# NVlabs/nvbio

Measured on AMD Instinct MI355X. Metric: aligned reads/s (100 bp, band=15), higher is better.
Workload: dtype int32 results (int16 lanes where proven exact; all-int32 kernel in roofline.a32); 1 GPU; nvbio::aln batched banded SW (configs[1]): 10000000 x 100 bp reads vs 150 bp windows per GPU, band=15, LOCAL Gotoh (2,-1,-2,-1); reads_per_gpu=10000000, read_len=100, band=15, type=LOCAL, parallelism=read-shard x1, gather to rank 0

## Files before the change

include/nvbio_hip.h:

```cpp
#ifndef NVBIO_HIP_H
#define NVBIO_HIP_H

#include <stdint.h>

#ifdef __cplusplus
extern "C" {
#endif

#define NVBIO_HIP_ABI_VERSION 2

enum { NVBIO_HIP_GLOBAL = 0, NVBIO_HIP_LOCAL = 1, NVBIO_HIP_SEMI_GLOBAL = 2 };

typedef struct nvbio_hip_string_set {
    const uint32_t* words;
    uint64_t        n_words;
    uint32_t        bits;
    uint32_t        big_endian;
    const uint64_t* begin;
    const uint32_t* length;
    uint32_t        fixed_length;
    uint32_t        _pad;
} nvbio_hip_string_set;

typedef struct nvbio_hip_gotoh_scheme {
    int32_t match, mismatch, gap_open, gap_ext;
} nvbio_hip_gotoh_scheme;


int nvbio_hip_banded_gotoh_score(
    const nvbio_hip_gotoh_scheme* scheme , int32_t type, uint32_t band_len,
    const nvbio_hip_string_set* patterns ,
    const nvbio_hip_string_set* texts    ,
    uint32_t max_pattern_len, uint32_t max_text_len ,
    uint32_t n, int32_t* out_score, uint32_t* out_sink, void* stream);

int nvbio_hip_gotoh_score(
    const nvbio_hip_gotoh_scheme* scheme , int32_t type,
    const nvbio_hip_string_set* patterns, const nvbio_hip_string_set* texts,
    uint32_t max_pattern_len, uint32_t max_text_len, const int32_t* min_score ,
    uint32_t n, int32_t* out_score, uint32_t* out_sink, uint8_t* out_ok, void* stream);

typedef struct nvbio_hip_sw_scheme { int32_t match, mismatch, deletion, insertion; } nvbio_hip_sw_scheme;

int nvbio_hip_banded_sw_score(
    const nvbio_hip_sw_scheme* scheme , int32_t type, uint32_t band_len,
    const nvbio_hip_string_set* patterns, const nvbio_hip_string_set* texts,
    uint32_t max_pattern_len, uint32_t max_text_len,
    uint32_t n, int32_t* out_score, uint32_t* out_sink, void* stream);
int nvbio_hip_sw_score(
    const nvbio_hip_sw_scheme* scheme , int32_t type,
    const nvbio_hip_string_set* patterns, const nvbio_hip_string_set* texts,
    uint32_t max_pattern_len, uint32_t max_text_len,
    uint32_t n, int32_t* out_score, uint32_t* out_sink, void* stream);

enum { NVBIO_HIP_GOTOH_ALIGNER = 0, NVBIO_HIP_SW_ALIGNER = 1 };
enum { NVBIO_HIP_PATTERN_BLOCKING = 0, NVBIO_HIP_TEXT_BLOCKING = 1 };
int nvbio_hip_alignment_score(
    int32_t aligner, int32_t algorithm, const int32_t* scheme4 , int32_t type,
    const nvbio_hip_string_set* patterns, const nvbio_hip_string_set* texts,
    uint32_t max_pattern_len, uint32_t max_text_len, const int32_t* min_score ,
    uint32_t n, int32_t* out_score, uint32_t* out_sink, uint8_t* out_ok , void* stream);

typedef struct nvbio_hip_gotoh_qual_scheme {
    int32_t match;
    int32_t pattern_gap_open, pattern_gap_ext, text_gap_open, text_gap_ext;
    int32_t mismatch[256];
} nvbio_hip_gotoh_qual_scheme;

int nvbio_hip_banded_gotoh_score_qual(
    const nvbio_hip_gotoh_qual_scheme* scheme , int32_t type, uint32_t band_len,
    const nvbio_hip_string_set* patterns, const uint8_t* quals, uint64_t n_quals,
    const nvbio_hip_string_set* texts,
    uint32_t max_pattern_len, uint32_t max_text_len,
    uint32_t n, int32_t* out_score, uint32_t* out_sink, void* stream);

int nvbio_hip_banded_gotoh_score_qual_views(
    const nvbio_hip_gotoh_qual_scheme* scheme , int32_t type, uint32_t band_len,
    const nvbio_hip_string_set* patterns, const uint8_t* quals, uint64_t n_quals, const uint8_t* pattern_flags ,
    const nvbio_hip_string_set* texts,
    uint32_t max_pattern_len, uint32_t max_text_len,
    uint32_t n, int32_t* out_score, uint32_t* out_sink, void* stream);

int nvbio_hip_banded_gotoh_score_qual_wave(
    const nvbio_hip_gotoh_qual_scheme* scheme, int32_t type, uint32_t band_len,
    const nvbio_hip_string_set* patterns, const uint8_t* quals , uint64_t n_quals,
    const nvbio_hip_string_set* texts, uint32_t max_pattern_len,
    uint32_t n, const uint32_t* n_on_device , const uint32_t* job_index , const uint32_t* out_index ,
    const uint32_t* gate , uint32_t gate_limit,
    int32_t* out_score, uint32_t* out_sink, void* stream);

int nvbio_hip_banded_gotoh_score_qual_bounded(
    const nvbio_hip_gotoh_qual_scheme* scheme, int32_t type, uint32_t band_len,
    const nvbio_hip_string_set* patterns, const uint8_t* quals, uint64_t n_quals, const uint8_t* pattern_flags,
    const nvbio_hip_string_set* texts,
    uint32_t max_pattern_len, uint32_t max_text_len,
    uint32_t n, const uint32_t* n_on_device, const int32_t* min_score, uint32_t* work_counter, const uint32_t* out_index,
    const uint32_t* gate , uint32_t gate_limit,
    int32_t* out_score, uint32_t* out_sink, void* stream);

uint64_t nvbio_hip_banded_gotoh_traceback_temp_bytes(uint32_t band_len, uint32_t max_pattern_len, uint32_t n);
int nvbio_hip_banded_gotoh_traceback(
    const nvbio_hip_gotoh_scheme* scheme , int32_t type, uint32_t band_len,
    const nvbio_hip_string_set* patterns, const nvbio_hip_string_set* texts,
    uint32_t max_pattern_len, uint32_t max_text_len, uint32_t n,
    int32_t* out_score, uint32_t* out_sink, uint32_t* out_source,
    uint16_t* out_cigar, uint32_t cigar_stride, uint32_t* out_cigar_len,
    void* temp, uint64_t temp_bytes, void* stream);
int nvbio_hip_banded_gotoh_traceback_qual(
    const nvbio_hip_gotoh_qual_scheme* scheme , int32_t type, uint32_t band_len,
    const nvbio_hip_string_set* patterns, const uint8_t* quals, uint64_t n_quals,
    const nvbio_hip_string_set* texts,
    uint32_t max_pattern_len, uint32_t max_text_len, uint32_t n,
    int32_t* out_score, uint32_t* out_sink, uint32_t* out_source,
    uint16_t* out_cigar, uint32_t cigar_stride, uint32_t* out_cigar_len,
    void* temp, uint64_t temp_bytes, void* stream);
int nvbio_hip_banded_gotoh_traceback_qual_known(
    const nvbio_hip_gotoh_qual_scheme* scheme , int32_t type, uint32_t band_len,
    const nvbio_hip_string_set* patterns, const uint8_t* quals, uint64_t n_quals,
    const nvbio_hip_string_set* texts,
    uint32_t max_pattern_len, uint32_t max_text_len, uint32_t n,
    int32_t* score , uint32_t* sink , uint32_t* out_source,
    uint16_t* out_cigar, uint32_t cigar_stride, uint32_t* out_cigar_len,
    void* temp, uint64_t temp_bytes, void* stream);

uint64_t nvbio_hip_gotoh_traceback_temp_bytes(uint32_t max_pattern_len, uint32_t max_text_len, uint32_t n);
int nvbio_hip_gotoh_traceback(
    const nvbio_hip_gotoh_scheme* scheme , int32_t type,
    const nvbio_hip_string_set* patterns, const nvbio_hip_string_set* texts,
    uint32_t max_pattern_len, uint32_t max_text_len, uint32_t n,
    int32_t* out_score, uint32_t* out_sink, uint32_t* out_source,
    uint16_t* out_cigar, uint32_t cigar_stride, uint32_t* out_cigar_len,
    void* temp, uint64_t temp_bytes, void* stream);

int nvbio_hip_gotoh_traceback_qual(
    const nvbio_hip_gotoh_qual_scheme* scheme , int32_t type,
    const nvbio_hip_string_set* patterns, const uint8_t* quals, uint64_t n_quals, const nvbio_hip_string_set* texts,
    uint32_t max_pattern_len, uint32_t max_text_len, uint32_t n,
    int32_t* out_score, uint32_t* out_sink, uint32_t* out_source,
    uint16_t* out_cigar, uint32_t cigar_stride, uint32_t* out_cigar_len,
    void* temp, uint64_t temp_bytes, void* stream);

int nvbio_hip_gotoh_traceback_known_score(
    const nvbio_hip_gotoh_scheme* scheme , int32_t type,
    const nvbio_hip_string_set* patterns, const nvbio_hip_string_set* texts, const int32_t* known_score,
    uint32_t max_pattern_len, uint32_t max_text_len, uint32_t n,
    int32_t* out_score, uint32_t* out_sink, uint32_t* out_source,
    uint16_t* out_cigar, uint32_t cigar_stride, uint32_t* out_cigar_len,
    void* temp, uint64_t temp_bytes, void* stream);
int nvbio_hip_gotoh_traceback_qual_known_score(
    const nvbio_hip_gotoh_qual_scheme* scheme , int32_t type,
    const nvbio_hip_string_set* patterns, const uint8_t* quals, uint64_t n_quals, const nvbio_hip_string_set* texts, const int32_t* known_score,
    uint32_t max_pattern_len, uint32_t max_text_len, uint32_t n,
    int32_t* out_score, uint32_t* out_sink, uint32_t* out_source,
    uint16_t* out_cigar, uint32_t cigar_stride, uint32_t* out_cigar_len,
    void* temp, uint64_t temp_bytes, void* stream);

uint64_t nvbio_hip_known_score_redone(void);

int nvbio_hip_banded_sw_traceback(
    const nvbio_hip_sw_scheme* scheme , int32_t type, uint32_t band_len,
    const nvbio_hip_string_set* patterns, const nvbio_hip_string_set* texts,
    uint32_t max_pattern_len, uint32_t max_text_len, uint32_t n,
    int32_t* out_score, uint32_t* out_sink, uint32_t* out_source,
    uint16_t* out_cigar, uint32_t cigar_stride, uint32_t* out_cigar_len,
    void* temp, uint64_t temp_bytes, void* stream);
int nvbio_hip_sw_traceback(
    const nvbio_hip_sw_scheme* scheme , int32_t type,
    const nvbio_hip_string_set* patterns, const nvbio_hip_string_set* texts,
    uint32_t max_pattern_len, uint32_t max_text_len, uint32_t n,
    int32_t* out_score, uint32_t* out_sink, uint32_t* out_source,
    uint16_t* out_cigar, uint32_t cigar_stride, uint32_t* out_cigar_len,
    void* temp, uint64_t temp_bytes, void* stream);

int nvbio_hip_alignment_score_qual(
    const nvbio_hip_gotoh_qual_scheme* scheme , int32_t algorithm, int32_t type,
    const nvbio_hip_string_set* patterns, const uint8_t* quals, uint64_t n_quals, const nvbio_hip_string_set* texts,
    uint32_t max_pattern_len, uint32_t max_text_len, const int32_t* min_score ,
    uint32_t n, int32_t* out_score, uint32_t* out_sink, uint8_t* out_ok , void* stream);

int nvbio_hip_alignment_score_qual_jobs(
    const nvbio_hip_gotoh_qual_scheme* scheme , int32_t algorithm, int32_t type,
    const nvbio_hip_string_set* patterns, const uint8_t* quals, uint64_t n_quals, const nvbio_hip_string_set* texts,
    uint32_t max_pattern_len, uint32_t max_text_len, const int32_t* min_score ,
    uint32_t n, const uint32_t* n_on_device, const uint32_t* job_index, const uint32_t* gate, uint32_t gate_limit, int32_t wave_form,
    int32_t* out_score, uint32_t* out_sink, uint8_t* out_ok , void* stream);

int nvbio_hip_hamming_score(
    const nvbio_hip_sw_scheme* scheme , int32_t algorithm, int32_t type,
    const nvbio_hip_string_set* patterns, const nvbio_hip_string_set* texts,
    uint32_t max_pattern_len, uint32_t max_text_len, const int32_t* min_score ,
    uint32_t n, int32_t* out_score, uint32_t* out_sink, uint8_t* out_ok , void* stream);
int nvbio_hip_hamming_score_qual(
    const nvbio_hip_gotoh_qual_scheme* scheme , int32_t algorithm, int32_t type,
    const nvbio_hip_string_set* patterns, const uint8_t* quals, uint64_t n_quals, const nvbio_hip_string_set* texts,
    uint32_t max_pattern_len, uint32_t max_text_len, const int32_t* min_score ,
    uint32_t n, int32_t* out_score, uint32_t* out_sink, uint8_t* out_ok , void* stream);
int nvbio_hip_hamming_score_qual_jobs(
    const nvbio_hip_gotoh_qual_scheme* scheme , int32_t algorithm, int32_t type,
    const nvbio_hip_string_set* patterns, const uint8_t* quals, uint64_t n_quals, const nvbio_hip_string_set* texts,
    uint32_t max_pattern_len, uint32_t max_text_len, const int32_t* min_score ,
    uint32_t n, const uint32_t* n_on_device, const uint32_t* job_index, const uint32_t* gate, uint32_t gate_limit, int32_t wave_form,
    int32_t* out_score, uint32_t* out_sink, uint8_t* out_ok , void* stream);

typedef struct nvbio_hip_fmindex {
    uint32_t        length;
    uint32_t        primary;
    uint32_t        L2[5];
    uint32_t        sa_int;
    const uint32_t* bwt_occ;
    const uint32_t* ssa;
    const uint32_t* ktab;
    uint32_t        ktab_k;
    uint32_t        _pad;
    const uint32_t* dimer;
    uint32_t        dimer_p1, dimer_fill1;
    uint32_t        dimer_S[4], dimer_T[4];
    const uint32_t* trimer;
} nvbio_hip_fmindex;

int nvbio_hip_fm_rank(const nvbio_hip_fmindex* fmi, const uint32_t* k, const uint8_t* c,
                      uint32_t n, uint32_t* out, void* stream);

int nvbio_hip_fm_rank4(const nvbio_hip_fmindex* fmi, const uint32_t* k,
                       uint32_t n, uint32_t* out, void* stream);

int nvbio_hip_fm_rank_range(const nvbio_hip_fmindex* fmi, const uint32_t* range, const uint8_t* c,
                            uint32_t n, uint32_t* out, void* stream);

int nvbio_hip_fm_match(const nvbio_hip_fmindex* fmi, const nvbio_hip_string_set* seeds,
                       uint32_t n, uint32_t* out_range, void* stream);

uint64_t nvbio_hip_fm_dimer_index_bytes(uint32_t length);
uint64_t nvbio_hip_fm_build_dimer_index_temp_bytes(uint32_t length);
int nvbio_hip_fm_build_dimer_index(const nvbio_hip_fmindex* fmi, uint32_t* out_dimer, void* temp, uint64_t temp_bytes, void* stream);
int nvbio_hip_fm_attach_dimer_index(nvbio_hip_fmindex* fmi, const uint32_t* dimer, void* stream);

uint64_t nvbio_hip_fm_trimer_index_bytes(uint32_t length);
uint64_t nvbio_hip_fm_build_trimer_index_temp_bytes(uint32_t length);
int nvbio_hip_fm_build_trimer_index(const nvbio_hip_fmindex* fmi, uint32_t* out_trimer, void* temp, uint64_t temp_bytes, void* stream);
int nvbio_hip_fm_attach_trimer_index(nvbio_hip_fmindex* fmi, const uint32_t* trimer, void* stream);

int nvbio_hip_banded_gotoh_score_host(const nvbio_hip_gotoh_scheme* scheme, int32_t type, uint32_t band_len,
                                      const nvbio_hip_string_set* patterns, const nvbio_hip_string_set* texts,
                                      uint32_t n, int32_t* out_score, uint32_t* out_sink, int32_t n_threads);
int nvbio_hip_banded_sw_score_host(const nvbio_hip_sw_scheme* scheme, int32_t type, uint32_t band_len,
                                   const nvbio_hip_string_set* patterns, const nvbio_hip_string_set* texts,
                                   uint32_t n, int32_t* out_score, uint32_t* out_sink, int32_t n_threads);
int nvbio_hip_alignment_score_host(int32_t aligner, int32_t algorithm, const int32_t* scheme4, int32_t type,
                                   const nvbio_hip_string_set* patterns, const nvbio_hip_string_set* texts, const int32_t* min_score ,
                                   uint32_t n, int32_t* out_score, uint32_t* out_sink, uint8_t* out_ok , int32_t n_threads);
int nvbio_hip_hamming_score_host(const nvbio_hip_sw_scheme* scheme, int32_t algorithm, int32_t type,
                                 const nvbio_hip_string_set* patterns, const nvbio_hip_string_set* texts, const int32_t* min_score ,
                                 uint32_t n, int32_t* out_score, uint32_t* out_sink, uint8_t* out_ok , int32_t n_threads);
int nvbio_hip_hamming_score_qual_host(const nvbio_hip_gotoh_qual_scheme* scheme, int32_t algorithm, int32_t type,
                                      const nvbio_hip_string_set* patterns, const uint8_t* quals, uint64_t n_quals, const nvbio_hip_string_set* texts,
                                      const int32_t* min_score ,
                                      uint32_t n, int32_t* out_score, uint32_t* out_sink, uint8_t* out_ok , int32_t n_threads);
int nvbio_hip_fm_rank_host(const nvbio_hip_fmindex* fmi, const uint32_t* k, const uint8_t* c, uint32_t n, uint32_t* out, int32_t n_threads);
int nvbio_hip_fm_match_host(const nvbio_hip_fmindex* fmi, const nvbio_hip_string_set* seeds, uint32_t n, uint32_t* out_range, int32_t n_threads);
int nvbio_hip_fm_locate_host(const nvbio_hip_fmindex* fmi, const uint32_t* sa_rows, uint32_t n, uint32_t* out_pos, int32_t n_threads);

int nvbio_hip_fm_build_ktab(const nvbio_hip_fmindex* fmi, uint32_t k, uint32_t* out_ktab, void* stream);
uint64_t nvbio_hip_fm_dense_ssa_entries(uint32_t length, uint32_t sa_int);
int nvbio_hip_fm_build_dense_ssa(const nvbio_hip_fmindex* fmi, uint32_t sa_int_out, uint32_t* out_ssa, void* stream);

typedef struct nvbio_hip_map_params {
    uint32_t seed_len;
    uint32_t min_read_len;
    uint32_t max_hits;
    uint32_t max_reseed;
    uint32_t retry;
    uint32_t rep_seeds;
    uint32_t fw, rc;
} nvbio_hip_map_params;

int nvbio_hip_map_exact(const nvbio_hip_fmindex* fmi, const nvbio_hip_string_set* reads,
                        const uint32_t* in_queue, uint32_t n, const nvbio_hip_map_params* params ,
                        const uint32_t* seed_freq_by_len ,
                        uint64_t* out_hits, uint32_t hits_stride, uint32_t* out_counts, uint8_t* out_reseed, void* stream);

enum { NVBIO_HIP_EXACT_MAPPING = 0, NVBIO_HIP_APPROX_MAPPING = 1, NVBIO_HIP_CASE_PRUNING_MAPPING = 2 };

int nvbio_hip_map(int32_t algorithm, uint32_t subseed_len,
                  const nvbio_hip_fmindex* fmi, const nvbio_hip_fmindex* rfmi ,
                  const nvbio_hip_string_set* reads, const uint32_t* in_queue, uint32_t n,
                  const nvbio_hip_map_params* params , const uint32_t* seed_freq_by_len ,
                  uint64_t* out_hits, uint32_t hits_stride, uint32_t* out_counts, uint8_t* out_reseed, void* stream);

uint64_t nvbio_hip_alignment_invalid(void);
int nvbio_hip_init_alignments(uint32_t n_reads, const uint32_t* read_len , uint32_t fixed_read_len,
                              const int32_t* worst_score_by_len , uint32_t mate,
                              uint64_t* best_alignments, uint32_t best_stride, void* stream);
int nvbio_hip_score_reduce(uint32_t n_active, const uint32_t* read_ids , const uint64_t* hit_begin,
                           const int32_t* hit_score, const uint32_t* hit_loc, const uint8_t* hit_rc,
                           const uint32_t* read_len , uint32_t fixed_read_len,
                           uint64_t* best_alignments, uint32_t best_stride, void* stream);

uint32_t nvbio_hip_sum_tree_node_count(uint32_t size);
int nvbio_hip_select_init(uint32_t n_reads, const char* read_names, const uint32_t* read_names_idx,
                          const uint64_t* hits, uint32_t hits_stride, const uint32_t* hit_counts,
                          float* probs, uint32_t probs_stride, uint32_t* trys , uint32_t* rseeds,
                          uint32_t max_effort_init, int32_t randomized, int32_t top_seed, void* stream);
int nvbio_hip_select_init_queued(uint32_t n_queue, const uint32_t* queue, const char* read_names, const uint32_t* read_names_idx,
                                 const uint64_t* hits, uint32_t hits_stride, const uint32_t* hit_counts,
                                 float* probs, uint32_t probs_stride, uint32_t* trys , uint32_t* rseeds,
                                 uint32_t max_effort_init, int32_t randomized, int32_t top_seed, void* stream);
uint64_t nvbio_hip_select_temp_bytes(uint32_t n_active, uint32_t n_multi);
int nvbio_hip_select(int32_t randomized, uint32_t n_multi, const uint32_t* active_in, uint32_t n_active,
                     uint64_t* hits, uint32_t hits_stride, uint32_t* hit_counts,
                     float* probs, uint32_t probs_stride, uint32_t* rseeds, const uint32_t* trys,
                     uint32_t* active_out, uint64_t* hit_begin, uint32_t* hit_read_id, uint32_t* hit_loc, uint32_t* hit_seed,
                     uint32_t* out_sizes, void* temp, uint64_t temp_bytes, void* stream);
int nvbio_hip_hit_deque_replay(uint32_t n_cases, const uint32_t* case_start, const uint8_t* ops, const uint64_t* vals, const uint32_t* caps,
                               const uint64_t* state_start, uint64_t* scratch, uint32_t scratch_stride, uint64_t* out_states, void* stream);
int nvbio_hip_locate_hits(const nvbio_hip_fmindex* fmi, const nvbio_hip_fmindex* rfmi, uint32_t n,
                          uint32_t* hit_loc, const uint32_t* hit_seed, void* stream);
int nvbio_hip_score_best_setup(uint32_t n_hits, const uint32_t* hit_read_id, const uint32_t* hit_loc, const uint32_t* hit_seed,
                               const uint64_t* read_begin , const uint32_t* read_len , uint32_t fixed_read_len,
                               uint64_t rc_offset, uint32_t band_len, uint32_t genome_length,
                               const uint64_t* best_alignments, uint32_t best_stride, int32_t score_limit,
                               uint64_t* pattern_begin, uint32_t* pattern_len ,
                               uint64_t* text_begin, uint32_t* text_len, int32_t* min_score,
                               int32_t* known_score ,
                               uint32_t* job_count , uint32_t* job_hit , void* stream);
int nvbio_hip_score_reduce_best_approx(uint32_t n_active, const uint32_t* active_reads, const uint64_t* hit_begin,
                                       const int32_t* hit_score, const uint32_t* hit_loc, const uint32_t* hit_seed,
                                       const uint32_t* read_len , uint32_t fixed_read_len,
                                       uint64_t* best_alignments, uint32_t best_stride, int32_t worst_score,
                                       uint32_t* trys, uint32_t* hit_counts,
                                       uint32_t n_ext, uint32_t min_ext, uint32_t max_ext, uint32_t max_effort,
                                       const int32_t* known_score ,
                                       const uint32_t* hit_sink , uint32_t* best_sink ,
                                       void* stream);
int nvbio_hip_traceback_best_known(uint32_t n, const uint32_t* idx , const uint64_t* best_alignments, const uint32_t* best_sink ,
                                   int32_t* out_score, uint32_t* out_sink , void* stream);

int nvbio_hip_score_reduce_paired(uint32_t n_active, const uint32_t* read_ids , const uint64_t* hit_begin,
    const uint32_t* hit_loc, const uint32_t* hit_sink, const int32_t* hit_score, const uint8_t* hit_rc,
    const uint32_t* opposite_loc, const uint32_t* opposite_sink, const uint32_t* opposite_sink2,
    const int32_t* opposite_score, const int32_t* opposite_score2,
    const uint32_t* read_len , uint32_t fixed_read_len, uint32_t anchor, int32_t pe_policy, int32_t pe_unpaired, int32_t score_limit,
    uint64_t* best_alignments, uint64_t* best_alignments_o, uint32_t best_stride, void* stream);

typedef struct nvbio_hip_pe_params {
    int32_t  pe_policy, min_frag_len, max_frag_len, pe_overlap, score_limit;
    uint32_t anchor, genome_length;
} nvbio_hip_pe_params;

int nvbio_hip_opposite_mate_windows(uint32_t n_hits, const uint32_t* hit_read_id, const uint8_t* hit_rc, const uint32_t* hit_loc, const int32_t* hit_score,
    const uint32_t* a_read_len , const uint32_t* o_read_len , uint32_t a_fixed_len, uint32_t o_fixed_len,
    const uint64_t* best_alignments, const uint64_t* best_alignments_o, uint32_t best_stride,
    int32_t match, const int32_t* min_score_by_len , int32_t text_gap_open, int32_t text_gap_ext, const nvbio_hip_pe_params* params ,
    uint8_t* out_valid, int32_t* out_min_score, uint8_t* out_read_rc, uint32_t* out_genome_begin, uint32_t* out_genome_end, void* stream);

int nvbio_hip_anchor_score_setup(uint32_t n_hits, const uint32_t* hit_read_id, const uint32_t* hit_loc, const uint32_t* hit_seed,
    const uint64_t* a_read_begin , const uint32_t* a_read_len , const uint32_t* o_read_len ,
    uint32_t a_fixed_len, uint32_t o_fixed_len, uint64_t rc_offset,
    uint32_t band_len, uint32_t genome_length, const uint64_t* best_alignments, const uint64_t* best_alignments_o, uint32_t best_stride,
    int32_t match, const int32_t* min_score_by_len , int32_t score_limit, uint32_t anchor,
    uint64_t* pattern_begin, uint32_t* pattern_len , uint64_t* text_begin, uint32_t* text_len, int32_t* min_score, void* stream);
int nvbio_hip_anchor_score_finish(uint32_t n_hits, const int32_t* raw_score, const uint32_t* raw_sink , const uint64_t* text_begin,
    const int32_t* min_score, int32_t worst_score, int32_t* hit_score, uint32_t* hit_sink, void* stream);
int nvbio_hip_opposite_score_setup(uint32_t n_hits, const uint32_t* hit_read_id, const uint32_t* hit_seed, const uint32_t* hit_loc, const int32_t* hit_score,
    int32_t worst_score, const uint32_t* a_read_len, const uint32_t* o_read_len, uint32_t a_fixed_len, uint32_t o_fixed_len,
    const uint64_t* best_alignments, const uint64_t* best_alignments_o, uint32_t best_stride,
    int32_t match, const int32_t* min_score_by_len , int32_t text_gap_open, int32_t text_gap_ext, const nvbio_hip_pe_params* params ,
    uint8_t* out_valid, int32_t* out_min_score, uint8_t* out_read_rc, uint32_t* out_genome_begin, uint32_t* out_genome_end,
    const uint64_t* o_read_begin, uint64_t o_rc_offset, uint64_t* out_pattern_begin, uint64_t* out_text_begin, uint32_t* out_text_len, void* stream);
int nvbio_hip_opposite_score_finish(uint32_t n_valid, const uint32_t* valid_idx, const uint8_t* valid_flags, const int32_t* raw_score , const uint32_t* raw_sink ,
    const int32_t* min_score , const uint32_t* genome_begin , int32_t worst_score,
    int32_t* opposite_score, int32_t* opposite_score2, uint32_t* opposite_loc, uint32_t* opposite_sink, uint32_t* opposite_sink2, void* stream);
int nvbio_hip_score_reduce_paired_best_approx(uint32_t n_active, const uint32_t* active_reads, const uint64_t* hit_begin,
    const uint32_t* hit_loc, const uint32_t* hit_sink, const int32_t* hit_score, const uint32_t* hit_seed,
    const uint32_t* opposite_loc, const uint32_t* opposite_sink, const uint32_t* opposite_sink2, const int32_t* opposite_score, const int32_t* opposite_score2,
    const uint32_t* read_len , uint32_t fixed_read_len, uint32_t anchor, int32_t pe_policy, int32_t pe_unpaired, int32_t score_limit,
    uint64_t* best_alignments, uint64_t* best_alignments_o, uint32_t best_stride,
    uint32_t* trys, uint32_t* hit_counts, uint32_t n_ext, uint32_t min_ext, uint32_t max_ext, uint32_t max_effort, void* stream);
int nvbio_hip_anchor_memo_mark(uint32_t n_hits, const uint32_t* hit_read_id, const uint32_t* hit_seed, const uint64_t* text_begin, const uint32_t* text_len,
    uint32_t anchor, const uint32_t* memo, uint8_t* from_memo, uint32_t* text_len_out,
    uint32_t* live_count , uint32_t* live_idx , void* stream);
int nvbio_hip_anchor_score_finish_memo(uint32_t n_hits, const int32_t* raw_score, const uint32_t* raw_sink, const uint64_t* text_begin, const int32_t* min_score,
    int32_t worst_score, const uint8_t* from_memo, const uint32_t* hit_read_id, const uint32_t* memo, int32_t* hit_score, uint32_t* hit_sink, void* stream);
int nvbio_hip_anchor_memo_update(uint32_t n_active, const uint32_t* active_reads, const uint64_t* hit_begin, const uint32_t* hit_read_id, const uint32_t* hit_seed,
    const uint64_t* text_begin, const uint32_t* text_len_setup, const uint8_t* from_memo, const int32_t* raw_score, const uint32_t* raw_sink, uint32_t anchor, uint32_t* memo, void* stream);
int nvbio_hip_list_flagged(uint32_t n, const uint8_t* flags, uint32_t value, uint32_t* count, uint32_t* idx, void* stream);
int nvbio_hip_opposite_memo_lookup(uint32_t n_hits, const uint32_t* hit_read_id, uint8_t* valid, const uint8_t* read_rc, const uint32_t* genome_begin,
    const uint32_t* genome_end, const int32_t* min_score, uint32_t anchor, const uint32_t* memo, int32_t worst_score,
    int32_t* opposite_score, int32_t* opposite_score2, uint32_t* opposite_loc, uint32_t* opposite_sink, uint32_t* opposite_sink2,
    uint32_t* text_len , void* stream);
int nvbio_hip_opposite_memo_update(uint32_t n_active, const uint32_t* active_reads, const uint64_t* hit_begin, const uint8_t* valid, const uint8_t* read_rc,
    const uint32_t* genome_begin, const uint32_t* genome_end, const int32_t* min_score, const int32_t* opposite_score, const uint32_t* opposite_sink,
    uint32_t anchor, uint32_t* memo, void* stream);
int nvbio_hip_mark_discordant(uint32_t n_reads, uint64_t* best_alignments, uint64_t* best_alignments_o, uint32_t best_stride, void* stream);

int nvbio_hip_pack_read_queue(uint32_t n, const uint32_t* queue, uint32_t top_flag, uint32_t* out, void* stream);

int nvbio_hip_mark_unaligned(uint32_t n_active, const uint32_t* active_reads, const uint64_t* best_alignments, uint8_t* reseed, void* stream);
uint64_t nvbio_hip_copy_flagged_temp_bytes(uint32_t n);
int nvbio_hip_copy_flagged(uint32_t n, const uint32_t* in, const uint8_t* flags, uint32_t* out, uint32_t* out_count ,
                           void* temp, uint64_t temp_bytes, void* stream);
int nvbio_hip_scatter_rows(uint32_t n, const uint32_t* idx, const void* src, void* dst, uint32_t row_bytes , void* stream);
int nvbio_hip_gather_rows(uint32_t n, const uint32_t* idx, const void* src, void* dst, uint32_t row_bytes , void* stream);
int nvbio_hip_traceback_best_setup(uint32_t n, const uint32_t* idx , const uint64_t* best_alignments, uint32_t band_len, uint32_t genome_length,
                                   const uint64_t* read_begin , const uint32_t* read_len , uint32_t fixed_read_len,
                                   uint64_t rc_offset, uint64_t mate_offset, int32_t want,
                                   uint8_t* out_valid, uint64_t* pattern_begin, uint32_t* pattern_len ,
                                   uint64_t* text_begin, uint32_t* text_len, void* stream);
int nvbio_hip_traceback_best_setup_mates(uint32_t n, const uint32_t* idx , const uint64_t* best_alignments, uint32_t band_len, uint32_t genome_length,
                                         const uint64_t* const read_begin[2] , const uint32_t* const read_len[2],
                                         const uint32_t fixed_read_len[2], const uint64_t rc_offset[2], uint64_t mate_offset, int32_t want,
                                         uint8_t* out_valid, uint64_t* pattern_begin, uint32_t* pattern_len, uint64_t* text_begin, uint32_t* text_len, void* stream);

int nvbio_hip_finish_alignment(uint32_t n, const uint8_t* valid, const nvbio_hip_string_set* patterns, const uint8_t* quals , uint64_t n_quals,
                               const nvbio_hip_string_set* texts, const uint16_t* cigar, uint32_t cigar_stride, const uint32_t* cigar_len,
                               const uint32_t* cigar_source , int32_t match, const int32_t* mismatch_by_quality , int32_t n_penalty,
                               const int32_t* gap_costs , const uint32_t* idx , uint64_t* best_alignments, uint8_t* out_mds, uint32_t mds_stride, uint32_t* out_mds_len, void* stream);

int nvbio_hip_gather_ranges(uint32_t n_ranges, uint32_t n_reads, const uint64_t* hits, uint32_t hits_stride, const uint32_t* hit_count_scan,
                            uint64_t* out_ranges, void* stream);
int nvbio_hip_select_all(uint64_t begin, uint32_t count, uint32_t n_reads, uint32_t n_ranges, const uint64_t* hits, uint32_t hits_stride,
                         const uint32_t* hit_count_scan, const uint64_t* hit_range_scan, uint32_t* out_loc, uint32_t* out_seed, uint32_t* out_read_id,
                         void* stream);
int nvbio_hip_mark_straddling(uint32_t n, const uint32_t* idx_queue, uint32_t n_sequences, const uint32_t* sequence_index, const uint32_t* hit_loc,
                              uint32_t seed_len, uint8_t* flags, void* stream);
int nvbio_hip_score_all_setup(uint32_t n, const uint32_t* idx , const uint32_t* hit_read_id, const uint32_t* hit_loc, const uint32_t* hit_seed,
                              const uint64_t* read_begin , const uint32_t* read_len , uint32_t fixed_read_len, uint64_t rc_offset,
                              uint32_t band_len, uint32_t genome_length,
                              uint64_t* pattern_begin, uint32_t* pattern_len , uint64_t* text_begin, uint32_t* text_len, void* stream);
int nvbio_hip_score_all_output(uint32_t n, const uint32_t* idx , const uint32_t* hit_read_id, const uint32_t* hit_loc, const uint32_t* hit_seed,
                               const int32_t* score, const int32_t* min_score_by_len , const uint32_t* read_len , uint32_t fixed_read_len,
                               uint8_t* out_flags, uint64_t* out_alignments, uint32_t* out_read_id, void* stream);
int nvbio_hip_traceback_all_setup(uint32_t n, const uint64_t* alignments, const uint32_t* read_id,
                                  const uint64_t* read_begin , const uint32_t* read_len , uint32_t fixed_read_len, uint64_t rc_offset,
                                  uint32_t band_len, uint32_t genome_length,
                                  uint64_t* pattern_begin, uint32_t* pattern_len , uint64_t* text_begin, uint32_t* text_len, void* stream);

uint64_t nvbio_hip_all_mapping_temp_bytes(uint32_t n);
int nvbio_hip_inclusive_scan_u32(uint32_t n, const uint32_t* in, uint32_t* out, void* temp, uint64_t temp_bytes, void* stream);
int nvbio_hip_inclusive_scan_u64(uint32_t n, const uint64_t* in, uint64_t* out, void* temp, uint64_t temp_bytes, void* stream);
int nvbio_hip_sort_hi_bits(uint32_t n, const uint32_t* keys, uint32_t* out_idx, void* temp, uint64_t temp_bytes, void* stream);
int nvbio_hip_sort_hits(uint32_t n, const uint32_t* hit_read_id, const uint32_t* hit_loc, const uint32_t* hit_seed, uint32_t* out_idx, uint8_t* out_first,
                        void* temp, uint64_t temp_bytes, void* stream);
int nvbio_hip_sort_hits_pingpong(uint32_t n, const uint32_t* hit_read_id, const uint32_t* hit_loc, const uint32_t* hit_seed, uint32_t* out_idx, uint8_t* out_first,
                                 uint32_t* out_stale, void* temp, uint64_t temp_bytes, void* stream);

int nvbio_hip_mapq(int32_t version, int32_t match, int32_t monotone, const int32_t* min_score_by_len ,
                   uint32_t n_reads, const uint64_t* best_alignments, uint32_t best_stride,
                   const uint32_t* read_len , uint32_t fixed_read_len, uint8_t* out_mapq, void* stream);

int nvbio_hip_mapq_paired(int32_t version, int32_t match, int32_t monotone, const int32_t* min_score_by_len ,
                          uint32_t n_reads, const uint64_t* best_alignments, const uint64_t* best_alignments_o, uint32_t best_stride,
                          const uint32_t* read_len , const uint32_t* o_read_len ,
                          uint32_t fixed_read_len, uint32_t o_fixed_read_len, uint8_t* out_mapq, void* stream);

int nvbio_hip_fm_locate(const nvbio_hip_fmindex* fmi, const uint32_t* sa_rows,
                        uint32_t n, uint32_t* out_pos, void* stream);

int nvbio_hip_fm_locate_ssa_iterator(const nvbio_hip_fmindex* fmi, const uint32_t* sa_rows,
                                     uint32_t n, uint32_t* out_it, void* stream);
int nvbio_hip_fm_lookup_ssa_iterator(const nvbio_hip_fmindex* fmi, const uint32_t* it,
                                     uint32_t n, uint32_t* out_pos, void* stream);

uint64_t nvbio_hip_fm_filter_temp_bytes(uint32_t n);
int nvbio_hip_fm_filter_rank(const nvbio_hip_fmindex* fmi, const nvbio_hip_string_set* seeds,
                             uint32_t n, uint32_t* out_range, uint64_t* out_slots,
                             void* temp, uint64_t temp_bytes, void* stream);

int nvbio_hip_fm_filter_locate(const nvbio_hip_fmindex* fmi, const uint32_t* range, const uint64_t* slots,
                               uint32_t n_queries, uint64_t begin, uint64_t end,
                               uint32_t* out_hits, void* stream);

#define NVBIO_HIP_EXTEND_FORWARD   0
#define NVBIO_HIP_EXTEND_BACKWARDS 1
int nvbio_hip_fm_extend(int32_t direction, const nvbio_hip_fmindex* f_fmi, const nvbio_hip_fmindex* r_fmi,
                        const uint32_t* f_ranges, const uint32_t* r_ranges, const uint8_t* c, uint32_t n,
                        uint32_t* out_f_ranges, uint32_t* out_r_ranges, void* stream);

#define NVBIO_HIP_ERROR_CAPACITY 0x10001
uint64_t nvbio_hip_fm_mem_temp_bytes(uint32_t n, uint32_t max_pattern_len);
int nvbio_hip_fm_mem_rank(const nvbio_hip_fmindex* f_fmi, const nvbio_hip_fmindex* r_fmi, const nvbio_hip_string_set* strings,
                          uint32_t n, uint32_t max_pattern_len, uint32_t min_intv, uint32_t max_intv, uint32_t min_span,
                          uint32_t* out_ranges, uint64_t capacity, uint64_t* out_index, uint64_t* out_slots, uint64_t* out_n_ranges,
                          void* temp, uint64_t temp_bytes, void* stream);

int nvbio_hip_fm_mem_locate(const nvbio_hip_fmindex* f_fmi, const uint32_t* ranges, const uint64_t* slots, uint64_t n_ranges,
                            uint64_t begin, uint64_t end, uint32_t* out_hits, void* stream);

int nvbio_hip_fm_extend_host(int32_t direction, const nvbio_hip_fmindex* f_fmi, const nvbio_hip_fmindex* r_fmi,
                             const uint32_t* f_ranges, const uint32_t* r_ranges, const uint8_t* c, uint32_t n,
                             uint32_t* out_f_ranges, uint32_t* out_r_ranges, int32_t n_threads);
int nvbio_hip_fm_mem_rank_host(const nvbio_hip_fmindex* f_fmi, const nvbio_hip_fmindex* r_fmi, const nvbio_hip_string_set* strings,
                               uint32_t n, uint32_t max_pattern_len, uint32_t min_intv, uint32_t max_intv, uint32_t min_span,
                               uint32_t* out_ranges, uint64_t capacity, uint64_t* out_index, uint64_t* out_slots, uint64_t* out_n_ranges,
                               uint64_t* out_records, int32_t n_threads);
int nvbio_hip_fm_mem_locate_host(const nvbio_hip_fmindex* f_fmi, const uint32_t* ranges, const uint64_t* slots, uint64_t n_ranges,
                                 uint64_t begin, uint64_t end, uint32_t* out_hits, int32_t n_threads);

uint64_t nvbio_hip_fm_mem_split_temp_bytes(uint32_t n, uint32_t max_pattern_len, uint64_t capacity);
int nvbio_hip_fm_mem_rank_split(const nvbio_hip_fmindex* f_fmi, const nvbio_hip_fmindex* r_fmi, const nvbio_hip_string_set* strings,
                                uint32_t n, uint32_t max_pattern_len, uint32_t min_intv, uint32_t max_intv, uint32_t min_span,
                                uint32_t split_len, uint32_t split_width,
                                uint32_t* out_ranges, uint64_t capacity, uint64_t* out_index, uint64_t* out_slots, uint64_t* out_n_ranges,
                                void* temp, uint64_t temp_bytes, void* stream);
int nvbio_hip_fm_mem_rank_split_host(const nvbio_hip_fmindex* f_fmi, const nvbio_hip_fmindex* r_fmi, const nvbio_hip_string_set* strings,
                                     uint32_t n, uint32_t max_pattern_len, uint32_t min_intv, uint32_t max_intv, uint32_t min_span,
                                     uint32_t split_len, uint32_t split_width,
                                     uint32_t* out_ranges, uint64_t capacity, uint64_t* out_index, uint64_t* out_slots, uint64_t* out_n_ranges,
                                     uint64_t* out_records, int32_t n_threads);

uint64_t nvbio_hip_build_bwt_occ_temp_bytes(uint32_t n);
int nvbio_hip_build_bwt_occ(uint32_t n, const uint32_t* bwt_words, uint32_t* out_bwt_occ, uint32_t* out_L2,
                            void* temp, uint64_t temp_bytes, void* stream);

uint64_t nvbio_hip_suffix_sort_temp_bytes(uint64_t n);
int nvbio_hip_suffix_sort(const uint32_t* words, uint32_t bits, uint32_t big_endian, uint64_t n, uint32_t* sa_out,
                          void* temp, uint64_t temp_bytes, void* stream);
uint32_t nvbio_hip_suffix_sort_last_rounds(uint64_t* out_unresolved, uint32_t capacity);
uint64_t nvbio_hip_bwt_temp_bytes(uint64_t n);
int nvbio_hip_bwt(const uint32_t* words, uint32_t bits, uint32_t big_endian, uint64_t n, uint32_t sa_int, uint32_t* bwt_words_out,
                  uint32_t* primary_out, uint32_t* ssa_out, uint32_t* sa_out, void* temp, uint64_t temp_bytes, void* stream);
int nvbio_hip_suffix_sort_host(const uint32_t* words, uint32_t bits, uint32_t big_endian, uint64_t n, uint32_t* sa_out, int32_t n_threads);
int nvbio_hip_bwt_host(const uint32_t* words, uint32_t bits, uint32_t big_endian, uint64_t n, uint32_t sa_int, uint32_t* bwt_words_out,
                       uint32_t* primary_out, uint32_t* ssa_out, uint32_t* sa_out, int32_t n_threads);

uint64_t nvbio_hip_set_suffix_sort_temp_bytes(uint64_t n_suffixes, uint32_t n_strings);
int nvbio_hip_set_suffix_sort(const nvbio_hip_string_set* set ,
                              uint32_t n_strings, uint64_t n_suffixes,
                              uint32_t* suffixes_out   ,
                              uint32_t* string_ids_out ,
                              uint32_t* cum_lengths_out,
                              void* temp, uint64_t temp_bytes, void* stream);
uint64_t nvbio_hip_set_bwt_temp_bytes(uint64_t n_suffixes, uint32_t n_strings);
int nvbio_hip_set_bwt(const nvbio_hip_string_set* set, uint32_t n_strings, uint64_t n_suffixes,
                      uint8_t*  bwt_out        ,
                      uint32_t* dollar_rows_out, uint32_t* dollar_ids_out ,
                      uint32_t* suffixes_out   ,
                      void* temp, uint64_t temp_bytes, void* stream);
int nvbio_hip_set_suffix_sort_host(const nvbio_hip_string_set* set, uint32_t n_strings, uint64_t n_suffixes, uint32_t* suffixes_out,
                                   uint32_t* string_ids_out, uint32_t* cum_lengths_out, int32_t n_threads);
int nvbio_hip_set_bwt_host(const nvbio_hip_string_set* set, uint32_t n_strings, uint64_t n_suffixes, uint8_t* bwt_out,
                           uint32_t* dollar_rows_out, uint32_t* dollar_ids_out, uint32_t* suffixes_out, int32_t n_threads);

int nvbio_hip_device_malloc(void** ptr, uint64_t bytes);
int nvbio_hip_device_free(void* ptr);
int nvbio_hip_device_free_ordered(void* ptr);
int nvbio_hip_device_free_after(void* ptr, void* stream);
int nvbio_hip_device_trim(void);
int nvbio_hip_device_mem_info(uint64_t* free_bytes, uint64_t* total_bytes, uint64_t* idle_cached_bytes);
int nvbio_hip_memcpy(void* dst, const void* src, uint64_t bytes, int kind, void* stream);
int nvbio_hip_memset(void* dst, int value, uint64_t bytes, void* stream);
int nvbio_hip_stream_synchronize(void* stream);
int nvbio_hip_stream_query(void* stream);
int nvbio_hip_host_malloc(void** ptr, uint64_t bytes);
int nvbio_hip_host_free(void* ptr);

int nvbio_hip_stream_create(void** stream, uint32_t non_blocking);
int nvbio_hip_stream_destroy(void* stream);

int nvbio_hip_comm_available(void);
int nvbio_hip_device_count(void);
int nvbio_hip_set_device(int device);
int nvbio_hip_get_device(void);
int nvbio_hip_comm_unique_id(uint8_t* id128);
int nvbio_hip_comm_init_rank(void** comm, int world, int rank, const uint8_t* id128);
int nvbio_hip_comm_init_all(void** comms, int n_devices, const int* devices );
int nvbio_hip_comm_destroy(void* comm);
int nvbio_hip_comm_rank(void* comm, int* rank, int* world);
int nvbio_hip_gather_records(void* comm, const void* send, const uint64_t* counts, uint32_t record_bytes, void* recv , int root, void* stream);
int nvbio_hip_comm_abort(void* comm);
typedef struct nvbio_hip_comm_transport {
    int (*rank)(void* comm, int* rank, int* world);
    int (*group_start)(void* comm);
    int (*group_end)(void* comm);
    int (*send)(void* comm, const void* buf, uint64_t bytes, int peer, void* stream);
    int (*recv)(void* comm, void* buf, uint64_t bytes, int peer, void* stream);
    int (*copy)(void* comm, void* dst, const void* src, uint64_t bytes, void* stream);
    int (*abort)(void* comm);
} nvbio_hip_comm_transport;
void nvbio_hip_comm_set_transport(const nvbio_hip_comm_transport* transport);

int nvbio_hip_set_test_switch(const char* name, int value);
int nvbio_hip_get_test_switch(const char* name);
const char* nvbio_hip_test_switch_name(int index);

int         nvbio_hip_abi_version(void);
const char* nvbio_hip_arch(void);
const char* nvbio_hip_last_kernel(void);
const char* nvbio_hip_last_kernel_detail(void);
const char* nvbio_hip_last_kernel_cell(void);
const char* nvbio_hip_last_kernel_frame(void);
const char* nvbio_hip_last_kernel_row(void);
const char* nvbio_hip_last_kernel_const(void);
const char* nvbio_hip_last_kernel_sub(void);
const char* nvbio_hip_last_kernel_fetch(void);

#ifdef __cplusplus
}
#endif
#endif
```

nvbio_amd/_lib.py:

```python
import ctypes as C
import os

HERE = os.path.dirname(os.path.abspath(__file__))
LIB_PATH = os.path.join(HERE, "lib", "libnvbio_hip.so")

SYMBOLS = [
    "nvbio_hip_banded_gotoh_score", "nvbio_hip_banded_gotoh_score_qual", "nvbio_hip_banded_gotoh_score_qual_views", "nvbio_hip_banded_gotoh_score_qual_bounded", "nvbio_hip_banded_gotoh_score_qual_wave", "nvbio_hip_gotoh_score", "nvbio_hip_banded_sw_score", "nvbio_hip_sw_score", "nvbio_hip_alignment_score", "nvbio_hip_alignment_score_qual", "nvbio_hip_alignment_score_qual_jobs",
    "nvbio_hip_hamming_score", "nvbio_hip_hamming_score_qual", "nvbio_hip_hamming_score_qual_jobs", "nvbio_hip_hamming_score_host", "nvbio_hip_hamming_score_qual_host",
    "nvbio_hip_banded_gotoh_traceback_temp_bytes", "nvbio_hip_banded_gotoh_traceback", "nvbio_hip_banded_gotoh_traceback_qual",
    "nvbio_hip_gotoh_traceback_temp_bytes", "nvbio_hip_gotoh_traceback", "nvbio_hip_gotoh_traceback_qual", "nvbio_hip_gotoh_traceback_known_score", "nvbio_hip_gotoh_traceback_qual_known_score", "nvbio_hip_known_score_redone", "nvbio_hip_banded_sw_traceback", "nvbio_hip_sw_traceback",
    "nvbio_hip_fm_rank", "nvbio_hip_fm_rank4", "nvbio_hip_fm_rank_range",
    "nvbio_hip_fm_match", "nvbio_hip_fm_build_ktab", "nvbio_hip_fm_dense_ssa_entries", "nvbio_hip_fm_build_dense_ssa",
    "nvbio_hip_banded_gotoh_score_host", "nvbio_hip_banded_sw_score_host", "nvbio_hip_alignment_score_host",
    "nvbio_hip_fm_rank_host", "nvbio_hip_fm_match_host", "nvbio_hip_fm_locate_host",
    "nvbio_hip_fm_dimer_index_bytes", "nvbio_hip_fm_build_dimer_index_temp_bytes", "nvbio_hip_fm_build_dimer_index", "nvbio_hip_fm_attach_dimer_index",
    "nvbio_hip_fm_trimer_index_bytes", "nvbio_hip_fm_build_trimer_index_temp_bytes", "nvbio_hip_fm_build_trimer_index", "nvbio_hip_fm_attach_trimer_index", "nvbio_hip_map_exact", "nvbio_hip_map",
    "nvbio_hip_alignment_invalid", "nvbio_hip_init_alignments", "nvbio_hip_score_reduce", "nvbio_hip_score_reduce_paired", "nvbio_hip_opposite_mate_windows", "nvbio_hip_mapq", "nvbio_hip_mapq_paired", "nvbio_hip_fm_locate",
    "nvbio_hip_sum_tree_node_count", "nvbio_hip_select_init", "nvbio_hip_select_init_queued", "nvbio_hip_select_temp_bytes", "nvbio_hip_select", "nvbio_hip_locate_hits", "nvbio_hip_hit_deque_replay",
    "nvbio_hip_score_best_setup", "nvbio_hip_score_reduce_best_approx",
    "nvbio_hip_anchor_score_setup", "nvbio_hip_anchor_score_finish", "nvbio_hip_anchor_memo_mark", "nvbio_hip_anchor_score_finish_memo", "nvbio_hip_anchor_memo_update", "nvbio_hip_opposite_score_setup", "nvbio_hip_opposite_score_finish",
    "nvbio_hip_score_reduce_paired_best_approx", "nvbio_hip_mark_discordant",
    "nvbio_hip_pack_read_queue", "nvbio_hip_mark_unaligned", "nvbio_hip_copy_flagged_temp_bytes", "nvbio_hip_copy_flagged", "nvbio_hip_traceback_best_setup", "nvbio_hip_traceback_best_setup_mates", "nvbio_hip_finish_alignment", "nvbio_hip_scatter_rows",
    "nvbio_hip_gather_ranges", "nvbio_hip_select_all", "nvbio_hip_mark_straddling", "nvbio_hip_score_all_setup", "nvbio_hip_score_all_output",
    "nvbio_hip_traceback_all_setup", "nvbio_hip_all_mapping_temp_bytes", "nvbio_hip_inclusive_scan_u32", "nvbio_hip_inclusive_scan_u64", "nvbio_hip_sort_hi_bits",
    "nvbio_hip_sort_hits", "nvbio_hip_sort_hits_pingpong", "nvbio_hip_gather_rows", "nvbio_hip_list_flagged", "nvbio_hip_opposite_memo_lookup", "nvbio_hip_opposite_memo_update", "nvbio_hip_traceback_best_known", "nvbio_hip_banded_gotoh_traceback_qual_known",
    "nvbio_hip_fm_locate_ssa_iterator", "nvbio_hip_fm_lookup_ssa_iterator",
    "nvbio_hip_fm_filter_temp_bytes", "nvbio_hip_fm_filter_rank", "nvbio_hip_fm_filter_locate",
    "nvbio_hip_fm_extend", "nvbio_hip_fm_mem_temp_bytes", "nvbio_hip_fm_mem_rank", "nvbio_hip_fm_mem_locate",
    "nvbio_hip_fm_extend_host", "nvbio_hip_fm_mem_rank_host", "nvbio_hip_fm_mem_locate_host",
    "nvbio_hip_fm_mem_split_temp_bytes", "nvbio_hip_fm_mem_rank_split", "nvbio_hip_fm_mem_rank_split_host",
    "nvbio_hip_build_bwt_occ_temp_bytes", "nvbio_hip_build_bwt_occ",
    "nvbio_hip_suffix_sort_temp_bytes", "nvbio_hip_suffix_sort", "nvbio_hip_suffix_sort_last_rounds", "nvbio_hip_bwt_temp_bytes", "nvbio_hip_bwt",
    "nvbio_hip_suffix_sort_host", "nvbio_hip_bwt_host",
    "nvbio_hip_set_suffix_sort_temp_bytes", "nvbio_hip_set_suffix_sort", "nvbio_hip_set_bwt_temp_bytes", "nvbio_hip_set_bwt",
    "nvbio_hip_set_suffix_sort_host", "nvbio_hip_set_bwt_host",
    "nvbio_hip_device_malloc", "nvbio_hip_device_free", "nvbio_hip_device_free_ordered", "nvbio_hip_device_free_after", "nvbio_hip_device_trim", "nvbio_hip_device_mem_info", "nvbio_hip_memcpy", "nvbio_hip_memset",
    "nvbio_hip_stream_synchronize", "nvbio_hip_stream_query", "nvbio_hip_host_malloc", "nvbio_hip_host_free", "nvbio_hip_stream_create", "nvbio_hip_stream_destroy",
    "nvbio_hip_comm_available", "nvbio_hip_device_count", "nvbio_hip_set_device", "nvbio_hip_get_device", "nvbio_hip_comm_unique_id", "nvbio_hip_comm_init_rank",
    "nvbio_hip_comm_init_all", "nvbio_hip_comm_destroy", "nvbio_hip_comm_rank", "nvbio_hip_gather_records", "nvbio_hip_comm_abort", "nvbio_hip_comm_set_transport",
    "nvbio_hip_abi_version", "nvbio_hip_arch", "nvbio_hip_last_kernel", "nvbio_hip_last_kernel_detail", "nvbio_hip_last_kernel_cell", "nvbio_hip_last_kernel_frame", "nvbio_hip_last_kernel_row", "nvbio_hip_last_kernel_const", "nvbio_hip_last_kernel_sub", "nvbio_hip_last_kernel_fetch", "nvbio_hip_set_test_switch", "nvbio_hip_get_test_switch", "nvbio_hip_test_switch_name",
]


class PeParamsStruct(C.Structure):
    _fields_ = [("pe_policy", C.c_int32), ("min_frag_len", C.c_int32), ("max_frag_len", C.c_int32), ("pe_overlap", C.c_int32),
                ("score_limit", C.c_int32), ("anchor", C.c_uint32), ("genome_length", C.c_uint32)]


class StringSetStruct(C.Structure):
    _fields_ = [("words", C.c_void_p), ("n_words", C.c_uint64), ("bits", C.c_uint32), ("big_endian", C.c_uint32),
                ("begin", C.c_void_p), ("length", C.c_void_p), ("fixed_length", C.c_uint32), ("_pad", C.c_uint32)]


class GotohSchemeStruct(C.Structure):
    _fields_ = [("match", C.c_int32), ("mismatch", C.c_int32), ("gap_open", C.c_int32), ("gap_ext", C.c_int32)]


class GotohQualSchemeStruct(C.Structure):
    _fields_ = [("match", C.c_int32), ("pattern_gap_open", C.c_int32), ("pattern_gap_ext", C.c_int32),
                ("text_gap_open", C.c_int32), ("text_gap_ext", C.c_int32), ("mismatch", C.c_int32 * 256)]


class MapParamsStruct(C.Structure):
    _fields_ = [(k, C.c_uint32) for k in ("seed_len", "min_read_len", "max_hits", "max_reseed", "retry", "rep_seeds", "fw", "rc")]


class FMIndexStruct(C.Structure):
    _fields_ = [("length", C.c_uint32), ("primary", C.c_uint32), ("L2", C.c_uint32 * 5), ("sa_int", C.c_uint32),
                ("bwt_occ", C.c_void_p), ("ssa", C.c_void_p), ("ktab", C.c_void_p), ("ktab_k", C.c_uint32), ("_pad", C.c_uint32),
                ("dimer", C.c_void_p), ("dimer_p1", C.c_uint32), ("dimer_fill1", C.c_uint32),
                ("dimer_S", C.c_uint32 * 4), ("dimer_T", C.c_uint32 * 4), ("trimer", C.c_void_p)]


_lib = None
ABI_VERSION = 2
ERROR_CAPACITY = 0x10001


def lib():
    global _lib
    if _lib is None:
        if not os.path.exists(LIB_PATH):
            raise RuntimeError(
                "nvbio_amd: %s is missing -- build it with `python -m nvbio_amd.build` "
                "(hipcc --offload-arch=gfx950); there is no CPU fallback" % LIB_PATH)
        L = C.CDLL(LIB_PATH)
        try:
            L.nvbio_hip_abi_version.restype = C.c_int
            found = L.nvbio_hip_abi_version()
        except AttributeError:
            found = None
        if found != ABI_VERSION:
            raise RuntimeError("nvbio_amd: lib/libnvbio_hip.so has ABI version %s, this package needs %d -- rebuild it (python -m nvbio_amd.build)" % (found, ABI_VERSION))
        for s in SYMBOLS:
            getattr(L, s)
        vp, u32, u64, i32 = C.c_void_p, C.c_uint32, C.c_uint64, C.c_int32
        P = C.POINTER
        L.nvbio_hip_banded_gotoh_score.argtypes = [P(GotohSchemeStruct), i32, u32, P(StringSetStruct), P(StringSetStruct), u32, u32, u32, vp, vp, vp]
        L.nvbio_hip_banded_gotoh_score_qual.argtypes = [P(GotohQualSchemeStruct), i32, u32, P(StringSetStruct), vp, u64, P(StringSetStruct), u32, u32, u32, vp, vp, vp]
        L.nvbio_hip_banded_gotoh_score_qual_views.argtypes = [P(GotohQualSchemeStruct), i32, u32, P(StringSetStruct), vp, u64, vp, P(StringSetStruct), u32, u32, u32, vp, vp, vp]
        L.nvbio_hip_banded_gotoh_score_qual_bounded.argtypes = [P(GotohQualSchemeStruct), i32, u32, P(StringSetStruct), vp, u64, vp, P(StringSetStruct), u32, u32, u32, vp, vp, vp, vp, vp, u32, vp, vp, vp]
        L.nvbio_hip_banded_gotoh_score_qual_wave.argtypes = [P(GotohQualSchemeStruct), i32, u32, P(StringSetStruct), vp, u64, P(StringSetStruct), u32, u32, vp, vp, vp, vp, u32, vp, vp, vp]
        L.nvbio_hip_banded_gotoh_traceback_temp_bytes.argtypes = [u32, u32, u32]
        L.nvbio_hip_banded_gotoh_traceback_temp_bytes.restype = u64
        L.nvbio_hip_banded_gotoh_traceback.argtypes = [P(GotohSchemeStruct), i32, u32, P(StringSetStruct), P(StringSetStruct), u32, u32, u32,
                                                       vp, vp, vp, vp, u32, vp, vp, u64, vp]
        L.nvbio_hip_banded_gotoh_traceback_qual.argtypes = [P(GotohQualSchemeStruct), i32, u32, P(StringSetStruct), vp, u64, P(StringSetStruct), u32, u32, u32,
                                                            vp, vp, vp, vp, u32, vp, vp, u64, vp]
        L.nvbio_hip_banded_gotoh_traceback_qual_known.argtypes = [P(GotohQualSchemeStruct), i32, u32, P(StringSetStruct), vp, u64, P(StringSetStruct), u32, u32, u32,
                                                            vp, vp, vp, vp, u32, vp, vp, u64, vp]
        L.nvbio_hip_banded_sw_score.argtypes = [P(GotohSchemeStruct), i32, u32, P(StringSetStruct), P(StringSetStruct), u32, u32, u32, vp, vp, vp]
        L.nvbio_hip_sw_score.argtypes = [P(GotohSchemeStruct), i32, P(StringSetStruct), P(StringSetStruct), u32, u32, u32, vp, vp, vp]
        L.nvbio_hip_alignment_score.argtypes = [i32, i32, vp, i32, P(StringSetStruct), P(StringSetStruct), u32, u32, vp, u32, vp, vp, vp, vp]
        L.nvbio_hip_gotoh_traceback_temp_bytes.argtypes = [u32, u32, u32]
        L.nvbio_hip_gotoh_traceback_temp_bytes.restype = u64
        L.nvbio_hip_gotoh_traceback.argtypes = [P(GotohSchemeStruct), i32, P(StringSetStruct), P(StringSetStruct), u32, u32, u32,
                                                vp, vp, vp, vp, u32, vp, vp, u64, vp]
        L.nvbio_hip_gotoh_traceback_qual.argtypes = [P(GotohQualSchemeStruct), i32, P(StringSetStruct), vp, u64, P(StringSetStruct), u32, u32, u32,
                                                     vp, vp, vp, vp, u32, vp, vp, u64, vp]
        L.nvbio_hip_gotoh_traceback_known_score.argtypes = [P(GotohSchemeStruct), i32, P(StringSetStruct), P(StringSetStruct), vp, u32, u32, u32,
                                                            vp, vp, vp, vp, u32, vp, vp, u64, vp]
        L.nvbio_hip_gotoh_traceback_qual_known_score.argtypes = [P(GotohQualSchemeStruct), i32, P(StringSetStruct), vp, u64, P(StringSetStruct), vp, u32, u32, u32,
                                                                 vp, vp, vp, vp, u32, vp, vp, u64, vp]
        L.nvbio_hip_known_score_redone.argtypes = []; L.nvbio_hip_known_score_redone.restype = u64
        L.nvbio_hip_banded_sw_traceback.argtypes = [P(GotohSchemeStruct), i32, u32, P(StringSetStruct), P(StringSetStruct), u32, u32, u32,
                                                    vp, vp, vp, vp, u32, vp, vp, u64, vp]
        L.nvbio_hip_sw_traceback.argtypes = [P(GotohSchemeStruct), i32, P(StringSetStruct), P(StringSetStruct), u32, u32, u32,
                                             vp, vp, vp, vp, u32, vp, vp, u64, vp]
        L.nvbio_hip_alignment_score_qual.argtypes = [P(GotohQualSchemeStruct), i32, i32, P(StringSetStruct), vp, u64, P(StringSetStruct), u32, u32, vp, u32, vp, vp, vp, vp]
        L.nvbio_hip_gotoh_score.argtypes = [P(GotohSchemeStruct), i32, P(StringSetStruct), P(StringSetStruct), u32, u32, vp, u32, vp, vp, vp, vp]
        L.nvbio_hip_hamming_score.argtypes = [P(GotohSchemeStruct), i32, i32, P(StringSetStruct), P(StringSetStruct), u32, u32, vp, u32, vp, vp, vp, vp]
        L.nvbio_hip_hamming_score_qual.argtypes = [P(GotohQualSchemeStruct), i32, i32, P(StringSetStruct), vp, u64, P(StringSetStruct), u32, u32, vp, u32, vp, vp, vp, vp]
        L.nvbio_hip_hamming_score_qual_jobs.argtypes = [P(GotohQualSchemeStruct), i32, i32, P(StringSetStruct), vp, u64, P(StringSetStruct), u32, u32, vp,
                                                        u32, vp, vp, vp, u32, i32, vp, vp, vp, vp]
        L.nvbio_hip_hamming_score_host.argtypes = [P(GotohSchemeStruct), i32, i32, P(StringSetStruct), P(StringSetStruct), vp, u32, vp, vp, vp, i32]
        L.nvbio_hip_hamming_score_qual_host.argtypes = [P(GotohQualSchemeStruct), i32, i32, P(StringSetStruct), vp, u64, P(StringSetStruct), vp, u32, vp, vp, vp, i32]
        L.nvbio_hip_fm_rank.argtypes = [P(FMIndexStruct), vp, vp, u32, vp, vp]
        L.nvbio_hip_fm_rank4.argtypes = [P(FMIndexStruct), vp, u32, vp, vp]
        L.nvbio_hip_fm_rank_range.argtypes = [P(FMIndexStruct), vp, vp, u32, vp, vp]
        L.nvbio_hip_fm_match.argtypes = [P(FMIndexStruct), P(StringSetStruct), u32, vp, vp]
        L.nvbio_hip_fm_build_ktab.argtypes = [P(FMIndexStruct), u32, vp, vp]
        L.nvbio_hip_banded_gotoh_score_host.argtypes = [P(GotohSchemeStruct), i32, u32, P(StringSetStruct), P(StringSetStruct), u32, vp, vp, i32]
        L.nvbio_hip_banded_sw_score_host.argtypes = [P(GotohSchemeStruct), i32, u32, P(StringSetStruct), P(StringSetStruct), u32, vp, vp, i32]
        L.nvbio_hip_alignment_score_host.argtypes = [i32, i32, vp, i32, P(StringSetStruct), P(StringSetStruct), vp, u32, vp, vp, vp, i32]
        L.nvbio_hip_fm_rank_host.argtypes = [P(FMIndexStruct), vp, vp, u32, vp, i32]
        L.nvbio_hip_fm_match_host.argtypes = [P(FMIndexStruct), P(StringSetStruct), u32, vp, i32]
        L.nvbio_hip_fm_locate_host.argtypes = [P(FMIndexStruct), vp, u32, vp, i32]
        L.nvbio_hip_fm_dimer_index_bytes.argtypes = [u32]; L.nvbio_hip_fm_dimer_index_bytes.restype = u64
        L.nvbio_hip_fm_build_dimer_index_temp_bytes.argtypes = [u32]; L.nvbio_hip_fm_build_dimer_index_temp_bytes.restype = u64
        L.nvbio_hip_fm_build_dimer_index.argtypes = [P(FMIndexStruct), vp, vp, u64, vp]
        L.nvbio_hip_fm_attach_dimer_index.argtypes = [P(FMIndexStruct), vp, vp]
        L.nvbio_hip_fm_trimer_index_bytes.argtypes = [u32]; L.nvbio_hip_fm_trimer_index_bytes.restype = u64
        L.nvbio_hip_fm_build_trimer_index_temp_bytes.argtypes = [u32]; L.nvbio_hip_fm_build_trimer_index_temp_bytes.restype = u64
        L.nvbio_hip_fm_build_trimer_index.argtypes = [P(FMIndexStruct), vp, vp, u64, vp]
        L.nvbio_hip_fm_attach_trimer_index.argtypes = [P(FMIndexStruct), vp, vp]
        L.nvbio_hip_map_exact.argtypes = [P(FMIndexStruct), P(StringSetStruct), vp, u32, P(MapParamsStruct), vp, vp, u32, vp, vp, vp]
        L.nvbio_hip_map.argtypes = [i32, u32, P(FMIndexStruct), P(FMIndexStruct), P(StringSetStruct), vp, u32, P(MapParamsStruct), vp, vp, u32, vp, vp, vp]
        L.nvbio_hip_alignment_invalid.argtypes = []
        L.nvbio_hip_alignment_invalid.restype = u64
        L.nvbio_hip_init_alignments.argtypes = [u32, vp, u32, vp, u32, vp, u32, vp]
        L.nvbio_hip_score_reduce.argtypes = [u32, vp, vp, vp, vp, vp, vp, u32, vp, u32, vp]
        L.nvbio_hip_sum_tree_node_count.argtypes = [u32]; L.nvbio_hip_sum_tree_node_count.restype = u32
        L.nvbio_hip_select_init.argtypes = [u32, vp, vp, vp, u32, vp, vp, u32, vp, vp, u32, i32, i32, vp]
        L.nvbio_hip_select_init_queued.argtypes = [u32, vp, vp, vp, vp, u32, vp, vp, u32, vp, vp, u32, i32, i32, vp]
        L.nvbio_hip_select_temp_bytes.argtypes = [u32, u32]; L.nvbio_hip_select_temp_bytes.restype = u64
        L.nvbio_hip_select.argtypes = [i32, u32, vp, u32, vp, u32, vp, vp, u32, vp, vp, vp, vp, vp, vp, vp, vp, vp, u64, vp]
        L.nvbio_hip_hit_deque_replay.argtypes = [u32, vp, vp, vp, vp, vp, vp, u32, vp, vp]
        L.nvbio_hip_locate_hits.argtypes = [P(FMIndexStruct), P(FMIndexStruct), u32, vp, vp, vp]
        L.nvbio_hip_score_best_setup.argtypes = [u32, vp, vp, vp, vp, vp, u32, u64, u32, u32, vp, u32, i32, vp, vp, vp, vp, vp, vp, vp, vp, vp]
        L.nvbio_hip_score_reduce_best_approx.argtypes = [u32, vp, vp, vp, vp, vp, vp, u32, vp, u32, i32, vp, vp, u32, u32, u32, u32, vp, vp, vp, vp]
        L.nvbio_hip_traceback_best_known.argtypes = [u32, vp, vp, vp, vp, vp, vp]
        L.nvbio_hip_anchor_score_setup.argtypes = [u32, vp, vp, vp, vp, vp, vp, u32, u32, u64, u32, u32, vp, vp, u32, i32, vp, i32, u32, vp, vp, vp, vp, vp, vp]
        L.nvbio_hip_anchor_score_finish.argtypes = [u32, vp, vp, vp, vp, i32, vp, vp, vp]
        L.nvbio_hip_opposite_score_setup.argtypes = [u32, vp, vp, vp, vp, i32, vp, vp, u32, u32, vp, vp, u32, i32, vp, i32, i32, P(PeParamsStruct), vp, vp, vp, vp, vp, vp, u64, vp, vp, vp, vp]
        L.nvbio_hip_scatter_rows.argtypes = [u32, vp, vp, vp, u32, vp]
        L.nvbio_hip_gather_rows.argtypes = [u32, vp, vp, vp, u32, vp]
        L.nvbio_hip_opposite_memo_lookup.argtypes = [u32, vp, vp, vp, vp, vp, vp, u32, vp, i32, vp, vp, vp, vp, vp, vp, vp]
        L.nvbio_hip_opposite_memo_update.argtypes = [u32, vp, vp, vp, vp, vp, vp, vp, vp, vp, u32, vp, vp]
        L.nvbio_hip_gather_ranges.argtypes = [u32, u32, vp, u32, vp, vp, vp]
        L.nvbio_hip_select_all.argtypes = [u64, u32, u32, u32, vp, u32, vp, vp, vp, vp, vp, vp]
        L.nvbio_hip_mark_straddling.argtypes = [u32, vp, u32, vp, vp, u32, vp, vp]
        L.nvbio_hip_score_all_setup.argtypes = [u32, vp, vp, vp, vp, vp, vp, u32, u64, u32, u32, vp, vp, vp, vp, vp]
        L.nvbio_hip_score_all_output.argtypes = [u32, vp, vp, vp, vp, vp, vp, vp, u32, vp, vp, vp, vp]
        L.nvbio_hip_traceback_all_setup.argtypes = [u32, vp, vp, vp, vp, u32, u64, u32, u32, vp, vp, vp, vp, vp]
        L.nvbio_hip_all_mapping_temp_bytes.argtypes = [u32]; L.nvbio_hip_all_mapping_temp_bytes.restype = u64
        L.nvbio_hip_inclusive_scan_u32.argtypes = [u32, vp, vp, vp, u64, vp]
        L.nvbio_hip_inclusive_scan_u64.argtypes = [u32, vp, vp, vp, u64, vp]
        L.nvbio_hip_sort_hi_bits.argtypes = [u32, vp, vp, vp, u64, vp]
        L.nvbio_hip_sort_hits.argtypes = [u32, vp, vp, vp, vp, vp, vp, u64, vp]
        L.nvbio_hip_sort_hits_pingpong.argtypes = [u32, vp, vp, vp, vp, vp, vp, vp, u64, vp]
        L.nvbio_hip_opposite_score_finish.argtypes = [u32, vp, vp, vp, vp, vp, vp, i32, vp, vp, vp, vp, vp, vp]
        L.nvbio_hip_score_reduce_paired_best_approx.argtypes = [u32, vp, vp, vp, vp, vp, vp, vp, vp, vp, vp, vp, vp, u32, u32, i32, i32, i32, vp, vp, u32, vp, vp, u32, u32, u32, u32, vp]
        L.nvbio_hip_mark_discordant.argtypes = [u32, vp, vp, u32, vp]
        L.nvbio_hip_pack_read_queue.argtypes = [u32, vp, u32, vp, vp]
        L.nvbio_hip_mark_unaligned.argtypes = [u32, vp, vp, vp, vp]
        L.nvbio_hip_copy_flagged_temp_bytes.argtypes = [u32]; L.nvbio_hip_copy_flagged_temp_bytes.restype = u64
        L.nvbio_hip_copy_flagged.argtypes = [u32, vp, vp, vp, vp, vp, u64, vp]
        L.nvbio_hip_finish_alignment.argtypes = [u32, vp, P(StringSetStruct), vp, u64, P(StringSetStruct), vp, u32, vp, vp, i32, vp, i32, vp, vp, vp, vp, u32, vp, vp]
        L.nvbio_hip_traceback_best_setup.argtypes = [u32, vp, vp, u32, u32, vp, vp, u32, u64, u64, i32, vp, vp, vp, vp, vp, vp]
        L.nvbio_hip_traceback_best_setup_mates.argtypes = [u32, vp, vp, u32, u32, C.POINTER(C.c_void_p), C.POINTER(C.c_void_p), C.POINTER(C.c_uint32), C.POINTER(C.c_uint64),
                                                           u64, i32, vp, vp, vp, vp, vp, vp]
        L.nvbio_hip_score_reduce_paired.argtypes = [u32, vp, vp, vp, vp, vp, vp, vp, vp, vp, vp, vp, vp, u32, u32, i32, i32, i32, vp, vp, u32, vp]
        L.nvbio_hip_opposite_mate_windows.argtypes = [u32, vp, vp, vp, vp, vp, vp, u32, u32, vp, vp, u32, i32, vp, i32, i32, P(PeParamsStruct),
                                                      vp, vp, vp, vp, vp, vp]
        L.nvbio_hip_mapq.argtypes = [i32, i32, i32, vp, u32, vp, u32, vp, u32, vp, vp]
        L.nvbio_hip_mapq_paired.argtypes = [i32, i32, i32, vp, u32, vp, vp, u32, vp, vp, u32, u32, vp, vp]
        L.nvbio_hip_fm_locate.argtypes = [P(FMIndexStruct), vp, u32, vp, vp]
        L.nvbio_hip_fm_locate_ssa_iterator.argtypes = [P(FMIndexStruct), vp, u32, vp, vp]
        L.nvbio_hip_fm_lookup_ssa_iterator.argtypes = [P(FMIndexStruct), vp, u32, vp, vp]
        L.nvbio_hip_fm_filter_temp_bytes.argtypes = [u32]
        L.nvbio_hip_fm_filter_temp_bytes.restype = u64
        L.nvbio_hip_fm_filter_rank.argtypes = [P(FMIndexStruct), P(StringSetStruct), u32, vp, vp, vp, u64, vp]
        L.nvbio_hip_fm_filter_locate.argtypes = [P(FMIndexStruct), vp, vp, u32, u64, u64, vp, vp]
        L.nvbio_hip_fm_extend.argtypes = [i32, P(FMIndexStruct), P(FMIndexStruct), vp, vp, vp, u32, vp, vp, vp]
        L.nvbio_hip_fm_mem_temp_bytes.argtypes = [u32, u32]
        L.nvbio_hip_fm_mem_temp_bytes.restype = u64
        L.nvbio_hip_fm_mem_rank.argtypes = [P(FMIndexStruct), P(FMIndexStruct), P(StringSetStruct), u32, u32, u32, u32, u32, vp, u64, vp, vp, P(u64), vp, u64, vp]
        L.nvbio_hip_fm_mem_locate.argtypes = [P(FMIndexStruct), vp, vp, u64, u64, u64, vp, vp]
        L.nvbio_hip_fm_extend_host.argtypes = [i32, P(FMIndexStruct), P(FMIndexStruct), vp, vp, vp, u32, vp, vp, i32]
        L.nvbio_hip_fm_mem_rank_host.argtypes = [P(FMIndexStruct), P(FMIndexStruct), P(StringSetStruct), u32, u32, u32, u32, u32, vp, u64, vp, vp, P(u64), P(u64), i32]
        L.nvbio_hip_fm_mem_locate_host.argtypes = [P(FMIndexStruct), vp, vp, u64, u64, u64, vp, i32]
        L.nvbio_hip_fm_mem_split_temp_bytes.argtypes = [u32, u32, u64]
        L.nvbio_hip_fm_mem_split_temp_bytes.restype = u64
        L.nvbio_hip_fm_mem_rank_split.argtypes = [P(FMIndexStruct), P(FMIndexStruct), P(StringSetStruct), u32, u32, u32, u32, u32, u32, u32, vp, u64, vp, vp, P(u64), vp, u64, vp]
        L.nvbio_hip_fm_mem_rank_split_host.argtypes = [P(FMIndexStruct), P(FMIndexStruct), P(StringSetStruct), u32, u32, u32, u32, u32, u32, u32, vp, u64, vp, vp, P(u64), P(u64), i32]
        L.nvbio_hip_build_bwt_occ_temp_bytes.argtypes = [u32]
        L.nvbio_hip_build_bwt_occ_temp_bytes.restype = u64
        L.nvbio_hip_build_bwt_occ.argtypes = [u32, vp, vp, vp, vp, u64, vp]
        L.nvbio_hip_suffix_sort_temp_bytes.argtypes = [u64]
        L.nvbio_hip_suffix_sort_temp_bytes.restype = u64
        L.nvbio_hip_suffix_sort.argtypes = [vp, u32, u32, u64, vp, vp, u64, vp]
        L.nvbio_hip_suffix_sort_last_rounds.argtypes = [P(u64), u32]
        L.nvbio_hip_suffix_sort_last_rounds.restype = u32
        L.nvbio_hip_bwt_temp_bytes.argtypes = [u64]
        L.nvbio_hip_bwt_temp_bytes.restype = u64
        L.nvbio_hip_bwt.argtypes = [vp, u32, u32, u64, u32, vp, P(u32), vp, vp, vp, u64, vp]
        L.nvbio_hip_suffix_sort_host.argtypes = [vp, u32, u32, u64, vp, i32]
        L.nvbio_hip_bwt_host.argtypes = [vp, u32, u32, u64, u32, vp, P(u32), vp, vp, i32]
        L.nvbio_hip_set_suffix_sort_temp_bytes.argtypes = [u64, u32]
        L.nvbio_hip_set_suffix_sort_temp_bytes.restype = u64
        L.nvbio_hip_set_suffix_sort.argtypes = [P(StringSetStruct), u32, u64, vp, vp, vp, vp, u64, vp]
        L.nvbio_hip_set_bwt_temp_bytes.argtypes = [u64, u32]
        L.nvbio_hip_set_bwt_temp_bytes.restype = u64
        L.nvbio_hip_set_bwt.argtypes = [P(StringSetStruct), u32, u64, vp, vp, vp, vp, vp, u64, vp]
        L.nvbio_hip_set_suffix_sort_host.argtypes = [P(StringSetStruct), u32, u64, vp, vp, vp, i32]
        L.nvbio_hip_set_bwt_host.argtypes = [P(StringSetStruct), u32, u64, vp, vp, vp, vp, i32]
        L.nvbio_hip_comm_unique_id.argtypes = [vp]
        L.nvbio_hip_comm_init_rank.argtypes = [P(vp), C.c_int, C.c_int, vp]
        L.nvbio_hip_comm_init_all.argtypes = [vp, C.c_int, vp]
        L.nvbio_hip_comm_destroy.argtypes = [vp]
        L.nvbio_hip_comm_rank.argtypes = [vp, P(C.c_int), P(C.c_int)]
        L.nvbio_hip_gather_records.argtypes = [vp, vp, vp, u32, vp, C.c_int, vp]
        L.nvbio_hip_set_device.argtypes = [C.c_int]
        L.nvbio_hip_abi_version.restype = C.c_int
        L.nvbio_hip_set_test_switch.argtypes = [C.c_char_p, C.c_int]
        L.nvbio_hip_get_test_switch.argtypes = [C.c_char_p]
        L.nvbio_hip_fm_dense_ssa_entries.argtypes = [u32, u32]
        L.nvbio_hip_fm_dense_ssa_entries.restype = u64
        L.nvbio_hip_fm_build_dense_ssa.argtypes = [P(FMIndexStruct), u32, vp, vp]
        L.nvbio_hip_test_switch_name.argtypes = [C.c_int]
        L.nvbio_hip_test_switch_name.restype = C.c_char_p
        L.nvbio_hip_device_free_after.argtypes = [vp, vp]
        L.nvbio_hip_device_mem_info.argtypes = [P(u64), P(u64), P(u64)]
        L.nvbio_hip_arch.restype = C.c_char_p
        L.nvbio_hip_last_kernel.restype = C.c_char_p
        L.nvbio_hip_last_kernel_detail.restype = C.c_char_p
        L.nvbio_hip_last_kernel_cell.restype = C.c_char_p
        L.nvbio_hip_last_kernel_frame.restype = C.c_char_p
        L.nvbio_hip_last_kernel_fetch.restype = C.c_char_p
        L.nvbio_hip_last_kernel_row.restype = C.c_char_p
        L.nvbio_hip_last_kernel_const.restype = C.c_char_p
        L.nvbio_hip_last_kernel_sub.restype = C.c_char_p
        _lib = L
    return _lib


def check(err, what):
    if err != 0:
        raise RuntimeError("nvbio_amd: %s failed with hipError %d" % (what, err))


def test_switch_names():
    out, k = [], 0
    while True:
        n = lib().nvbio_hip_test_switch_name(k)
        if not n:
            return out
        out.append(n.decode()); k += 1


def device_mem_info():
    f, t, i = C.c_uint64(), C.c_uint64(), C.c_uint64()
    check(lib().nvbio_hip_device_mem_info(C.byref(f), C.byref(t), C.byref(i)), "nvbio_hip_device_mem_info")
    return f.value, t.value, i.value


def set_test_switch(name, value):
    check(lib().nvbio_hip_set_test_switch(name.encode(), int(value)), "nvbio_hip_set_test_switch(%s)" % name)


class test_switch:

    def __init__(self, name, value):
        self.name, self.value = name, int(value)

    def __enter__(self):
        self.saved = lib().nvbio_hip_get_test_switch(self.name.encode())
        set_test_switch(self.name, self.value)
        return self

    def __exit__(self, *exc):
        set_test_switch(self.name, self.saved)
        return False


def current_stream_ptr():
    import torch
    if not torch.cuda.is_available():
        return C.c_void_p(0)
    return C.c_void_p(torch.cuda.current_stream().cuda_stream)
```

nvbio_amd/csrc/banded_gotoh.hip:

```cpp
#include "banded_gotoh_bounded.h"
#define NVB_PAIR_EXTERN
#include "banded_gotoh_pair.h"
#include <mutex>
#include <unordered_map>
#include <atomic>
#include <vector>
#include <algorithm>
#include <cstring>
#include <cstdlib>

namespace nvb {

thread_local const char* g_last_kernel = "";
thread_local PairLaunch g_last_pair;

#define NVB_DECL(B) \
    extern template hipError_t launch_band_width<B, NoQual>(const GotohParams&, const NoQual&, int, bool, hipStream_t); \
    extern template hipError_t launch_band_width<B, QualArgs>(const GotohParams&, const QualArgs&, int, bool, hipStream_t);
NVB_DECL(3) NVB_DECL(5) NVB_DECL(7) NVB_DECL(15) NVB_DECL(31)
#undef NVB_DECL
#define NVB_DECL(B) extern template hipError_t launch_band_width_asym<B>(const GotohParams&, int, bool, hipStream_t);
NVB_DECL(3) NVB_DECL(5) NVB_DECL(7) NVB_DECL(15) NVB_DECL(31)
#undef NVB_DECL
#define NVB_DECL(B) \
    extern template hipError_t launch_band_width_bounded<B, NoQual>(const GotohParams&, const NoQual&, const BoundArgs&, int, bool, hipStream_t); \
    extern template hipError_t launch_band_width_bounded<B, QualArgs>(const GotohParams&, const QualArgs&, const BoundArgs&, int, bool, hipStream_t);
NVB_DECL(3) NVB_DECL(5) NVB_DECL(7) NVB_DECL(15) NVB_DECL(31)
#undef NVB_DECL

template <typename QA>
static hipError_t launch_bounded(const GotohParams& p, const QA& qa, const BoundArgs& ba, int type, uint32_t band, bool width16, hipStream_t s)
{
    switch (band) {
    case 3:  return launch_band_width_bounded<3, QA>(p, qa, ba, type, width16, s);
    case 5:  return launch_band_width_bounded<5, QA>(p, qa, ba, type, width16, s);
    case 7:  return launch_band_width_bounded<7, QA>(p, qa, ba, type, width16, s);
    case 15: return launch_band_width_bounded<15, QA>(p, qa, ba, type, width16, s);
    case 31: return launch_band_width_bounded<31, QA>(p, qa, ba, type, width16, s);
    default: return hipErrorNotSupported;
    }
}

static hipError_t launch_asym(const GotohParams& p, int type, uint32_t band, bool width16, hipStream_t s)
{
    switch (band) {
    case 3:  return launch_band_width_asym<3>(p, type, width16, s);
    case 5:  return launch_band_width_asym<5>(p, type, width16, s);
    case 7:  return launch_band_width_asym<7>(p, type, width16, s);
    case 15: return launch_band_width_asym<15>(p, type, width16, s);
    case 31: return launch_band_width_asym<31>(p, type, width16, s);
    default: return hipErrorNotSupported;
    }
}

template <typename QA>
static hipError_t launch(const GotohParams& p, const QA& qa, int type, uint32_t band, bool width16, hipStream_t s)
{
    switch (band) {
    case 3:  return launch_band_width<3, QA>(p, qa, type, width16, s);
    case 5:  return launch_band_width<5, QA>(p, qa, type, width16, s);
    case 7:  return launch_band_width<7, QA>(p, qa, type, width16, s);
    case 15: return launch_band_width<15, QA>(p, qa, type, width16, s);
    case 31: return launch_band_width<31, QA>(p, qa, type, width16, s);
    default: return hipErrorNotSupported;
    }
}

static uint32_t max_len_16bit(int32_t match, int32_t best_pair , int64_t A , int32_t gap_open, int32_t gap_ext, int type, uint32_t band,
                              int32_t row_step )
{
    if (gap_open > 0 || gap_ext > 0) return 0;
    if (A == 0) return 0xFFFFFFFFu;
    if (type == NVBIO_HIP_LOCAL) {
        if (match < 0 || A > 100) return 0;
        const int64_t per_row = int64_t(std::max(best_pair, 0)) + row_step;
        if (per_row <= 0) return 0xFFFFFFFFu;
        return uint32_t(1022 / per_row);
    }
    const int64_t lim = (15000 / A - int64_t(band) - 2) / (row_step ? 2 : 1);
    return lim <= 0 ? 0u : uint32_t(lim);
}

static bool pair_admitted(const GotohParams& p, int type, uint32_t band, uint32_t lim16)
{
    if (test_switch(SW_BANDED_PAIR) == 1 || type != NVBIO_HIP_LOCAL || band != 15u) return false;
    if (p.pat.length || p.txt.length || p.n_dev || p.out_index || p.gate) return false;
    const uint32_t M = p.pat.fixed_length, N = p.txt.fixed_length;
    if (M == 0u || M > lim16 || uint64_t(N) < uint64_t(M) + band - 1u) return false;
    if (p.gap_ext > 0 || p.gap_open > p.gap_ext) return false;
    return p.mismatch >= p.gap_open && int64_t(std::max(p.match, p.mismatch)) - p.gap_open <= 7 && p.match >= p.gap_open;
}

static bool pair_stream_admitted(const GotohParams& p)
{
    return p.pat.s.bits != 8u && p.pat.s.n_words <= (1ull << 29) && p.txt.s.n_words <= (1ull << 29);
}
template <typename CELL, int ROW>
static hipError_t launch_pair_row(const GotohParams& p, hipStream_t s)
{
    g_last_pair.row = (ROW & PF_ROW2) ? "fold2" : "plain";
    g_last_pair.consts = (ROW & PF_CONST2) ? "literal" : "scalar";
    g_last_pair.sub = (ROW & PF_SUBLDS) ? "lds" : "perm";
    g_last_pair.fetch = "generic";
    if (!pair_stream_admitted(p)) return launch_band_pair<15, CELL, PF_SINK_VCC | ROW>(p, s);
    g_last_pair.fetch = "stream";
    switch (PF_STREAM | (p.pat.s.bits == 2u ? PF_PAT2 : 0) | (p.pat.s.big_endian ? PF_PBE : 0) | (p.txt.s.big_endian ? PF_TBE : 0)) {
#define NVB_CASE(F) case (F): return launch_band_pair<15, CELL, (F) | ROW>(p, s);
    NVB_PAIR_STREAM_FORMS(NVB_CASE)
#undef NVB_CASE
    }
    return hipErrorNotSupported;
}
template <typename CELL>
static hipError_t launch_pair(const GotohParams& p, hipStream_t s)
{
    if constexpr (CELL::COLUMN)
    {
        if (test_switch(SW_PAIR_ROW) != 1)
        {
            if (test_switch(SW_PAIR_CONST) != 1 && test_switch(SW_PAIR_SUB) != 1)
                switch (p.gap_ext) {
                case  0: return launch_pair_row<CELL, PF_ROW2 | PF_CONST2 | PF_SUBLDS>(p, s);
                case -1: return launch_pair_row<CELL, PF_ROW2 | PF_CONST2 | PF_SUBLDS | PF_GE1>(p, s);
                case -2: return launch_pair_row<CELL, PF_ROW2 | PF_CONST2 | PF_SUBLDS | PF_GE2>(p, s);
                case -3: return launch_pair_row<CELL, PF_ROW2 | PF_CONST2 | PF_SUBLDS | PF_GE3>(p, s);
                }
            if (test_switch(SW_PAIR_CONST) != 1)
                switch (p.gap_ext) {
                case  0: return launch_pair_row<CELL, PF_ROW2 | PF_CONST2>(p, s);
                case -1: return launch_pair_row<CELL, PF_ROW2 | PF_CONST2 | PF_GE1>(p, s);
                case -2: return launch_pair_row<CELL, PF_ROW2 | PF_CONST2 | PF_GE2>(p, s);
                case -3: return launch_pair_row<CELL, PF_ROW2 | PF_CONST2 | PF_GE3>(p, s);
                }
            return launch_pair_row<CELL, PF_ROW2>(p, s);
        }
    }
    return launch_pair_row<CELL, 0>(p, s);
}

static bool pair_max3_admitted(const GotohParams& p)
{
    if (test_switch(SW_BANDED_PAIR) == 2) return false;
    const int64_t per_row = int64_t(std::max(std::max(p.match, p.mismatch), 0)) - p.gap_ext;
    return int64_t(p.pat.fixed_length) * per_row <= PM3_ROW_LIMIT;
}

static bool pair_column_admitted(const GotohParams& p)
{
    if (test_switch(SW_BANDED_PAIR) == 3 || !pair_max3_admitted(p)) return false;
    const int64_t s_max = std::max(p.match, p.mismatch), G = -int64_t(p.gap_ext) * 32, D = (int64_t(p.gap_ext) - p.gap_open) * 32;
    if (s_max - p.gap_open - p.gap_ext > PD3_BYTE_LIMIT) return false;
    return pd3_top(D, G, p.pat.fixed_length, std::max<int64_t>(s_max, 0)) <= PD3_TOP;
}

}

template <typename QA>
static int banded_gotoh_dispatch(nvb::GotohParams& p, const QA& qa, int64_t max_abs_cost, int32_t best_pair, int32_t type, uint32_t band_len,
                                 const nvbio_hip_string_set* patterns, hipStream_t s, const char* tag16, const char* tag32, const bool views = false,
                                 const nvb::BoundArgs* bound = nullptr, const bool asym = false, const bool plain_entry = false)
{
    using namespace nvb;
    g_last_pair = PairLaunch();
    const bool rt = !asym && !bound;
    const uint32_t lim_plain = test_switch(SW_FORCE_32BIT) == 1 ? 0u
                             : max_len_16bit(p.match, best_pair, max_abs_cost, std::max(p.gap_open, p.txt_gap_open), std::max(p.gap_ext, p.txt_gap_ext), type, band_len, 0);
    const uint32_t lim16 = !rt ? lim_plain : test_switch(SW_FORCE_32BIT) == 1 ? 0u
                         : max_len_16bit(p.match, best_pair, max_abs_cost, std::max(p.gap_open, p.txt_gap_open), std::max(p.gap_ext, p.txt_gap_ext), type, band_len,
                                         p.gap_ext < 0 ? -p.gap_ext : 0);
    const uint32_t lim16p = (rt && type == NVBIO_HIP_LOCAL && lim_plain > lim16) ? lim_plain : lim16;
    const bool fixed = (patterns->length == nullptr);
    hipError_t e = hipSuccess;
    {
        const uint32_t maxM = fixed ? patterns->fixed_length : p.stage_pw ;
        p.stage_pw = p.stage_tw = 0;
        if (maxM != 0 && test_switch(SW_NO_STAGING) != 1) {
            uint32_t pw = stage_words_pattern(32u / patterns->bits - 1u, maxM, patterns->bits);
            if (views) {
                const uint32_t per = 32u / patterns->bits, c16 = (maxM + 15u) & ~15u;
                pw = std::max(pw, (per - 1u + c16 + 16u + per - 1u) / per + (patterns->bits == 4 ? 3u : 2u));
            }
            pw = (pw + 3u) & ~3u;
            const uint32_t tw = (stage_words_text(15u, maxM, band_len) + 3u) & ~3u;
            if ((pw + tw) * 1024u <= 32768u) { p.stage_pw = pw; p.stage_tw = tw; }
        }
    }
    auto go = [&](const bool width16) -> hipError_t {
        if (asym)   return launch_asym(p, type, band_len, width16, s);
        if (!bound) return launch<QA>(p, qa, type, band_len, width16, s);
        if (hipError_t z = hipMemsetAsync(bound->counter, 0, 4u, s)) return z;
        return launch_bounded<QA>(p, qa, *bound, type, band_len, width16, s);
    };
    p.plain16 = 0u;
    if (plain_entry && pair_admitted(p, type, band_len, lim16)) {
        g_last_kernel = g_last_pair.kernel = tag16;
        const bool max3 = pair_max3_admitted(p);
        const bool column = max3 && pair_column_admitted(p);
        g_last_pair.cell = max3 ? "max3" : "u16";
        g_last_pair.frame = column ? "column" : "row";
        return column ? launch_pair<PD3>(p, s) : max3 ? launch_pair<PM3>(p, s) : launch_pair<P16>(p, s);
    }
    if (lim16 > 0 && (!fixed || patterns->fixed_length <= lim16)) {
        p.len_lo = 0; p.len_hi = lim16;
        g_last_kernel = tag16;
        e = go(true);
        if (e != hipSuccess) return e;
    }
    if (lim16p > lim16 && (!fixed || (patterns->fixed_length > lim16 && patterns->fixed_length <= lim16p))) {
        p.len_lo = lim16 + 1u; p.len_hi = lim16p; p.plain16 = 1u;
        if (fixed) g_last_kernel = tag16;
        e = go(true);
        p.plain16 = 0u;
        if (e != hipSuccess) return e;
    }
    if (lim16p != 0xFFFFFFFFu && (!fixed || patterns->fixed_length > lim16p)) {
        p.len_lo = lim16p > 0 ? lim16p + 1 : 0; p.len_hi = 0xFFFFFFFFu;
        if (fixed || lim16p == 0) g_last_kernel = tag32;
        e = go(false);
    }
    return e;
}

static int check_banded_args(int32_t type, uint32_t band_len, const nvbio_hip_string_set* patterns, const nvbio_hip_string_set* texts)
{
    if (!patterns || !texts) return hipErrorInvalidValue;
    if (type < 0 || type > 2) return hipErrorInvalidValue;
    if (!(patterns->bits == 2 || patterns->bits == 4 || patterns->bits == 8) || texts->bits != 2) return hipErrorNotSupported;
    if (!(band_len == 3 || band_len == 5 || band_len == 7 || band_len == 15 || band_len == 31)) return hipErrorNotSupported;
    return hipSuccess;
}
static int check_banded_ptrs(const nvbio_hip_string_set* patterns, const nvbio_hip_string_set* texts, const int32_t* out_score, const uint32_t* out_sink)
{
    if (!out_score || !out_sink) return hipErrorInvalidValue;
    if (!patterns->words || !texts->words || !patterns->begin || !texts->begin ||
        patterns->n_words == 0 || texts->n_words == 0) return hipErrorInvalidValue;
    return hipSuccess;
}
static inline int64_t iabs64(int32_t v) { return v < 0 ? -int64_t(v) : int64_t(v); }

NVB_API int nvbio_hip_banded_gotoh_score(
    const nvbio_hip_gotoh_scheme* scheme, int32_t type, uint32_t band_len,
    const nvbio_hip_string_set* patterns, const nvbio_hip_string_set* texts,
    uint32_t max_pattern_len, uint32_t max_text_len,
    uint32_t n, int32_t* out_score, uint32_t* out_sink, void* stream)
{
    (void)max_text_len;
    using namespace nvb;
    if (!scheme) return hipErrorInvalidValue;
    if (int e = check_banded_args(type, band_len, patterns, texts)) return e;
    if (n == 0) return hipSuccess;
    if (int e = check_banded_ptrs(patterns, texts, out_score, out_sink)) return e;

    GotohParams p;
    p.pat = make_string_set(patterns);
    p.txt = make_string_set(texts);
    p.match = scheme->match; p.mismatch = scheme->mismatch;
    p.gap_open = scheme->gap_open; p.gap_ext = scheme->gap_ext;
    p.txt_gap_open = scheme->gap_open; p.txt_gap_ext = scheme->gap_ext;
    p.n = n; p.out_score = out_score; p.out_sink = out_sink; p.n_dev = nullptr; p.out_index = nullptr; p.gate = nullptr; p.gate_limit = 0;
    p.stage_pw = max_pattern_len; p.stage_tw = 0;
    const int64_t A = std::max(std::max(iabs64(scheme->match), iabs64(scheme->mismatch)), std::max(iabs64(scheme->gap_open), iabs64(scheme->gap_ext)));
    return banded_gotoh_dispatch(p, NoQual(), A, std::max(scheme->match, scheme->mismatch), type, band_len, patterns, to_stream(stream),
                                 "banded_gotoh_score_kernel<A16>", "banded_gotoh_score_kernel<A32>", false, nullptr, false, true);
}

NVB_API int nvbio_hip_banded_gotoh_score_qual(
    const nvbio_hip_gotoh_qual_scheme* scheme, int32_t type, uint32_t band_len,
    const nvbio_hip_string_set* patterns, const uint8_t* quals, uint64_t n_quals,
    const nvbio_hip_string_set* texts,
    uint32_t max_pattern_len, uint32_t max_text_len,
    uint32_t n, int32_t* out_score, uint32_t* out_sink, void* stream)
{
    return nvbio_hip_banded_gotoh_score_qual_views(scheme, type, band_len, patterns, quals, n_quals, nullptr, texts, max_pattern_len, max_text_len, n, out_score, out_sink, stream);
}

NVB_API int nvbio_hip_banded_gotoh_score_qual_views(
    const nvbio_hip_gotoh_qual_scheme* scheme, int32_t type, uint32_t band_len,
    const nvbio_hip_string_set* patterns, const uint8_t* quals, uint64_t n_quals, const uint8_t* pattern_flags,
    const nvbio_hip_string_set* texts,
    uint32_t max_pattern_len, uint32_t max_text_len,
    uint32_t n, int32_t* out_score, uint32_t* out_sink, void* stream)
{
    (void)max_text_len;
    using namespace nvb;
    if (!scheme) return hipErrorInvalidValue;
    if (int e = check_banded_args(type, band_len, patterns, texts)) return e;
    if (n == 0) return hipSuccess;
    if (int e = check_banded_ptrs(patterns, texts, out_score, out_sink)) return e;
    if (!quals || n_quals < 4) return hipErrorInvalidValue;
    if (pattern_flags && patterns->bits == 8u) return hipErrorNotSupported;

    GotohParams p;
    p.pat = make_string_set(patterns);
    p.txt = make_string_set(texts);
    p.match = scheme->match; p.mismatch = 0;
    p.gap_open = scheme->pattern_gap_open; p.gap_ext = scheme->pattern_gap_ext;
    p.txt_gap_open = scheme->text_gap_open; p.txt_gap_ext = scheme->text_gap_ext;
    p.n = n; p.out_score = out_score; p.out_sink = out_sink; p.n_dev = nullptr; p.out_index = nullptr; p.gate = nullptr; p.gate_limit = 0;
    p.stage_pw = max_pattern_len; p.stage_tw = 0;
    QualArgs qa;
    qa.quals = quals; qa.n_quals = n_quals; qa.flags = pattern_flags;
    int64_t A = std::max(std::max(iabs64(scheme->match), iabs64(scheme->pattern_gap_open)), std::max(iabs64(scheme->pattern_gap_ext),
                std::max(iabs64(scheme->text_gap_open), iabs64(scheme->text_gap_ext))));
    int32_t best_pair = scheme->match;
    for (int i = 0; i < 256; ++i) { qa.lut[i] = scheme->mismatch[i]; A = std::max(A, iabs64(scheme->mismatch[i])); best_pair = std::max(best_pair, scheme->mismatch[i]); }
    return banded_gotoh_dispatch(p, qa, A, best_pair, type, band_len, patterns, to_stream(stream),
                                 pattern_flags ? "banded_gotoh_score_kernel<A16,qual,views>" : "banded_gotoh_score_kernel<A16,qual>",
                                 pattern_flags ? "banded_gotoh_score_kernel<A32,qual,views>" : "banded_gotoh_score_kernel<A32,qual>", pattern_flags != nullptr);
}

NVB_API int nvbio_hip_banded_gotoh_score_qual_bounded(
    const nvbio_hip_gotoh_qual_scheme* scheme, int32_t type, uint32_t band_len,
    const nvbio_hip_string_set* patterns, const uint8_t* quals, uint64_t n_quals, const uint8_t* pattern_flags,
    const nvbio_hip_string_set* texts,
    uint32_t max_pattern_len, uint32_t max_text_len,
    uint32_t n, const uint32_t* n_on_device, const int32_t* min_score, uint32_t* work_counter, const uint32_t* out_index,
    const uint32_t* gate, uint32_t gate_limit,
    int32_t* out_score, uint32_t* out_sink, void* stream)
{
    (void)max_text_len;
    using namespace nvb;
    if (!scheme || (min_score && !work_counter) || (min_score && gate)) return hipErrorInvalidValue;
    if (int e = check_banded_args(type, band_len, patterns, texts)) return e;
    if (n == 0) return hipSuccess;
    if (int e = check_banded_ptrs(patterns, texts, out_score, out_sink)) return e;
    if (!quals || n_quals < 4) return hipErrorInvalidValue;
    if (pattern_flags && patterns->bits == 8u) return hipErrorNotSupported;

    GotohParams p;
    p.pat = make_string_set(patterns);
    p.txt = make_string_set(texts);
    p.match = scheme->match; p.mismatch = 0;
    p.gap_open = scheme->pattern_gap_open; p.gap_ext = scheme->pattern_gap_ext;
    p.txt_gap_open = scheme->text_gap_open; p.txt_gap_ext = scheme->text_gap_ext;
    p.n = n; p.out_score = out_score; p.out_sink = out_sink; p.n_dev = nullptr; p.out_index = nullptr; p.gate = nullptr; p.gate_limit = 0;
    p.stage_pw = max_pattern_len; p.stage_tw = 0;
    QualArgs qa;
    qa.quals = quals; qa.n_quals = n_quals; qa.flags = pattern_flags;
    int64_t A = std::max(std::max(iabs64(scheme->match), iabs64(scheme->pattern_gap_open)), std::max(iabs64(scheme->pattern_gap_ext),
                std::max(iabs64(scheme->text_gap_open), iabs64(scheme->text_gap_ext))));
    int32_t best_pair = scheme->match;
    for (int i = 0; i < 256; ++i) { qa.lut[i] = scheme->mismatch[i]; A = std::max(A, iabs64(scheme->mismatch[i])); best_pair = std::max(best_pair, scheme->mismatch[i]); }
    if (!min_score)
    {
        p.n_dev = n_on_device; p.out_index = out_index; p.gate = gate; p.gate_limit = gate_limit;
        return banded_gotoh_dispatch(p, qa, A, best_pair, type, band_len, patterns, to_stream(stream),
                                     pattern_flags ? "banded_gotoh_score_kernel<A16,qual,views>" : "banded_gotoh_score_kernel<A16,qual>",
                                     pattern_flags ? "banded_gotoh_score_kernel<A32,qual,views>" : "banded_gotoh_score_kernel<A32,qual>", pattern_flags != nullptr);
    }
    BoundArgs ba;
    const bool gaps_ok = scheme->pattern_gap_open <= 0 && scheme->pattern_gap_ext <= 0;
    ba.min_score = gaps_ok ? min_score : nullptr;
    ba.n_dev = n_on_device; ba.counter = work_counter; ba.out_index = out_index;
    ba.cap = std::max(best_pair, 0);
    static const int refill = [] { const char* e = getenv("NVBIO_HIP_BOUNDED_REFILL"); return std::min(64, std::max(1, e ? atoi(e) : 16)); }();
    ba.refill = uint32_t(refill);
    return banded_gotoh_dispatch(p, qa, A, best_pair, type, band_len, patterns, to_stream(stream),
                                 "banded_gotoh_score_bounded_kernel<A16,qual>", "banded_gotoh_score_bounded_kernel<A32,qual>", pattern_flags != nullptr, &ba);
}

NVB_API int nvbio_hip_banded_sw_score(
    const nvbio_hip_sw_scheme* scheme, int32_t type, uint32_t band_len,
    const nvbio_hip_string_set* patterns, const nvbio_hip_string_set* texts,
    uint32_t max_pattern_len, uint32_t max_text_len,
    uint32_t n, int32_t* out_score, uint32_t* out_sink, void* stream)
{
    if (!scheme) return hipErrorInvalidValue;
    if (scheme->deletion == scheme->insertion)
    {
        const nvbio_hip_gotoh_scheme g = { scheme->match, scheme->mismatch, scheme->deletion, scheme->deletion };
        return nvbio_hip_banded_gotoh_score(&g, type, band_len, patterns, texts, max_pattern_len, max_text_len, n, out_score, out_sink, stream);
    }
    (void)max_text_len;
    using namespace nvb;
    if (int e = check_banded_args(type, band_len, patterns, texts)) return e;
    if (n == 0) return hipSuccess;
    if (int e = check_banded_ptrs(patterns, texts, out_score, out_sink)) return e;
    GotohParams p;
    p.pat = make_string_set(patterns);
    p.txt = make_string_set(texts);
    p.match = scheme->match; p.mismatch = scheme->mismatch;
    p.gap_open = p.gap_ext = scheme->insertion;
    p.f_gap_open = p.f_gap_ext = scheme->deletion;
    p.txt_gap_open = p.txt_gap_ext = scheme->deletion;
    p.n = n; p.out_score = out_score; p.out_sink = out_sink; p.n_dev = nullptr; p.out_index = nullptr; p.gate = nullptr; p.gate_limit = 0;
    p.stage_pw = max_pattern_len; p.stage_tw = 0;
    const int64_t A = std::max(std::max(iabs64(scheme->match), iabs64(scheme->mismatch)), std::max(iabs64(scheme->deletion), iabs64(scheme->insertion)));
    return banded_gotoh_dispatch(p, NoQual(), A, std::max(scheme->match, scheme->mismatch), type, band_len, patterns, to_stream(stream),
                                 "banded_gotoh_score_kernel<A16X>", "banded_gotoh_score_kernel<A32X>", false, nullptr, true);
}

namespace nvb {
static std::mutex g_streams_mtx;
static std::vector<hipStream_t> g_streams[64];
static void register_stream(int dev, hipStream_t s) { if (dev >= 0 && dev < 64) { std::lock_guard<std::mutex> lock(g_streams_mtx); g_streams[dev].push_back(s); } }
static void forget_stream(hipStream_t s)
{
    std::lock_guard<std::mutex> lock(g_streams_mtx);
    for (auto& v : g_streams) v.erase(std::remove(v.begin(), v.end(), s), v.end());
}

struct CachedBlock { void* ptr; uint64_t bytes; uint64_t stamp; };
struct BlockCache
{
    std::mutex mtx;
    std::vector<CachedBlock> idle;
    std::unordered_map<void*, uint64_t> live;
    uint64_t idle_bytes = 0, clock = 0;
};
static BlockCache g_cache[64];
static int env_int(const char* name, int dflt) { const char* e = getenv(name); return e ? atoi(e) : dflt; }
static uint64_t cache_keep_bytes() { static const uint64_t keep = uint64_t(std::max(0, env_int("NVBIO_HIP_POOL_KEEP_MB", 2048))) << 20; return keep; }
static hipMemPool_t rocm_pool(int dev)
{
    static std::mutex mtx;
    static hipMemPool_t pools[64] = {};
    static bool tried[64] = {};
    static const bool use = env_int("NVBIO_HIP_ROCM_POOL", 0) == 1;
    if (!use || dev < 0 || dev >= 64) return nullptr;
    std::lock_guard<std::mutex> lock(mtx);
    if (!tried[dev]) {
        tried[dev] = true;
        hipMemPoolProps props = {};
        props.allocType = hipMemAllocationTypePinned;
        props.handleTypes = hipMemHandleTypeNone;
        props.location.type = hipMemLocationTypeDevice;
        props.location.id = dev;
        hipMemPool_t pool = nullptr;
        if (hipMemPoolCreate(&pool, &props) == hipSuccess) {
            uint64_t keep = uint64_t(256) << 20;
            (void)hipMemPoolSetAttribute(pool, hipMemPoolAttrReleaseThreshold, &keep);
            pools[dev] = pool;
        } else (void)hipGetLastError();
    }
    return pools[dev];
}
static void drop_idle(BlockCache& c, std::vector<void*>& victims, uint64_t keep)
{
    while (c.idle_bytes > keep && !c.idle.empty())
    {
        size_t k = 0;
        for (size_t j = 1; j < c.idle.size(); ++j) if (c.idle[j].stamp < c.idle[k].stamp) k = j;
        victims.push_back(c.idle[k].ptr);
        c.idle_bytes -= c.idle[k].bytes;
        c.idle[k] = c.idle.back(); c.idle.pop_back();
    }
}
}
NVB_API int nvbio_hip_device_malloc(void** ptr, uint64_t bytes)
{
    if (!ptr) return hipErrorInvalidValue;
    int dev = 0;
    if (hipError_t e = hipGetDevice(&dev)) return e;
    if (dev < 0 || dev >= 64) return hipMalloc(ptr, bytes ? bytes : 1);
    if (hipMemPool_t pool = nvb::rocm_pool(dev))
    {
        if (hipError_t e = hipMallocFromPoolAsync(ptr, bytes ? bytes : 1, pool, nullptr)) return e;
        return hipStreamSynchronize(nullptr);
    }
    const uint64_t n = ((bytes ? bytes : 1) + 511ull) & ~511ull;
    nvb::BlockCache& c = nvb::g_cache[dev];
    void* p = nullptr;
    {
        std::lock_guard<std::mutex> lock(c.mtx);
        size_t best = c.idle.size();
        for (size_t k = 0; k < c.idle.size(); ++k)
            if (c.idle[k].bytes >= n && c.idle[k].bytes <= 2u * n && (best == c.idle.size() || c.idle[k].bytes < c.idle[best].bytes)) best = k;
        if (best != c.idle.size())
        {
            p = c.idle[best].ptr;
            c.live[p] = c.idle[best].bytes;
            c.idle_bytes -= c.idle[best].bytes;
            c.idle[best] = c.idle.back(); c.idle.pop_back();
        }
    }
    if (!p)
    {
        hipError_t e = hipMalloc(&p, n);
        if (e != hipSuccess)
        {
            (void)hipGetLastError();
            std::vector<void*> victims;
            { std::lock_guard<std::mutex> lock(c.mtx); nvb::drop_idle(c, victims, 0); }
            for (void* v : victims) (void)hipFree(v);
            e = hipMalloc(&p, n);
            if (e != hipSuccess) return e;
        }
        std::lock_guard<std::mutex> lock(c.mtx);
        c.live[p] = n;
    }
    *ptr = p;
    static const int poison = nvb::env_int("NVBIO_HIP_POISON_ALLOC", -1);
    if (poison >= 0) (void)hipMemsetAsync(p, poison & 255, bytes ? bytes : 1, nullptr);
    return hipStreamSynchronize(nullptr);
}
static int free_impl(void* ptr, bool ordered, hipStream_t extra = nullptr)
{
    if (!ptr) return hipSuccess;
    int dev = 0;
    static const bool sync_free = nvb::env_int("NVBIO_HIP_SYNC_FREE", 0) == 1;
    const bool have_dev = hipGetDevice(&dev) == hipSuccess && dev >= 0 && dev < 64;
    if (!have_dev) { if (hipError_t e = hipDeviceSynchronize()) return e; return hipFree(ptr); }
    if (sync_free || !ordered) { if (hipError_t e = hipDeviceSynchronize()) return e; }
    else
    {
        std::lock_guard<std::mutex> lock(nvb::g_streams_mtx);
        std::vector<hipStream_t> behind(nvb::g_streams[dev]);
        if (extra && std::find(behind.begin(), behind.end(), extra) == behind.end()) behind.push_back(extra);
        for (hipStream_t s : behind)
        {
            hipEvent_t ev = nullptr;
            hipError_t e = hipEventCreateWithFlags(&ev, hipEventDisableTiming);
            if (e == hipSuccess) e = hipEventRecord(ev, s);
            if (e == hipSuccess) e = hipStreamWaitEvent(nullptr, ev, 0);
            if (ev) (void)hipEventDestroy(ev);
            if (e != hipSuccess)
            {
                (void)hipGetLastError();
                if (hipError_t es = hipDeviceSynchronize()) return es;
                break;
            }
        }
    }
    if (nvb::rocm_pool(dev)) return hipFreeAsync(ptr, nullptr);
    nvb::BlockCache& c = nvb::g_cache[dev];
    std::vector<void*> victims;
    {
        std::lock_guard<std::mutex> lock(c.mtx);
        auto it = c.live.find(ptr);
        if (it == c.live.end()) victims.push_back(ptr);
        else
        {
            c.idle.push_back(nvb::CachedBlock{ ptr, it->second, ++c.clock });
            c.idle_bytes += it->second;
            c.live.erase(it);
            nvb::drop_idle(c, victims, nvb::cache_keep_bytes());
        }
    }
    hipError_t r = hipSuccess;
    for (void* v : victims) { const hipError_t e = hipFree(v); if (e != hipSuccess) r = e; }
    return r;
}
NVB_API int nvbio_hip_device_free(void* ptr)         { return free_impl(ptr, false); }
NVB_API int nvbio_hip_device_free_ordered(void* ptr) { return free_impl(ptr, true); }
NVB_API int nvbio_hip_device_free_after(void* ptr, void* stream) { return free_impl(ptr, true, nvb::to_stream(stream)); }
NVB_API int nvbio_hip_device_trim(void)
{
    int dev = 0;
    if (hipError_t e = hipGetDevice(&dev)) return e;
    if (dev < 0 || dev >= 64) return hipSuccess;
    std::vector<void*> victims;
    { std::lock_guard<std::mutex> lock(nvb::g_cache[dev].mtx); nvb::drop_idle(nvb::g_cache[dev], victims, 0); }
    hipError_t r = hipSuccess;
    for (void* v : victims) { const hipError_t e = hipFree(v); if (e != hipSuccess) r = e; }
    return r;
}
NVB_API int nvbio_hip_device_mem_info(uint64_t* free_bytes, uint64_t* total_bytes, uint64_t* idle_cached_bytes)
{
    size_t f = 0, t = 0;
    if (hipError_t e = hipMemGetInfo(&f, &t)) return e;
    int dev = 0;
    uint64_t idle = 0;
    if (hipGetDevice(&dev) == hipSuccess && dev >= 0 && dev < 64) { std::lock_guard<std::mutex> lock(nvb::g_cache[dev].mtx); idle = nvb::g_cache[dev].idle_bytes; }
    if (free_bytes) *free_bytes = f;
    if (total_bytes) *total_bytes = t;
    if (idle_cached_bytes) *idle_cached_bytes = idle;
    return hipSuccess;
}
namespace nvb {
uint32_t seeding_grid(uint64_t n_items) { return uint32_t((n_items + 255u) / 256u); }
}
NVB_API int nvbio_hip_stream_create(void** stream, uint32_t non_blocking)
{
    if (!stream) return hipErrorInvalidValue;
    hipStream_t s = nullptr;
    const hipError_t e = hipStreamCreateWithFlags(&s, non_blocking ? hipStreamNonBlocking : hipStreamDefault);
    *stream = s;
    int dev = 0;
    if (e == hipSuccess && hipGetDevice(&dev) == hipSuccess) nvb::register_stream(dev, s);
    return e;
}
NVB_API int nvbio_hip_stream_destroy(void* stream)
{
    if (!stream) return hipSuccess;
    nvb::forget_stream(nvb::to_stream(stream));
    return hipStreamDestroy(nvb::to_stream(stream));
}

namespace nvb {
static std::atomic<int> g_switch[SW_COUNT];
static const char* const g_switch_name[SW_COUNT] = { "NVBIO_HIP_FORCE_32BIT", "NVBIO_HIP_NO_STAGING", "NVBIO_HIP_FULL_GENERIC", "NVBIO_HIP_ED_SWEEP",
                                                     "NVBIO_HIP_FULL_SINGLE_JOB", "NVBIO_HIP_FULL_ROWS", "NVBIO_HIP_TRACEBACK_LANES", "NVBIO_HIP_SELECT_LANES",
                                                     "NVBIO_HIP_BANDED_PAIR", "NVBIO_HIP_PAIR_ROW", "NVBIO_HIP_PAIR_CONST", "NVBIO_HIP_PAIR_SUB" };
static void seed_switches()
{
    static std::once_flag once;
    std::call_once(once, [] { for (int k = 0; k < SW_COUNT; ++k) { const char* e = getenv(g_switch_name[k]); g_switch[k].store(e ? atoi(e) : 0, std::memory_order_relaxed); } });
}
int test_switch(TestSwitch which) { seed_switches(); return g_switch[which].load(std::memory_order_relaxed); }
}
NVB_API int nvbio_hip_set_test_switch(const char* name, int value)
{
    if (!name) return hipErrorInvalidValue;
    nvb::seed_switches();
    for (int k = 0; k < nvb::SW_COUNT; ++k)
        if (strcmp(name, nvb::g_switch_name[k]) == 0) { nvb::g_switch[k].store(value, std::memory_order_relaxed); return hipSuccess; }
    return hipErrorInvalidValue;
}
NVB_API const char* nvbio_hip_test_switch_name(int index) { return (index >= 0 && index < nvb::SW_COUNT) ? nvb::g_switch_name[index] : nullptr; }
NVB_API int nvbio_hip_get_test_switch(const char* name)
{
    if (!name) return -1;
    for (int k = 0; k < nvb::SW_COUNT; ++k) if (strcmp(name, nvb::g_switch_name[k]) == 0) return nvb::test_switch(nvb::TestSwitch(k));
    return -1;
}

NVB_API int nvbio_hip_memcpy(void* dst, const void* src, uint64_t bytes, int kind, void* stream)
{
    const hipMemcpyKind k = kind == 1 ? hipMemcpyHostToDevice : kind == 2 ? hipMemcpyDeviceToHost : hipMemcpyDeviceToDevice;
    if (bytes == 0) return hipSuccess;
    hipError_t e = hipMemcpyAsync(dst, src, bytes, k, nvb::to_stream(stream));
    if (e != hipSuccess) return e;
    return kind == 2 ? hipStreamSynchronize(nvb::to_stream(stream)) : hipSuccess;
}
NVB_API int nvbio_hip_memset(void* dst, int value, uint64_t bytes, void* stream) { return bytes ? hipMemsetAsync(dst, value, bytes, nvb::to_stream(stream)) : hipSuccess; }
NVB_API int nvbio_hip_stream_synchronize(void* stream) { return hipStreamSynchronize(nvb::to_stream(stream)); }
NVB_API int nvbio_hip_stream_query(void* stream)
{
    const hipError_t e = hipStreamQuery(nvb::to_stream(stream));
    if (e == hipErrorNotReady) (void)hipGetLastError();
    return e;
}
NVB_API int nvbio_hip_host_malloc(void** ptr, uint64_t bytes)
{
    if (!ptr) return hipErrorInvalidValue;
    *ptr = nullptr;
    return hipHostMalloc(ptr, bytes ? bytes : 1u, hipHostMallocDefault);
}
NVB_API int nvbio_hip_host_free(void* ptr) { return ptr ? hipHostFree(ptr) : hipSuccess; }

NVB_API int         nvbio_hip_abi_version(void) { return NVBIO_HIP_ABI_VERSION; }
NVB_API const char* nvbio_hip_arch(void)        { return "gfx950"; }
NVB_API const char* nvbio_hip_last_kernel(void) { return nvb::g_last_kernel; }
static const char* pair_fact(const char* fact) { return (nvb::g_last_pair.kernel && nvb::g_last_pair.kernel == nvb::g_last_kernel) ? fact : ""; }
NVB_API const char* nvbio_hip_last_kernel_detail(void) { return pair_fact("pair"); }
NVB_API const char* nvbio_hip_last_kernel_fetch(void)  { return pair_fact(nvb::g_last_pair.fetch); }
NVB_API const char* nvbio_hip_last_kernel_frame(void)  { return pair_fact(nvb::g_last_pair.frame); }
NVB_API const char* nvbio_hip_last_kernel_row(void)    { return pair_fact(nvb::g_last_pair.row); }
NVB_API const char* nvbio_hip_last_kernel_const(void)  { return pair_fact(nvb::g_last_pair.consts); }
NVB_API const char* nvbio_hip_last_kernel_sub(void)    { return pair_fact(nvb::g_last_pair.sub); }
NVB_API const char* nvbio_hip_last_kernel_cell(void)   { return pair_fact(nvb::g_last_pair.cell); }
```

nvbio_amd/csrc/banded_gotoh_pair.h:

```cpp
#pragma once
#include "banded_gotoh_impl.h"

namespace nvb {

template <int BAND>
struct PairState {
    uint32_t S[BAND];
    uint32_t F[BAND - 1];
    uint32_t tc[16];
    uint32_t z;
    uint32_t best[2], besti[2];
};

enum PairForm : int {
    PF_SINK_VCC = 0, PF_SINK_KEY = 1,
    PF_STREAM   = 4,
    PF_PAT2     = 2,
    PF_PBE      = 8, PF_TBE = 256,
    PF_KO_SINK  = 16, PF_KO_TABLE = 32, PF_KO_FETCH = 64, PF_KO_BOUND = 128,
    PF_FOLD2    = 1024,
    PF_CONST2   = 16384 | 131072,
    PF_GE1      = 32768, PF_GE2 = 65536, PF_GE3 = PF_GE1 | PF_GE2,
    PF_SUBLDS   = 262144,
    PF_KO_PERM  = 524288
};
constexpr int pair_ge(int form)     { return (form / PF_GE1) & 3; }
constexpr int pair_ge_bits(int ge)  { return ge * PF_GE1; }
constexpr int PF_ROW2 = PF_FOLD2;
#define NVB_PAIR_STREAM_FORMS_(Y, A) \
    Y(A, PF_STREAM) Y(A, PF_STREAM | PF_PBE) Y(A, PF_STREAM | PF_TBE) Y(A, PF_STREAM | PF_PBE | PF_TBE) \
    Y(A, PF_STREAM | PF_PAT2) Y(A, PF_STREAM | PF_PAT2 | PF_PBE) Y(A, PF_STREAM | PF_PAT2 | PF_TBE) Y(A, PF_STREAM | PF_PAT2 | PF_PBE | PF_TBE)
#define NVB_PAIR_APPLY_(X, F) X(F)
#define NVB_PAIR_STREAM_FORMS(X) NVB_PAIR_STREAM_FORMS_(NVB_PAIR_APPLY_, X)
#define NVB_PAIR_CELLS_(X, F) X(P16, (F)) X(PM3, (F)) X(PD3, (F)) X(PD3, (F) | PF_ROW2)
#define NVB_PAIR_GES_(X, F)   X(PD3, (F) | PF_ROW2 | PF_CONST2) X(PD3, (F) | PF_ROW2 | PF_CONST2 | PF_GE1) X(PD3, (F) | PF_ROW2 | PF_CONST2 | PF_GE2) X(PD3, (F) | PF_ROW2 | PF_CONST2 | PF_GE3)
#define NVB_PAIR_INSTANCES_B15(X)     NVB_PAIR_CELLS_(X, PF_SINK_VCC) NVB_PAIR_STREAM_FORMS_(NVB_PAIR_CELLS_, X)
#define NVB_PAIR_INSTANCES_B15_LIT(X) NVB_PAIR_GES_(X, PF_SINK_VCC) NVB_PAIR_STREAM_FORMS_(NVB_PAIR_GES_, X)
#define NVB_PAIR_SUBS_(X, F)  NVB_PAIR_GES_(X, (F) | PF_SUBLDS)
#define NVB_PAIR_INSTANCES_B15_SUB(X) NVB_PAIR_SUBS_(X, PF_SINK_VCC) NVB_PAIR_STREAM_FORMS_(NVB_PAIR_SUBS_, X)
#define NVB_PAIR_INSTANCES(X)         NVB_PAIR_INSTANCES_B15(X) NVB_PAIR_INSTANCES_B15_LIT(X) NVB_PAIR_INSTANCES_B15_SUB(X)

__host__ __device__ constexpr uint32_t sub_index(uint32_t ca, uint32_t cb) { return (ca & 3u) | (cb << 2) | ((ca >> 2) << 6); }
__host__ __device__ constexpr uint32_t sub_code_a(uint32_t index)          { return (index & 3u) | ((index >> 6) << 2); }
__host__ __device__ constexpr uint32_t sub_code_b(uint32_t index)          { return (index >> 2) & 15u; }
__device__ __forceinline__ uint32_t sub_bfi(uint32_t mask, uint32_t a, uint32_t b) { return (a & mask) | (b & ~mask); }
__device__ __forceinline__ void sub_row_words(const uint64_t PA, const uint64_t PB, uint64_t& RE, uint64_t& RO)
{
    uint32_t re[2], ro[2];
    #pragma unroll
    for (int h = 0; h < 2; ++h)
    {
        const uint32_t a = uint32_t(PA >> (32 * h)), b = uint32_t(PB >> (32 * h));
        re[h] = sub_bfi(0x03030303u, a,      sub_bfi(0x3C3C3C3Cu, b << 2, a << 4));
        ro[h] = sub_bfi(0x03030303u, a >> 4, sub_bfi(0x3C3C3C3Cu, b >> 2, a));
    }
    RE = re[0] | uint64_t(re[1]) << 32; RO = ro[0] | uint64_t(ro[1]) << 32;
}

struct PairOps {
    static constexpr bool COLUMN = false;
    static __device__ __forceinline__ uint32_t rep(int32_t c)               { return (uint32_t(c) & 0xFFFFu) * 0x10001u; }
    static __device__ __forceinline__ uint32_t mx(uint32_t a, uint32_t b)   { uint32_t r; asm("v_pk_max_u16 %0, %1, %2" : "=v"(r) : "v"(a), "v"(b)); return r; }
    static constexpr uint32_t SEL_BASE = 0x0C040C00u;
    static __device__ __forceinline__ uint32_t subst(uint32_t tlo, uint32_t thi, uint32_t sel) { return __builtin_amdgcn_perm(thi, tlo, sel); }

    template <int FORM, int BAND>
    static __device__ __forceinline__ void sink(PairState<BAND>& st, uint32_t rowkey, const uint32_t i) { fold<FORM>(st, rowkey - st.z, i); }
    template <int FORM, int BAND>
    static __device__ __forceinline__ void fold(PairState<BAND>& st, const uint32_t rowkey, const uint32_t i)
    {
        if (FORM & PF_KO_SINK) { st.best[0] = mx(st.best[0], rowkey); return; }
        if (FORM & PF_SINK_KEY)
        {
            const uint32_t frame = (31u << 15) | (i << 5);
            uint32_t a, b, wa, wb;
            asm("v_and_b32 %[a], 0xffff, %[rk]\n\t"
                "v_lshrrev_b32 %[b], 16, %[rk]\n\t"
                "v_lshl_or_b32 %[wa], %[a], 15, %[fr]\n\t"
                "v_lshl_or_b32 %[wb], %[b], 15, %[fr]\n\t"
                "v_and_or_b32 %[wa], %[a], 31, %[wa]\n\t"
                "v_and_or_b32 %[wb], %[b], 31, %[wb]\n\t"
                "v_max_u32 %[ba], %[ba], %[wa]\n\t"
                "v_max_u32 %[bb], %[bb], %[wb]"
                : [a] "=&v"(a), [b] "=&v"(b), [wa] "=&v"(wa), [wb] "=&v"(wb), [ba] "+&v"(st.best[0]), [bb] "+&v"(st.best[1])
                : [rk] "v"(rowkey), [fr] "s"(frame));
            return;
        }
        const uint32_t rk[2] = { rowkey & 0xFFFFu, rowkey >> 16 };
        #pragma unroll
        for (int h = 0; h < 2; ++h)
        {
            const bool upd = (rk[h] | 31u) >= st.best[h];
            st.best[h]  = upd ? rk[h] : st.best[h];
            st.besti[h] = upd ? i : st.besti[h];
        }
    }
};

struct P16 : PairOps {
    static constexpr int32_t FLOOR = 0;

    template <int J, bool EDGE>
    static __device__ __forceinline__ void cell(uint32_t& Fj, const uint32_t Fnext, const uint32_t Snext, uint32_t& Sj, uint32_t& E, uint32_t& rowkey,
                                                const uint32_t g, const uint32_t D, const uint32_t G, const uint32_t tlo, const uint32_t thi, const uint32_t Z)
    {
        uint32_t d, h;
        if (EDGE)
            asm("v_perm_b32 %[d], %[thi], %[tlo], %[g]\n\t"
                "v_mov_b32 %[f], %[sn]\n\t"
                "v_add_u32 %[d], %[s], %[d]\n\t"
                "v_pk_max_u16 %[h], %[sn], %[z]\n\t"
                "v_pk_max_u16 %[h], %[h], %[d]\n\t"
                "v_pk_max_u16 %[h], %[h], %[e]\n\t"
                "v_sub_u32 %[s], %[h], %[dd]\n\t"
                "v_add_u32 %[d], %[sj], %[h]\n\t"
                "v_pk_max_u16 %[e], %[e], %[s]\n\t"
                "v_sub_u32 %[e], %[e], %[gg]\n\t"
                "v_pk_max_u16 %[rk], %[rk], %[d]"
                : [f] "=&v"(Fj), [d] "=&v"(d), [h] "=&v"(h), [s] "+v"(Sj), [e] "+v"(E), [rk] "+v"(rowkey)
                : [g] "v"(g), [tlo] "v"(tlo), [thi] "v"(thi), [sn] "v"(Snext), [dd] "v"(D), [gg] "v"(G), [z] "v"(Z), [sj] "n"(J * 0x10001));
        else
            asm("v_perm_b32 %[d], %[thi], %[tlo], %[g]\n\t"
                "v_pk_max_u16 %[f], %[fn], %[sn]\n\t"
                "v_add_u32 %[d], %[s], %[d]\n\t"
                "v_pk_max_u16 %[h], %[f], %[z]\n\t"
                "v_pk_max_u16 %[h], %[h], %[d]\n\t"
                "v_pk_max_u16 %[h], %[h], %[e]\n\t"
                "v_sub_u32 %[s], %[h], %[dd]\n\t"
                "v_add_u32 %[d], %[sj], %[h]\n\t"
                "v_pk_max_u16 %[e], %[e], %[s]\n\t"
                "v_sub_u32 %[e], %[e], %[gg]\n\t"
                "v_pk_max_u16 %[rk], %[rk], %[d]"
                : [f] "=&v"(Fj), [d] "=&v"(d), [h] "=&v"(h), [s] "+v"(Sj), [e] "+v"(E), [rk] "+v"(rowkey)
                : [g] "v"(g), [tlo] "v"(tlo), [thi] "v"(thi), [fn] "v"(Fnext), [sn] "v"(Snext), [dd] "v"(D), [gg] "v"(G), [z] "v"(Z), [sj] "n"(J * 0x10001));
    }

    template <int BAND, int R, int J, int END>
    struct Cells {
        static __device__ __forceinline__ void run(PairState<BAND>& st, uint32_t& E, uint32_t& rowkey, const uint32_t D, const uint32_t G, const uint32_t tlo, const uint32_t thi)
        {
            cell<J, J + 1 == BAND - 1>(st.F[J], st.F[J + 1 < BAND - 1 ? J + 1 : 0], st.S[J + 1], st.S[J], E, rowkey, st.tc[(R + J) & 15], D, G, tlo, thi, st.z);
            Cells<BAND, R, J + 1, END>::run(st, E, rowkey, D, G, tlo, thi);
        }
    };
    template <int BAND, int R, int END>
    struct Cells<BAND, R, END, END> {
        static __device__ __forceinline__ void run(PairState<BAND>&, uint32_t&, uint32_t&, uint32_t, uint32_t, uint32_t, uint32_t) {}
    };

    template <int BAND, int R, int FORM>
    static __device__ __forceinline__ void row(PairState<BAND>& st, const uint32_t i, const uint32_t D, const uint32_t G, const uint32_t g_new, const uint32_t tlo, const uint32_t thi)
    {
        st.z += G;
        st.F[0] = (1 == BAND - 1) ? st.S[1] : mx(st.F[1 < BAND - 1 ? 1 : 0], st.S[1]);
        uint32_t hi = mx(mx(st.F[0], st.S[0] + subst(tlo, thi, st.tc[R & 15])), st.z);
        uint32_t rowkey = hi;
        st.S[0] = hi - D;
        uint32_t E = st.S[0] - G;
        Cells<BAND, R, 1, BAND - 1>::run(st, E, rowkey, D, G, tlo, thi);
        st.tc[(R + BAND - 1) & 15] = g_new;
        hi = mx(mx(E, st.S[BAND - 1] + subst(tlo, thi, g_new)), st.z);
        rowkey = mx(rowkey, hi + uint32_t(BAND - 1) * 0x10001u);
        st.S[BAND - 1] = hi - D;
        sink<FORM>(st, rowkey, i);
    }
};

constexpr int32_t PM3_ROW_LIMIT = (0x7BFF - 255 - 0x0400 - 448) / 32;
struct PM3 : PairOps {
    static constexpr int32_t FLOOR = 0x0400;
    static __device__ __forceinline__ uint32_t mx3(uint32_t a, uint32_t b, uint32_t c) { uint32_t r; asm("v_pk_maximum3_f16 %0, %1, %2, %3" : "=v"(r) : "v"(a), "v"(b), "v"(c)); return r; }

    template <int J>
    static __device__ __forceinline__ void cell2(uint32_t& F0, uint32_t& F1, const uint32_t F2, uint32_t& S0, uint32_t& S1, const uint32_t S2, uint32_t& E, uint32_t& rowkey,
                                                 const uint32_t g0, const uint32_t g1, const uint32_t D, const uint32_t G, const uint32_t tlo, const uint32_t thi, const uint32_t Z)
    {
        uint32_t d0, d1, h;
        asm("v_perm_b32 %[d0], %[thi], %[tlo], %[g0]\n\t"
            "v_perm_b32 %[d1], %[thi], %[tlo], %[g1]\n\t"
            "v_pk_maximum3_f16 %[f0], %[f1], %[s1], %[z]\n\t"
            "v_pk_maximum3_f16 %[f1], %[f2], %[s2], %[z]\n\t"
            "v_add_u32 %[d0], %[s0], %[d0]\n\t"
            "v_add_u32 %[d1], %[s1], %[d1]\n\t"
            "v_pk_maximum3_f16 %[h], %[f0], %[d0], %[e]\n\t"
            "v_sub_u32 %[s0], %[h], %[dd]\n\t"
            "v_add_u32 %[d0], %[j0], %[h]\n\t"
            "v_pk_max_u16 %[e], %[e], %[s0]\n\t"
            "v_sub_u32 %[e], %[e], %[gg]\n\t"
            "v_pk_maximum3_f16 %[h], %[f1], %[d1], %[e]\n\t"
            "v_sub_u32 %[s1], %[h], %[dd]\n\t"
            "v_add_u32 %[d1], %[j1], %[h]\n\t"
            "v_pk_max_u16 %[e], %[e], %[s1]\n\t"
            "v_sub_u32 %[e], %[e], %[gg]\n\t"
            "v_pk_maximum3_f16 %[rk], %[rk], %[d0], %[d1]"
            : [f0] "=&v"(F0), [f1] "+&v"(F1), [d0] "=&v"(d0), [d1] "=&v"(d1), [h] "=&v"(h), [s0] "+&v"(S0), [s1] "+&v"(S1), [e] "+&v"(E), [rk] "+&v"(rowkey)
            : [g0] "v"(g0), [g1] "v"(g1), [tlo] "v"(tlo), [thi] "v"(thi), [f2] "v"(F2), [s2] "v"(S2), [dd] "v"(D), [gg] "v"(G), [z] "v"(Z),
              [j0] "n"(J * 0x10001), [j1] "n"((J + 1) * 0x10001));
    }

    template <int J>
    static __device__ __forceinline__ void tail2(uint32_t& F0, uint32_t& S0, uint32_t& S1, uint32_t& E, uint32_t& rowkey,
                                                 const uint32_t g0, const uint32_t g1, const uint32_t D, const uint32_t G, const uint32_t tlo, const uint32_t thi, const uint32_t Z)
    {
        uint32_t d0, d1, h;
        asm("v_perm_b32 %[d0], %[thi], %[tlo], %[g0]\n\t"
            "v_perm_b32 %[d1], %[thi], %[tlo], %[g1]\n\t"
            "v_pk_max_u16 %[f0], %[s1], %[z]\n\t"
            "v_add_u32 %[d0], %[s0], %[d0]\n\t"
            "v_add_u32 %[d1], %[s1], %[d1]\n\t"
            "v_pk_maximum3_f16 %[h], %[f0], %[d0], %[e]\n\t"
            "v_sub_u32 %[s0], %[h], %[dd]\n\t"
            "v_add_u32 %[d0], %[j0], %[h]\n\t"
            "v_pk_max_u16 %[e], %[e], %[s0]\n\t"
            "v_sub_u32 %[e], %[e], %[gg]\n\t"
            "v_pk_maximum3_f16 %[h], %[e], %[d1], %[z]\n\t"
            "v_sub_u32 %[s1], %[h], %[dd]\n\t"
            "v_add_u32 %[d1], %[j1], %[h]\n\t"
            "v_pk_maximum3_f16 %[rk], %[rk], %[d0], %[d1]"
            : [f0] "=&v"(F0), [d0] "=&v"(d0), [d1] "=&v"(d1), [h] "=&v"(h), [s0] "+&v"(S0), [s1] "+&v"(S1), [e] "+&v"(E), [rk] "+&v"(rowkey)
            : [g0] "v"(g0), [g1] "v"(g1), [tlo] "v"(tlo), [thi] "v"(thi), [dd] "v"(D), [gg] "v"(G), [z] "v"(Z),
              [j0] "n"(J * 0x10001), [j1] "n"((J + 1) * 0x10001));
    }

    template <int BAND, int R, int J, int END>
    struct Cells {
        static __device__ __forceinline__ void run(PairState<BAND>& st, uint32_t& E, uint32_t& rowkey, const uint32_t D, const uint32_t G, const uint32_t tlo, const uint32_t thi)
        {
            cell2<J>(st.F[J], st.F[J + 1], st.F[J + 2], st.S[J], st.S[J + 1], st.S[J + 2], E, rowkey, st.tc[(R + J) & 15], st.tc[(R + J + 1) & 15], D, G, tlo, thi, st.z);
            Cells<BAND, R, J + 2, END>::run(st, E, rowkey, D, G, tlo, thi);
        }
    };
    template <int BAND, int R, int END>
    struct Cells<BAND, R, END, END> {
        static __device__ __forceinline__ void run(PairState<BAND>&, uint32_t&, uint32_t&, uint32_t, uint32_t, uint32_t, uint32_t) {}
    };

    template <int BAND, int R, int FORM>
    static __device__ __forceinline__ void row(PairState<BAND>& st, const uint32_t i, const uint32_t D, const uint32_t G, const uint32_t g_new, const uint32_t tlo, const uint32_t thi)
    {
        static_assert(BAND % 2 == 1, "columns 1 ... BAND-3 go two at a time");
        st.z += G;
        st.F[0] = (1 == BAND - 1) ? mx(st.S[1], st.z) : mx3(st.F[1 < BAND - 1 ? 1 : 0], st.S[1], st.z);
        const uint32_t hi = mx(st.F[0], st.S[0] + subst(tlo, thi, st.tc[R & 15]));
        uint32_t rowkey = hi;
        st.S[0] = hi - D;
        uint32_t E = st.S[0] - G;
        Cells<BAND, R, 1, BAND - 2>::run(st, E, rowkey, D, G, tlo, thi);
        st.tc[(R + BAND - 1) & 15] = g_new;
        tail2<BAND - 2>(st.F[BAND - 2], st.S[BAND - 2], st.S[BAND - 1], E, rowkey, st.tc[(R + BAND - 2) & 15], g_new, D, G, tlo, thi, st.z);
        sink<FORM>(st, rowkey, i);
    }
};

constexpr int32_t PD3_TOP = 0x7BFF, PD3_BYTE_LIMIT = 7;
constexpr int64_t pd3_top(int64_t D, int64_t G, int64_t M, int64_t s_plus, int64_t band = 15)
{
    return 0x0400 + D + G + G * (2 * M + band - 1) + 32 * M * s_plus + 255;
}
template <int BAND>
struct ColumnFrame {
    uint32_t z[16];
    uint32_t k[BAND];
    uint32_t D, step;
    uint32_t pair;
};
struct PD3 : PairOps {
    static constexpr bool COLUMN = true;
    static constexpr int32_t FLOOR = 0x0400;

    template <int FORM> static constexpr int32_t klit(int j)     { return int32_t(uint32_t(j + (14 - j) * 32 * pair_ge(FORM)) * 0x10001u); }
    template <int FORM> static constexpr int32_t pairlit()       { return int32_t(uint32_t(2 * 32 * pair_ge(FORM)) * 0x10001u); }

#define NVB_PD3_PERM1 "v_perm_b32 %[d], %[thi], %[tlo], %[g0]\n\t"
#define NVB_PD3_PERM2 "v_perm_b32 %[d0], %[thi], %[tlo], %[g0]\n\t" "v_perm_b32 %[d1], %[thi], %[tlo], %[g1]\n\t"
#define NVB_PD3_XOR1  "v_xor_b32 %[d], %[tlo], %[g0]\n\t"
#define NVB_PD3_XOR2  "v_xor_b32 %[d0], %[tlo], %[g0]\n\t" "v_xor_b32 %[d1], %[tlo], %[g1]\n\t"
#define NVB_PD3_COL0(L) L \
            "v_pk_maximum3_f16 %[f0], %[f1], %[s1], %[z0]\n\t" \
            "v_add_u32 %[d], %[s0], %[d]\n\t" \
            "v_pk_max_u16 %[h], %[f0], %[d]\n\t" \
            "v_subrev_u32 %[s0], %[dd], %[h]\n\t" \
            "v_add_u32 %[rk], %[k0], %[h]"
#define NVB_PD3_COL0_OUT [f0] "=&v"(F0), [d] "=&v"(d), [h] "=&v"(h), [s0] "+&v"(S0), [rk] "=&v"(rowkey)
#define NVB_PD3_COL0_IN  [g0] "v"(g0), [tlo] "v"(tlo), [thi] "v"(thi), [f1] "v"(F1), [s1] "v"(S1), [z0] "s"(Z0)
    template <int FORM>
    static __device__ __forceinline__ void col0(uint32_t& F0, const uint32_t F1, uint32_t& S0, const uint32_t S1, uint32_t& rowkey,
                                                const uint32_t g0, const uint32_t D, const uint32_t tlo, const uint32_t thi, const uint32_t Z0, const uint32_t K0)
    {
        uint32_t d = g0, h;
        if constexpr ((FORM & PF_SUBLDS) != 0)      asm(NVB_PD3_COL0("") : [f0] "=&v"(F0), [d] "+&v"(d), [h] "=&v"(h), [s0] "+&v"(S0), [rk] "=&v"(rowkey)
                                                                         : [f1] "v"(F1), [s1] "v"(S1), [z0] "s"(Z0), [dd] "v"(D), [k0] "n"(klit<FORM>(0)));
        else if constexpr ((FORM & PF_KO_PERM) != 0) asm(NVB_PD3_COL0(NVB_PD3_XOR1) : NVB_PD3_COL0_OUT : NVB_PD3_COL0_IN, [dd] "v"(D), [k0] "n"(klit<FORM>(0)));
        else if constexpr ((FORM & PF_CONST2) != 0) asm(NVB_PD3_COL0(NVB_PD3_PERM1) : NVB_PD3_COL0_OUT : NVB_PD3_COL0_IN, [dd] "v"(D), [k0] "n"(klit<FORM>(0)));
        else                                        asm(NVB_PD3_COL0(NVB_PD3_PERM1) : NVB_PD3_COL0_OUT : NVB_PD3_COL0_IN, [dd] "s"(D), [k0] "s"(K0));
    }

#define NVB_PD3_CELL2(L, P) L \
            "v_pk_maximum3_f16 %[f0], %[f1], %[s1], %[z0]\n\t" \
            "v_pk_maximum3_f16 %[f1], %[f2], %[s2], %[z1]\n\t" \
            "v_add_u32 %[d0], %[s0], %[d0]\n\t" \
            "v_add_u32 %[d1], %[s1], %[d1]\n\t" P \
            "v_pk_maximum3_f16 %[h], %[f0], %[d0], %[ei]\n\t" \
            "v_subrev_u32 %[s0], %[dd], %[h]\n\t" \
            "v_add_u32 %[d0], %[k0], %[h]\n\t" P \
            "v_pk_max_u16 %[e], %[ei], %[s0]\n\t" \
            "v_pk_maximum3_f16 %[h], %[f1], %[d1], %[e]\n\t" \
            "v_subrev_u32 %[s1], %[dd], %[h]\n\t" \
            "v_add_u32 %[d1], %[k1], %[h]\n\t" P \
            "v_pk_max_u16 %[e], %[e], %[s1]\n\t" \
            "v_pk_maximum3_f16 %[rk], %[rk], %[d0], %[d1]"
#define NVB_PD3_CELL2_OUT [f0] "=&v"(F0), [f1] "+&v"(F1), [d0] "=&v"(d0), [d1] "=&v"(d1), [h] "=&v"(h), [s0] "+&v"(S0), [s1] "+&v"(S1), [e] "=&v"(E), [rk] "+&v"(rowkey)
#define NVB_PD3_CELL2_IN  [g0] "v"(g0), [g1] "v"(g1), [tlo] "v"(tlo), [thi] "v"(thi), [f2] "v"(F2), [s2] "v"(S2), [ei] "v"(Ein), [z0] "s"(Z0), [z1] "s"(Z1)
    template <int FORM, int J>
    static __device__ __forceinline__ void cell2(uint32_t& F0, uint32_t& F1, const uint32_t F2, uint32_t& S0, uint32_t& S1, const uint32_t S2, const uint32_t Ein, uint32_t& E,
                                                 uint32_t& rowkey, const uint32_t g0, const uint32_t g1, const uint32_t D, const uint32_t tlo, const uint32_t thi,
                                                 const uint32_t Z0, const uint32_t Z1, const uint32_t K0, const uint32_t K1)
    {
        uint32_t d0 = g0, d1 = g1, h;
        if constexpr ((FORM & PF_SUBLDS) != 0)
            asm(NVB_PD3_CELL2("", "s_nop 0\n\t")
                : [f0] "=&v"(F0), [f1] "+&v"(F1), [d0] "+&v"(d0), [d1] "+&v"(d1), [h] "=&v"(h), [s0] "+&v"(S0), [s1] "+&v"(S1), [e] "=&v"(E), [rk] "+&v"(rowkey)
                : [f2] "v"(F2), [s2] "v"(S2), [ei] "v"(Ein), [z0] "s"(Z0), [z1] "s"(Z1), [dd] "v"(D), [k0] "n"(klit<FORM>(J)), [k1] "n"(klit<FORM>(J + 1)));
        else if constexpr ((FORM & PF_KO_PERM) != 0) asm(NVB_PD3_CELL2(NVB_PD3_XOR2, "s_nop 0\n\t") : NVB_PD3_CELL2_OUT : NVB_PD3_CELL2_IN, [dd] "v"(D), [k0] "n"(klit<FORM>(J)), [k1] "n"(klit<FORM>(J + 1)));
        else if constexpr ((FORM & PF_CONST2) != 0) asm(NVB_PD3_CELL2(NVB_PD3_PERM2, "s_nop 0\n\t") : NVB_PD3_CELL2_OUT : NVB_PD3_CELL2_IN, [dd] "v"(D), [k0] "n"(klit<FORM>(J)), [k1] "n"(klit<FORM>(J + 1)));
        else                                        asm(NVB_PD3_CELL2(NVB_PD3_PERM2, "") : NVB_PD3_CELL2_OUT : NVB_PD3_CELL2_IN, [dd] "s"(D), [k0] "s"(K0), [k1] "s"(K1));
    }

#define NVB_PD3_TAIL2(L) L \
            "v_pk_max_u16 %[f0], %[s1], %[z0]\n\t" \
            "v_add_u32 %[d0], %[s0], %[d0]\n\t" \
            "v_add_u32 %[d1], %[s1], %[d1]\n\t" \
            "v_pk_maximum3_f16 %[h], %[f0], %[d0], %[ei]\n\t" \
            "v_subrev_u32 %[s0], %[dd], %[h]\n\t" \
            "v_add_u32 %[d0], %[k0], %[h]\n\t" \
            "v_pk_max_u16 %[e], %[ei], %[s0]\n\t" \
            "v_pk_maximum3_f16 %[h], %[e], %[d1], %[z1]\n\t" \
            "v_subrev_u32 %[s1], %[dd], %[h]\n\t" \
            "v_add_u32 %[d1], %[k1], %[h]\n\t" \
            "v_pk_maximum3_f16 %[rk], %[rk], %[d0], %[d1]"
#define NVB_PD3_TAIL2_OUT [f0] "=&v"(F0), [d0] "=&v"(d0), [d1] "=&v"(d1), [h] "=&v"(h), [e] "=&v"(e), [s0] "+&v"(S0), [s1] "+&v"(S1), [rk] "+&v"(rowkey)
#define NVB_PD3_TAIL2_IN  [g0] "v"(g0), [g1] "v"(g1), [tlo] "v"(tlo), [thi] "v"(thi), [ei] "v"(Ein), [z0] "s"(Z0), [z1] "s"(Z1)
    template <int FORM, int J>
    static __device__ __forceinline__ void tail2(uint32_t& F0, uint32_t& S0, uint32_t& S1, const uint32_t Ein, uint32_t& rowkey,
                                                 const uint32_t g0, const uint32_t g1, const uint32_t D, const uint32_t tlo, const uint32_t thi,
                                                 const uint32_t Z0, const uint32_t Z1, const uint32_t K0, const uint32_t K1)
    {
        uint32_t d0 = g0, d1 = g1, h, e;
        if constexpr ((FORM & PF_SUBLDS) != 0)
            asm(NVB_PD3_TAIL2("")
                : [f0] "=&v"(F0), [d0] "+&v"(d0), [d1] "+&v"(d1), [h] "=&v"(h), [e] "=&v"(e), [s0] "+&v"(S0), [s1] "+&v"(S1), [rk] "+&v"(rowkey)
                : [ei] "v"(Ein), [z0] "s"(Z0), [z1] "s"(Z1), [dd] "v"(D), [k0] "n"(klit<FORM>(J)), [k1] "n"(klit<FORM>(J + 1)));
        else if constexpr ((FORM & PF_KO_PERM) != 0) asm(NVB_PD3_TAIL2(NVB_PD3_XOR2) : NVB_PD3_TAIL2_OUT : NVB_PD3_TAIL2_IN, [dd] "v"(D), [k0] "n"(klit<FORM>(J)), [k1] "n"(klit<FORM>(J + 1)));
        else if constexpr ((FORM & PF_CONST2) != 0) asm(NVB_PD3_TAIL2(NVB_PD3_PERM2) : NVB_PD3_TAIL2_OUT : NVB_PD3_TAIL2_IN, [dd] "v"(D), [k0] "n"(klit<FORM>(J)), [k1] "n"(klit<FORM>(J + 1)));
        else                                        asm(NVB_PD3_TAIL2(NVB_PD3_PERM2) : NVB_PD3_TAIL2_OUT : NVB_PD3_TAIL2_IN, [dd] "s"(D), [k0] "s"(K0), [k1] "s"(K1));
    }

    template <int BAND, int R, int FORM, int J, int END>
    struct Cells {
        static __device__ __forceinline__ void run(PairState<BAND>& st, const ColumnFrame<BAND>& fr, const uint32_t Ein, uint32_t& E, uint32_t& rowkey, const uint32_t tlo, const uint32_t thi)
        {
            uint32_t En;
            cell2<FORM, J>(st.F[J], st.F[J + 1], st.F[J + 2], st.S[J], st.S[J + 1], st.S[J + 2], Ein, En, rowkey, st.tc[(R + J) & 15], st.tc[(R + J + 1) & 15], fr.D, tlo, thi,
                           fr.z[(2 * R + J) & 15], fr.z[(2 * R + J + 1) & 15], fr.k[J], fr.k[J + 1]);
            Cells<BAND, R, FORM, J + 2, END>::run(st, fr, En, E, rowkey, tlo, thi);
        }
    };
    template <int BAND, int R, int FORM, int END>
    struct Cells<BAND, R, FORM, END, END> {
        static __device__ __forceinline__ void run(PairState<BAND>&, const ColumnFrame<BAND>&, const uint32_t Ein, uint32_t& E, uint32_t&, uint32_t, uint32_t) { E = Ein; }
    };

    template <int BAND, int R, int FORM, int J, int END>
    struct SubCells {
        static __device__ __forceinline__ void run(PairState<BAND>& st, const ColumnFrame<BAND>& fr, const uint32_t Ein, uint32_t& E, uint32_t& rowkey, const uint32_t (&w)[BAND])
        {
            uint32_t En;
            cell2<FORM, J>(st.F[J], st.F[J + 1], st.F[J + 2], st.S[J], st.S[J + 1], st.S[J + 2], Ein, En, rowkey, w[J], w[J + 1], fr.D, 0u, 0u,
                           fr.z[(2 * R + J) & 15], fr.z[(2 * R + J + 1) & 15], fr.k[J], fr.k[J + 1]);
            SubCells<BAND, R, FORM, J + 2, END>::run(st, fr, En, E, rowkey, w);
        }
    };
    template <int BAND, int R, int FORM, int END>
    struct SubCells<BAND, R, FORM, END, END> {
        static __device__ __forceinline__ void run(PairState<BAND>&, const ColumnFrame<BAND>&, const uint32_t Ein, uint32_t& E, uint32_t&, const uint32_t (&)[BAND]) { E = Ein; }
    };

    template <int BAND>
    static __device__ __forceinline__ void open(ColumnFrame<BAND>& fr, const int32_t d32, const int32_t g32)
    {
        #pragma unroll
        for (int s = 0; s < 16; ++s) fr.z[s] = rep(d32 + g32 + FLOOR + g32 * (2 + (s <= BAND - 3 ? s : s - 16)));
        #pragma unroll
        for (int j = 0; j < BAND; ++j) fr.k[j] = rep(j + (BAND - 1 - j) * g32);
        fr.D = rep(d32);
        fr.step = rep(16 * g32);
        fr.pair = rep(2 * g32);
    }

    template <int BAND, int R, int FORM>
    static __device__ __forceinline__ void row(PairState<BAND>& st, ColumnFrame<BAND>& fr, const uint32_t i, const uint32_t g_new, const uint32_t tlo, const uint32_t thi, uint32_t& rk2,
                                               const uint32_t* sub = nullptr)
    {
        static_assert(BAND == 15, "a row's zeros, 2 i ... 2 i + BAND - 1, and the two the next row adds fill the ring of 16; columns go two at a time");
        fr.z[(2 * R + BAND - 2) & 15] += fr.step;
        fr.z[(2 * R + BAND - 1) & 15] += fr.step;
        uint32_t rowkey, E;
        if constexpr ((FORM & PF_SUBLDS) != 0)
        {
            constexpr int HEAD = 8, SPLIT = 5;
            st.tc[(R + BAND - 1) & 15] = g_new;
            uint32_t w[BAND], Em;
            #pragma unroll
            for (int j = 0; j < HEAD; ++j) w[j] = *reinterpret_cast<const uint32_t*>(reinterpret_cast<const char*>(sub) + (tlo ^ st.tc[(R + j) & 15]));
            col0<FORM>(st.F[0], st.F[1], st.S[0], st.S[1], rowkey, w[0], fr.D, 0u, 0u, fr.z[(2 * R) & 15], fr.k[0]);
            SubCells<BAND, R, FORM, 1, SPLIT>::run(st, fr, st.S[0], Em, rowkey, w);
            #pragma unroll
            for (int j = HEAD; j < BAND; ++j) w[j] = *reinterpret_cast<const uint32_t*>(reinterpret_cast<const char*>(sub) + (tlo ^ st.tc[(R + j) & 15]));
            SubCells<BAND, R, FORM, SPLIT, BAND - 2>::run(st, fr, Em, E, rowkey, w);
            tail2<FORM, BAND - 2>(st.F[BAND - 2], st.S[BAND - 2], st.S[BAND - 1], E, rowkey, w[BAND - 2], w[BAND - 1], fr.D, 0u, 0u,
                                  fr.z[(2 * R + BAND - 2) & 15], fr.z[(2 * R + BAND - 1) & 15], fr.k[BAND - 2], fr.k[BAND - 1]);
        }
        else
        {
            col0<FORM>(st.F[0], st.F[1], st.S[0], st.S[1], rowkey, st.tc[R & 15], fr.D, tlo, thi, fr.z[(2 * R) & 15], fr.k[0]);
            Cells<BAND, R, FORM, 1, BAND - 2>::run(st, fr, st.S[0], E, rowkey, tlo, thi);
            st.tc[(R + BAND - 1) & 15] = g_new;
            tail2<FORM, BAND - 2>(st.F[BAND - 2], st.S[BAND - 2], st.S[BAND - 1], E, rowkey, st.tc[(R + BAND - 2) & 15], g_new, fr.D, tlo, thi,
                                  fr.z[(2 * R + BAND - 2) & 15], fr.z[(2 * R + BAND - 1) & 15], fr.k[BAND - 2], fr.k[BAND - 1]);
        }
        if constexpr ((FORM & PF_FOLD2) != 0)
        {
            if constexpr ((R & 1) == 0) rk2 = rowkey;
            else fold<FORM>(st, mx(rk2 + ((FORM & PF_CONST2) ? uint32_t(pairlit<FORM>()) : fr.pair), rowkey + rep(16)) - fr.z[(2 * R + BAND - 1) & 15], i - 1u);
        }
        else fold<FORM>(st, rowkey - fr.z[(2 * R + BAND - 1) & 15], i);
    }

    template <int BAND, int FORM>
    static __device__ __forceinline__ void fold_last(PairState<BAND>& st, const uint32_t rk2, const uint32_t M, const int32_t d32, const int32_t g32)
    {
        fold<FORM>(st, rk2 - rep(d32 + g32 + FLOOR + g32 * int32_t(2u * M + BAND - 1)), M - 1u);
    }
};

template <typename CELL, int BAND, int FORM, int R, int END>
struct PairRows {
    static __device__ __forceinline__ void run(PairState<BAND>& st, ColumnFrame<BAND>& fr, const uint32_t i0, const uint32_t M, const uint32_t D, const uint32_t G,
                                               const uint64_t PA, const uint64_t PB, const uint32_t (&XT)[2], const uint32_t* tab, const uint32_t (&KT)[2], uint32_t& rk2)
    {
        if ((FORM & PF_KO_BOUND) || i0 + R < M)
        {
            if constexpr ((FORM & PF_SUBLDS) != 0)
            {
                constexpr int K = R >> 1;
                const uint32_t zw = uint32_t(((R & 1) ? PB : PA) >> (32 * (K >> 2))), xw = XT[R & 1];
                uint32_t rw = (K & 3) == 0 ? (zw << 2) & 0x3FCu : (zw >> (8 * (K & 3) - 2)) & 0x3FCu;
                uint32_t cw = K == 0 ? (xw << 2) & 0x3Cu : (xw >> (4 * K - 2)) & 0x3Cu;
                asm("" : "+v"(rw)); asm("" : "+v"(cw));
                CELL::template row<BAND, R, FORM>(st, fr, i0 + R, cw, rw, 0u, rk2, tab);
            }
            else if constexpr (CELL::COLUMN)
            {
                const uint32_t g = ((XT[R >> 3] >> (2 * (R & 7))) & 0x00030003u) | CELL::SEL_BASE;
                if (FORM & PF_KO_TABLE) CELL::template row<BAND, R, FORM>(st, fr, i0 + R, g, KT[0], KT[1], rk2);
                else                    CELL::template row<BAND, R, FORM>(st, fr, i0 + R, g, tab[uint32_t(PA >> (4 * R)) & 15u], tab[uint32_t(PB >> (4 * R)) & 15u], rk2);
            }
            else
            {
                const uint32_t g = ((XT[R >> 3] >> (2 * (R & 7))) & 0x00030003u) | CELL::SEL_BASE;
                if (FORM & PF_KO_TABLE) CELL::template row<BAND, R, FORM>(st, i0 + R, D, G, g, KT[0], KT[1]);
                else                    CELL::template row<BAND, R, FORM>(st, i0 + R, D, G, g, tab[uint32_t(PA >> (4 * R)) & 15u], tab[uint32_t(PB >> (4 * R)) & 15u]);
            }
        }
        PairRows<CELL, BAND, FORM, R + 1, END>::run(st, fr, i0, M, D, G, PA, PB, XT, tab, KT, rk2);
    }
};
template <typename CELL, int BAND, int FORM, int END> struct PairRows<CELL, BAND, FORM, END, END> {
    static __device__ __forceinline__ void run(PairState<BAND>&, ColumnFrame<BAND>&, uint32_t, uint32_t, uint32_t, uint32_t, uint64_t, uint64_t, const uint32_t (&)[2], const uint32_t*, const uint32_t (&)[2], uint32_t&) {}
};

constexpr int PAIR_LANES = 128;
template <int BAND, typename CELL, int FORM>
__global__ void __launch_bounds__(PAIR_LANES) __attribute__((amdgpu_waves_per_eu((FORM & PF_SUBLDS) ? 5 : 1)))
banded_gotoh_pair_kernel(const GotohParams p)
{
    static_assert(BAND >= 3 && BAND <= 16, "the ring of 16");
    constexpr bool STREAM = (FORM & PF_STREAM) != 0, KEY = (FORM & PF_SINK_KEY) != 0, FOLD2 = (FORM & PF_FOLD2) != 0, SUBLDS = (FORM & PF_SUBLDS) != 0;
    static_assert(!(FORM & (PF_SUBLDS | PF_KO_PERM)) || ((FORM & PF_FOLD2) && (FORM & PF_CONST2) == PF_CONST2), "the LDS words and the probe's xor row are forms of the library's row");
    static_assert(!SUBLDS || !(FORM & (PF_KO_TABLE | PF_KO_PERM)), "the LDS words have no lookup to knock out");
    static_assert(!(FORM & (PF_FOLD2 | PF_CONST2)) || CELL::COLUMN, "the pair fold and the literals are the column frame's");
    static_assert(!FOLD2 || !(FORM & (PF_SINK_KEY | PF_KO_SINK | PF_KO_BOUND)), "the pair fold is the compare-and-select fold's, over the job's own rows");
    static_assert(!(FORM & PF_GE3) || (FORM & PF_CONST2), "|G_e| is the literal form's parameter");
    constexpr bool P4 = !(FORM & PF_PAT2), PBE = (FORM & PF_PBE) != 0, TBE = (FORM & PF_TBE) != 0;
    __shared__ uint32_t s_tab[16];
    __shared__ uint32_t s_sub[256];
    if constexpr (SUBLDS)
    {
        const uint32_t tg = uint32_t(-p.gap_ext * 32);
        const uint32_t sm = uint32_t((p.match - p.gap_open) * 32) + tg, sx = uint32_t((p.mismatch - p.gap_open) * 32) + tg;
        for (uint32_t k = threadIdx.x; k < 256u; k += uint32_t(PAIR_LANES))
            s_sub[k] = (sub_code_a(k) == 0u ? sm : sx) | ((sub_code_b(k) == 0u ? sm : sx) << 16);
    }
    else if (threadIdx.x < 16u)
    {
        const uint32_t tg = CELL::COLUMN ? uint32_t(-p.gap_ext * 32) : 0u;
        const uint32_t sm = uint32_t((p.match - p.gap_open) * 32) + tg, sx = uint32_t((p.mismatch - p.gap_open) * 32) + tg;
        uint32_t t = sx * 0x01010101u;
        if (threadIdx.x < 4u) t = (t & ~(0xFFu << (8u * threadIdx.x))) | (sm << (8u * threadIdx.x));
        s_tab[threadIdx.x] = t;
    }
    __syncthreads();
    const uint32_t lane = blockIdx.x * uint32_t(PAIR_LANES) + threadIdx.x;
    if (lane >= p.n / 2u + (p.n & 1u)) return;
    const uint32_t id[2] = { 2u * lane, 2u * lane + 1u < p.n ? 2u * lane + 1u : 2u * lane };
    const uint32_t M = (FORM & PF_KO_BOUND) ? 96u : p.pat.fixed_length;
    const Stream ps[2] = { p.pat.s, p.pat.s }, ts[2] = { p.txt.s, p.txt.s };
    const uint64_t pb[2] = { p.pat.begin[id[0]], p.pat.begin[id[1]] }, tb[2] = { p.txt.begin[id[0]], p.txt.begin[id[1]] };

    const int32_t d32 = (p.gap_ext - p.gap_open) * 32, g32 = -p.gap_ext * 32;
    uint32_t D = CELL::rep(d32), G = CELL::rep(g32);
    if (!CELL::COLUMN) { asm("" : "+v"(D)); asm("" : "+v"(G)); }
    uint32_t KT[2] = { 0u, 0u };
    if (FORM & PF_KO_TABLE) { KT[0] = s_tab[threadIdx.x & 3u]; KT[1] = s_tab[(threadIdx.x >> 2) & 3u]; asm("" : "+v"(KT[0])); asm("" : "+v"(KT[1])); }

    PairState<BAND> st;
    #pragma unroll
    for (int j = 0; j < BAND; ++j) st.S[j] = CELL::rep(g32 + CELL::FLOOR + (CELL::COLUMN ? g32 * j : 0));
    #pragma unroll
    for (int j = 0; j < BAND - 1; ++j) st.F[j] = CELL::rep(CELL::FLOOR);
    st.z = CELL::rep(d32 + g32 + CELL::FLOOR);
    ColumnFrame<BAND> fr;
    if constexpr (CELL::COLUMN) CELL::open(fr, d32, g32);
    if constexpr ((FORM & PF_CONST2) != 0) asm("" : "+v"(fr.D));
    st.best[0] = st.best[1] = 0u; st.besti[0] = st.besti[1] = 0u;
    uint32_t rk2 = 0u;
    {
        const uint32_t TA = fetch16_2bit(ts[0], tb[0]), TB = fetch16_2bit(ts[1], tb[1]);
        #pragma unroll
        for (int j = 0; j < BAND - 1; ++j)
            st.tc[j] = SUBLDS ? (((TA >> (2 * j)) & 3u) | (((TB >> (2 * j)) & 3u) << 2)) << 2
                              : CELL::SEL_BASE | ((TA >> (2 * j)) & 3u) | (((TB >> (2 * j)) & 3u) << 16);
    }

    const uint32_t plast = stream_last_off(p.pat.s), tlast = stream_last_off(p.txt.s);
    GroupStream gp[2], gt[2];
    uint64_t PA, PB;
    uint32_t TA, TB;
    if (STREAM)
    {
        if (P4) { PA = stream_open_4bit<PBE>(ps[0], plast, pb[0], gp[0]); PB = stream_open_4bit<PBE>(ps[1], plast, pb[1], gp[1]); }
        else    { PA = expand_2to4(stream_open_2bit<PBE>(ps[0], plast, pb[0], gp[0])); PB = expand_2to4(stream_open_2bit<PBE>(ps[1], plast, pb[1], gp[1])); }
        TA = stream_open_2bit<TBE>(ts[0], tlast, tb[0] + BAND - 1, gt[0]); TB = stream_open_2bit<TBE>(ts[1], tlast, tb[1] + BAND - 1, gt[1]);
    }
    else
    {
        PA = fetch_pattern16(ps[0], pb[0]); PB = fetch_pattern16(ps[1], pb[1]);
        TA = fetch16_2bit(ts[0], tb[0] + BAND - 1); TB = fetch16_2bit(ts[1], tb[1] + BAND - 1);
    }
    for (uint32_t i0 = 0; i0 < M; i0 += 16u)
    {
        uint64_t PAn = 0, PBn = 0;
        uint32_t TAn = 0, TBn = 0;
        uint2 rp[2] = { make_uint2(0u, 0u), make_uint2(0u, 0u) };
        uint32_t rt[2] = { 0u, 0u };
        if (FORM & PF_KO_FETCH) {}
        else if (STREAM)
        {
            if (P4) { rp[0] = stream_load_4bit(ps[0], plast, gp[0]); rp[1] = stream_load_4bit(ps[1], plast, gp[1]); }
            else    { rp[0].x = stream_load_2bit(ps[0], plast, gp[0]); rp[1].x = stream_load_2bit(ps[1], plast, gp[1]); }
            rt[0] = stream_load_2bit(ts[0], tlast, gt[0]); rt[1] = stream_load_2bit(ts[1], tlast, gt[1]);
        }
        else
        {
            PAn = fetch_pattern16(ps[0], pb[0] + i0 + 16u); PBn = fetch_pattern16(ps[1], pb[1] + i0 + 16u);
            TAn = fetch16_2bit(ts[0], tb[0] + i0 + 16u + BAND - 1); TBn = fetch16_2bit(ts[1], tb[1] + i0 + 16u + BAND - 1);
        }
        if constexpr (SUBLDS)
        {
            uint64_t RE, RO;
            sub_row_words(PA, PB, RE, RO);
            const uint32_t XT[2] = { sub_bfi(0x33333333u, TA, TB << 2), sub_bfi(0x33333333u, TA >> 2, TB) };
            PairRows<CELL, BAND, FORM, 0, 16>::run(st, fr, i0, M, D, G, RE, RO, XT, s_sub, KT, rk2);
        }
        else
        {
            const uint32_t XT[2] = { (TA & 0xFFFFu) | (TB << 16), (TA >> 16) | (TB & 0xFFFF0000u) };
            PairRows<CELL, BAND, FORM, 0, 16>::run(st, fr, i0, M, D, G, PA, PB, XT, s_tab, KT, rk2);
        }
        if (FORM & PF_KO_FETCH)
        {
            PA = (PA << 4) | (PA >> 60); PB = (PB << 8) | (PB >> 56);
            TA = funnel(TA, TA, 2u); TB = funnel(TB, TB, 6u);
        }
        else if (STREAM)
        {
            if (P4) { PA = stream_group_4bit<PBE>(gp[0], rp[0]); PB = stream_group_4bit<PBE>(gp[1], rp[1]); }
            else    { PA = expand_2to4(stream_group_2bit<PBE>(gp[0], rp[0].x)); PB = expand_2to4(stream_group_2bit<PBE>(gp[1], rp[1].x)); }
            TA = stream_group_2bit<TBE>(gt[0], rt[0]); TB = stream_group_2bit<TBE>(gt[1], rt[1]);
        }
        else { PA = PAn; PB = PBn; TA = TAn; TB = TBn; }
    }

    if constexpr (FOLD2) { if (M & 1u) CELL::template fold_last<BAND, FORM>(st, rk2, M, d32, g32); }
    #pragma unroll
    for (int h = 0; h < 2; ++h)
    {
        if (h == 1 && id[1] == id[0]) break;
        const uint32_t j = st.best[h] & (FOLD2 ? 15u : 31u), i = KEY ? (st.best[h] >> 5) & 1023u : st.besti[h] + (FOLD2 ? (st.best[h] >> 4) & 1u : 0u);
        p.out_score[id[h]] = int32_t(st.best[h] >> (KEY ? 20 : 5));
        reinterpret_cast<uint2*>(p.out_sink)[id[h]] = make_uint2(i + j + 1u, i + 1u);
    }
}

template <int BAND, typename CELL, int FORM>
hipError_t launch_band_pair(const GotohParams& p, hipStream_t stream)
{
    const uint32_t n_lanes = p.n / 2u + (p.n & 1u);
    hipLaunchKernelGGL((banded_gotoh_pair_kernel<BAND, CELL, FORM>), dim3((n_lanes + PAIR_LANES - 1u) / PAIR_LANES), dim3(PAIR_LANES), 0, stream, p);
    return hipGetLastError();
}

#ifdef NVB_PAIR_EXTERN
#define NVB_DECL(CELL, F) extern template hipError_t launch_band_pair<15, CELL, (F)>(const GotohParams&, hipStream_t);
NVB_PAIR_INSTANCES(NVB_DECL)
#undef NVB_DECL
#endif

}
```

nvbio_amd/csrc/common.h:

```cpp
#pragma once
#include <hip/hip_runtime.h>
#include <stdint.h>
#include "../../include/nvbio_hip.h"

#define NVB_API extern "C" __attribute__((visibility("default")))

namespace nvb {

extern thread_local const char* g_last_kernel;
struct PairLaunch {
    const char* kernel = nullptr;
    const char* cell   = "";
    const char* fetch  = "";
    const char* frame  = "";
    const char* row    = "";
    const char* consts = "";
    const char* sub    = "";
};
extern thread_local PairLaunch g_last_pair;

enum TestSwitch { SW_FORCE_32BIT = 0, SW_NO_STAGING, SW_FULL_GENERIC, SW_ED_SWEEP, SW_FULL_SINGLE_JOB, SW_FULL_ROWS, SW_TRACEBACK_LANES, SW_SELECT_LANES, SW_BANDED_PAIR, SW_PAIR_ROW, SW_PAIR_CONST, SW_PAIR_SUB, SW_COUNT };
int test_switch(TestSwitch which);


__device__ __forceinline__ uint32_t rev2(uint32_t x)
{
    x = __brev(x);
    return ((x & 0xAAAAAAAAu) >> 1) | ((x & 0x55555555u) << 1);
}
__device__ __forceinline__ uint32_t rev4(uint32_t x)
{
    x = __builtin_bswap32(x);
    return ((x & 0xF0F0F0F0u) >> 4) | ((x & 0x0F0F0F0Fu) << 4);
}
__device__ __forceinline__ uint32_t funnel(uint32_t lo, uint32_t hi, uint32_t sh)
{
    return __builtin_amdgcn_alignbit(hi, lo, sh);
}

typedef const uint32_t __attribute__((address_space(3)))* lds_words_t;

struct Stream {
    const uint32_t* words;
    uint64_t        n_words;
    uint32_t        bits;
    uint32_t        big_endian;
    lds_words_t     lds;
    uint64_t        kb;
};

__device__ __forceinline__ uint32_t ld_word_global(const Stream& s, uint64_t k)
{
    return s.words[k < s.n_words ? k : s.n_words - 1];
}
__device__ __forceinline__ uint32_t ld_word(const Stream& s, uint64_t k)
{
    return s.lds ? s.lds[(k - s.kb) * 256u] : ld_word_global(s, k);
}

__device__ __forceinline__ uint32_t fetch16_2bit(const Stream& s, uint64_t sym)
{
    const uint64_t k  = sym >> 4;
    const uint32_t sh = (uint32_t(sym) & 15u) << 1;
    uint32_t w0 = ld_word(s, k), w1 = ld_word(s, k + 1);
    if (s.big_endian) { w0 = rev2(w0); w1 = rev2(w1); }
    return funnel(w0, w1, sh);
}
__device__ __forceinline__ uint64_t fetch16_4bit(const Stream& s, uint64_t sym)
{
    const uint64_t k  = sym >> 3;
    const uint32_t sh = (uint32_t(sym) & 7u) << 2;
    uint32_t w0 = ld_word(s, k), w1 = ld_word(s, k + 1), w2 = ld_word(s, k + 2);
    if (s.big_endian) { w0 = rev4(w0); w1 = rev4(w1); w2 = rev4(w2); }
    const uint32_t lo = funnel(w0, w1, sh), hi = funnel(w1, w2, sh);
    return (uint64_t(hi) << 32) | lo;
}
struct GroupStream {
    uint32_t off;
    uint32_t carry;
    uint32_t sh;
};
__device__ __forceinline__ uint32_t stream_last_off(const Stream& s) { return uint32_t(s.n_words - 1u) * 4u; }
__device__ __forceinline__ uint32_t stream_raw(const Stream& s, uint32_t off) { return *reinterpret_cast<const uint32_t*>(reinterpret_cast<const char*>(s.words) + off); }
template <int BITS, bool BE>
__device__ __forceinline__ uint32_t canonical(uint32_t w) { return !BE ? w : BITS == 2 ? rev2(w) : rev4(w); }
__device__ __forceinline__ uint32_t stream_min(uint32_t a, uint32_t b) { return a < b ? a : b; }
template <bool BE>
__device__ __forceinline__ uint32_t stream_open_2bit(const Stream& s, const uint32_t last, uint64_t sym, GroupStream& g)
{
    const uint64_t k = sym >> 4;
    const uint32_t o0 = k < s.n_words ? uint32_t(k) * 4u : last;
    g.off = stream_min(o0 + 4u, last); g.sh = (uint32_t(sym) & 15u) << 1;
    const uint32_t w0 = canonical<2, BE>(stream_raw(s, o0));
    g.carry = canonical<2, BE>(stream_raw(s, g.off));
    return funnel(w0, g.carry, g.sh);
}
template <bool BE>
__device__ __forceinline__ uint64_t stream_open_4bit(const Stream& s, const uint32_t last, uint64_t sym, GroupStream& g)
{
    const uint64_t k = sym >> 3;
    const uint32_t o0 = k < s.n_words ? uint32_t(k) * 4u : last, o1 = stream_min(o0 + 4u, last);
    g.off = stream_min(o0 + 8u, last); g.sh = (uint32_t(sym) & 7u) << 2;
    const uint32_t w0 = canonical<4, BE>(stream_raw(s, o0)), w1 = canonical<4, BE>(stream_raw(s, o1));
    g.carry = canonical<4, BE>(stream_raw(s, g.off));
    return (uint64_t(funnel(w1, g.carry, g.sh)) << 32) | funnel(w0, w1, g.sh);
}
__device__ __forceinline__ uint32_t stream_load_2bit(const Stream& s, const uint32_t last, GroupStream& g)
{
    g.off = stream_min(g.off + 4u, last);
    return stream_raw(s, g.off);
}
__device__ __forceinline__ uint2 stream_load_4bit(const Stream& s, const uint32_t last, GroupStream& g)
{
    const uint32_t o1 = stream_min(g.off + 4u, last);
    g.off = stream_min(g.off + 8u, last);
    return make_uint2(stream_raw(s, o1), stream_raw(s, g.off));
}
template <bool BE>
__device__ __forceinline__ uint32_t stream_group_2bit(GroupStream& g, const uint32_t raw)
{
    const uint32_t w0 = g.carry;
    g.carry = canonical<2, BE>(raw);
    return funnel(w0, g.carry, g.sh);
}
template <bool BE>
__device__ __forceinline__ uint64_t stream_group_4bit(GroupStream& g, const uint2 raw)
{
    const uint32_t w0 = g.carry, w1 = canonical<4, BE>(raw.x);
    g.carry = canonical<4, BE>(raw.y);
    return (uint64_t(funnel(w1, g.carry, g.sh)) << 32) | funnel(w0, w1, g.sh);
}

__device__ __forceinline__ uint64_t fetch16_8bit(const Stream& s, uint64_t sym)
{
    const uint64_t k  = sym >> 2;
    const uint32_t sh = (uint32_t(sym) & 3u) << 3;
    uint32_t w[5];
    #pragma unroll
    for (int i = 0; i < 5; ++i) { w[i] = ld_word(s, k + i); if (s.big_endian) w[i] = __builtin_bswap32(w[i]); }
    uint64_t out = 0;
    #pragma unroll
    for (int i = 0; i < 4; ++i)
    {
        const uint32_t b = funnel(w[i], w[i + 1], sh);
        const uint32_t t = b & 0xFCFCFCFCu;
        const uint32_t big = ((((t & 0x7F7F7F7Fu) + 0x7F7F7F7Fu) | t) & 0x80808080u) >> 7;
        const uint32_t n = ~b;
        const uint32_t ff = ((((n & 0x7F7F7F7Fu) + 0x7F7F7F7Fu) | n) & 0x80808080u) >> 7;
        uint32_t v = ((b & 0x03030303u) & ~(big * 3u)) | (big << 2) | ((big & ~ff) * 15u);
        v = (v | (v >> 4)) & 0x00FF00FFu;
        v = (v | (v >> 8)) & 0x0000FFFFu;
        out |= uint64_t(v) << (16 * i);
    }
    return out;
}
__device__ __forceinline__ uint64_t expand_2to4(uint32_t v)
{
    uint64_t x = v;
    x = (x | (x << 16)) & 0x0000FFFF0000FFFFull;
    x = (x | (x <<  8)) & 0x00FF00FF00FF00FFull;
    x = (x | (x <<  4)) & 0x0F0F0F0F0F0F0F0Full;
    x = (x | (x <<  2)) & 0x3333333333333333ull;
    return x;
}
__device__ __forceinline__ uint64_t fetch_pattern16(const Stream& s, uint64_t sym)
{
    return (s.bits == 4) ? fetch16_4bit(s, sym) : (s.bits == 8) ? fetch16_8bit(s, sym) : expand_2to4(fetch16_2bit(s, sym));
}
__device__ __forceinline__ uint32_t get_symbol(const Stream& s, uint64_t sym)
{
    if (s.bits == 2) {
        const uint32_t w = ld_word(s, sym >> 4), k = uint32_t(sym) & 15u;
        return (w >> (s.big_endian ? 30u - 2u * k : 2u * k)) & 3u;
    } else if (s.bits == 4) {
        const uint32_t w = ld_word(s, sym >> 3), k = uint32_t(sym) & 7u;
        return (w >> (s.big_endian ? 28u - 4u * k : 4u * k)) & 15u;
    } else {
        const uint32_t w = ld_word(s, sym >> 2), k = uint32_t(sym) & 3u;
        return (w >> (s.big_endian ? 24u - 8u * k : 8u * k)) & 255u;
    }
}

__host__ __device__ inline uint32_t empty_pattern_exit_block(uint32_t N, uint32_t BLK, int32_t match, int32_t min_score)
{
    const uint32_t nb = BLK * ((N + BLK - 1u) / BLK), end_block = nb > BLK ? nb : BLK;
    for (uint32_t block = 0; block + BLK < end_block; block += BLK)
        if (-(1 << 30) + int32_t(N - block - BLK) * match < min_score) return block;
    return 0xFFFFFFFFu;
}

struct StringSet {
    Stream          s;
    const uint64_t* begin;
    const uint32_t* length;
    uint32_t        fixed_length;
};

inline StringSet make_string_set(const nvbio_hip_string_set* h)
{
    StringSet d;
    d.s.words = h->words; d.s.n_words = h->n_words; d.s.bits = h->bits; d.s.big_endian = h->big_endian;
    d.s.lds = nullptr; d.s.kb = 0;
    d.begin = h->begin; d.length = h->length; d.fixed_length = h->fixed_length;
    return d;
}

inline hipStream_t to_stream(void* s) { return reinterpret_cast<hipStream_t>(s); }

uint32_t seeding_grid(uint64_t n_items);

}
```

Before: 6.954 billion reads/s.

## Read substitution scores for two adjacent cells per LDS load in banded pair kernel

```diff
diff --git a/include/nvbio_hip.h b/include/nvbio_hip.h
--- a/include/nvbio_hip.h
+++ b/include/nvbio_hip.h
@@ -592,6 +592,7 @@
 const char* nvbio_hip_last_kernel_row(void);
 const char* nvbio_hip_last_kernel_const(void);
 const char* nvbio_hip_last_kernel_sub(void);
+const char* nvbio_hip_last_kernel_subread(void);
 const char* nvbio_hip_last_kernel_fetch(void);
 
 #ifdef __cplusplus
diff --git a/nvbio_amd/_lib.py b/nvbio_amd/_lib.py
--- a/nvbio_amd/_lib.py
+++ b/nvbio_amd/_lib.py
@@ -38,7 +38,7 @@
     "nvbio_hip_stream_synchronize", "nvbio_hip_stream_query", "nvbio_hip_host_malloc", "nvbio_hip_host_free", "nvbio_hip_stream_create", "nvbio_hip_stream_destroy",
     "nvbio_hip_comm_available", "nvbio_hip_device_count", "nvbio_hip_set_device", "nvbio_hip_get_device", "nvbio_hip_comm_unique_id", "nvbio_hip_comm_init_rank",
     "nvbio_hip_comm_init_all", "nvbio_hip_comm_destroy", "nvbio_hip_comm_rank", "nvbio_hip_gather_records", "nvbio_hip_comm_abort", "nvbio_hip_comm_set_transport",
-    "nvbio_hip_abi_version", "nvbio_hip_arch", "nvbio_hip_last_kernel", "nvbio_hip_last_kernel_detail", "nvbio_hip_last_kernel_cell", "nvbio_hip_last_kernel_frame", "nvbio_hip_last_kernel_row", "nvbio_hip_last_kernel_const", "nvbio_hip_last_kernel_sub", "nvbio_hip_last_kernel_fetch", "nvbio_hip_set_test_switch", "nvbio_hip_get_test_switch", "nvbio_hip_test_switch_name",
+    "nvbio_hip_abi_version", "nvbio_hip_arch", "nvbio_hip_last_kernel", "nvbio_hip_last_kernel_detail", "nvbio_hip_last_kernel_cell", "nvbio_hip_last_kernel_frame", "nvbio_hip_last_kernel_row", "nvbio_hip_last_kernel_const", "nvbio_hip_last_kernel_sub", "nvbio_hip_last_kernel_subread", "nvbio_hip_last_kernel_fetch", "nvbio_hip_set_test_switch", "nvbio_hip_get_test_switch", "nvbio_hip_test_switch_name",
 ]
 
 
@@ -271,6 +271,7 @@
         L.nvbio_hip_last_kernel_row.restype = C.c_char_p
         L.nvbio_hip_last_kernel_const.restype = C.c_char_p
         L.nvbio_hip_last_kernel_sub.restype = C.c_char_p
+        L.nvbio_hip_last_kernel_subread.restype = C.c_char_p
         _lib = L
     return _lib
 
diff --git a/nvbio_amd/csrc/banded_gotoh.hip b/nvbio_amd/csrc/banded_gotoh.hip
--- a/nvbio_amd/csrc/banded_gotoh.hip
+++ b/nvbio_amd/csrc/banded_gotoh.hip
@@ -101,6 +101,7 @@
     g_last_pair.row = (ROW & PF_ROW2) ? "fold2" : "plain";
     g_last_pair.consts = (ROW & PF_CONST2) ? "literal" : "scalar";
     g_last_pair.sub = (ROW & PF_SUBLDS) ? "lds" : "perm";
+    g_last_pair.subread = (ROW & PF_SUBLDS2) ? "pair" : (ROW & PF_SUBLDS) ? "single" : "";
     g_last_pair.fetch = "generic";
     if (!pair_stream_admitted(p)) return launch_band_pair<15, CELL, PF_SINK_VCC | ROW>(p, s);
     g_last_pair.fetch = "stream";
@@ -118,6 +119,13 @@
     {
         if (test_switch(SW_PAIR_ROW) != 1)
         {
+            if (test_switch(SW_PAIR_CONST) != 1 && test_switch(SW_PAIR_SUB) != 1 && test_switch(SW_PAIR_SUB) != 2)
+                switch (p.gap_ext) {
+                case  0: return launch_pair_row<CELL, PF_ROW2 | PF_CONST2 | PF_SUBLDS | PF_SUBLDS2>(p, s);
+                case -1: return launch_pair_row<CELL, PF_ROW2 | PF_CONST2 | PF_SUBLDS | PF_SUBLDS2 | PF_GE1>(p, s);
+                case -2: return launch_pair_row<CELL, PF_ROW2 | PF_CONST2 | PF_SUBLDS | PF_SUBLDS2 | PF_GE2>(p, s);
+                case -3: return launch_pair_row<CELL, PF_ROW2 | PF_CONST2 | PF_SUBLDS | PF_SUBLDS2 | PF_GE3>(p, s);
+                }
             if (test_switch(SW_PAIR_CONST) != 1 && test_switch(SW_PAIR_SUB) != 1)
                 switch (p.gap_ext) {
                 case  0: return launch_pair_row<CELL, PF_ROW2 | PF_CONST2 | PF_SUBLDS>(p, s);
@@ -649,4 +657,5 @@
 NVB_API const char* nvbio_hip_last_kernel_row(void)    { return pair_fact(nvb::g_last_pair.row); }
 NVB_API const char* nvbio_hip_last_kernel_const(void)  { return pair_fact(nvb::g_last_pair.consts); }
 NVB_API const char* nvbio_hip_last_kernel_sub(void)    { return pair_fact(nvb::g_last_pair.sub); }
+NVB_API const char* nvbio_hip_last_kernel_subread(void) { return pair_fact(nvb::g_last_pair.subread); }
 NVB_API const char* nvbio_hip_last_kernel_cell(void)   { return pair_fact(nvb::g_last_pair.cell); }
diff --git a/nvbio_amd/csrc/banded_gotoh_pair.h b/nvbio_amd/csrc/banded_gotoh_pair.h
--- a/nvbio_amd/csrc/banded_gotoh_pair.h
+++ b/nvbio_amd/csrc/banded_gotoh_pair.h
@@ -22,7 +22,10 @@
     PF_CONST2   = 16384 | 131072,
     PF_GE1      = 32768, PF_GE2 = 65536, PF_GE3 = PF_GE1 | PF_GE2,
     PF_SUBLDS   = 262144,
-    PF_KO_PERM  = 524288
+    PF_KO_PERM  = 524288,
+    PF_SUBLDS2  = 1048576,
+    PF_KO_XOR8  = 2097152, PF_PAD_XOR = 4194304, PF_PAD_EDGE = 8388608,
+    PF_AHEAD2   = 16777216
 };
 constexpr int pair_ge(int form)     { return (form / PF_GE1) & 3; }
 constexpr int pair_ge_bits(int ge)  { return ge * PF_GE1; }
@@ -38,7 +41,9 @@
 #define NVB_PAIR_INSTANCES_B15_LIT(X) NVB_PAIR_GES_(X, PF_SINK_VCC) NVB_PAIR_STREAM_FORMS_(NVB_PAIR_GES_, X)
 #define NVB_PAIR_SUBS_(X, F)  NVB_PAIR_GES_(X, (F) | PF_SUBLDS)
 #define NVB_PAIR_INSTANCES_B15_SUB(X) NVB_PAIR_SUBS_(X, PF_SINK_VCC) NVB_PAIR_STREAM_FORMS_(NVB_PAIR_SUBS_, X)
-#define NVB_PAIR_INSTANCES(X)         NVB_PAIR_INSTANCES_B15(X) NVB_PAIR_INSTANCES_B15_LIT(X) NVB_PAIR_INSTANCES_B15_SUB(X)
+#define NVB_PAIR_SUB2S_(X, F) NVB_PAIR_GES_(X, (F) | PF_SUBLDS | PF_SUBLDS2)
+#define NVB_PAIR_INSTANCES_B15_SUB2(X) NVB_PAIR_SUB2S_(X, PF_SINK_VCC) NVB_PAIR_STREAM_FORMS_(NVB_PAIR_SUB2S_, X)
+#define NVB_PAIR_INSTANCES(X)         NVB_PAIR_INSTANCES_B15(X) NVB_PAIR_INSTANCES_B15_LIT(X) NVB_PAIR_INSTANCES_B15_SUB(X) NVB_PAIR_INSTANCES_B15_SUB2(X)
 
 __host__ __device__ constexpr uint32_t sub_index(uint32_t ca, uint32_t cb) { return (ca & 3u) | (cb << 2) | ((ca >> 2) << 6); }
 __host__ __device__ constexpr uint32_t sub_code_a(uint32_t index)          { return (index & 3u) | ((index >> 6) << 2); }
@@ -55,6 +60,39 @@
         ro[h] = sub_bfi(0x03030303u, a >> 4, sub_bfi(0x3C3C3C3Cu, b >> 2, a));
     }
     RE = re[0] | uint64_t(re[1]) << 32; RO = ro[0] | uint64_t(ro[1]) << 32;
+}
+
+__host__ __device__ constexpr uint32_t sub2_index(uint32_t c0a, uint32_t c0b, uint32_t da, uint32_t db, uint32_t na, uint32_t nb)
+{
+    return da | (c0a << 2) | (c0b << 4) | (db << 6) | (na << 8) | (nb << 9);
+}
+__host__ __device__ constexpr uint32_t sub2_row_byte(uint32_t nib_a, uint32_t nib_b) { return (nib_a & 3u) | ((nib_b & 3u) << 2) | (nib_a >= 4u ? 64u : 0u) | (nib_b >= 4u ? 128u : 0u); }
+__host__ __device__ constexpr uint32_t sub2_col_byte(uint32_t t0a, uint32_t t0b, uint32_t t1a, uint32_t t1b) { return (t0a ^ t1a) | (t0a << 2) | (t0b << 4) | ((t0b ^ t1b) << 6); }
+__host__ __device__ constexpr uint32_t sub2_word(uint32_t index, uint32_t h, uint32_t sm, uint32_t sx)
+{
+    const uint32_t ca = ((index >> 2) & 3u) ^ (h ? index & 3u : 0u), cb = ((index >> 4) & 3u) ^ (h ? (index >> 6) & 3u : 0u);
+    return ((ca == 0u && !(index & 256u)) ? sm : sx) | (((cb == 0u && !(index & 512u)) ? sm : sx) << 16);
+}
+__device__ __forceinline__ void sub2_row_words(const uint64_t PA, const uint64_t PB, uint64_t& RE, uint64_t& RO)
+{
+    uint32_t re[2], ro[2];
+    #pragma unroll
+    for (int h = 0; h < 2; ++h)
+    {
+        const uint32_t a = uint32_t(PA >> (32 * h)), b = uint32_t(PB >> (32 * h));
+        const uint32_t na = (a | (a >> 1)) & 0x44444444u, nb = (b | (b >> 1)) & 0x44444444u;
+        re[h] = (a & 0x03030303u)        | ((b << 2) & 0x0C0C0C0Cu) | ((na << 4) & 0x40404040u) | ((nb << 5) & 0x80808080u);
+        ro[h] = ((a >> 4) & 0x03030303u) | ((b >> 2) & 0x0C0C0C0Cu) | (na & 0x40404040u)        | ((nb << 1) & 0x80808080u);
+    }
+    RE = re[0] | uint64_t(re[1]) << 32; RO = ro[0] | uint64_t(ro[1]) << 32;
+}
+__device__ __forceinline__ void sub2_col_words(const uint32_t TA, const uint32_t TB, const uint32_t prev_a, const uint32_t prev_b, uint32_t (&CW)[4])
+{
+    const uint32_t PA = (TA << 2) | prev_a, PB = (TB << 2) | prev_b, DA = TA ^ PA, DB = TB ^ PB;
+    const uint32_t ue = sub_bfi(0x33333333u, DA, PA << 2), uo = sub_bfi(0x33333333u, DA >> 2, PA);
+    const uint32_t ve = sub_bfi(0x33333333u, PB, DB << 2), vo = sub_bfi(0x33333333u, PB >> 2, DB);
+    CW[0] = sub_bfi(0x0F0F0F0Fu, ue, ve << 4); CW[2] = sub_bfi(0x0F0F0F0Fu, ue >> 4, ve);
+    CW[1] = sub_bfi(0x0F0F0F0Fu, uo, vo << 4); CW[3] = sub_bfi(0x0F0F0F0Fu, uo >> 4, vo);
 }
 
 struct PairOps {
@@ -275,12 +313,13 @@
 #define NVB_PD3_PERM2 "v_perm_b32 %[d0], %[thi], %[tlo], %[g0]\n\t" "v_perm_b32 %[d1], %[thi], %[tlo], %[g1]\n\t"
 #define NVB_PD3_XOR1  "v_xor_b32 %[d], %[tlo], %[g0]\n\t"
 #define NVB_PD3_XOR2  "v_xor_b32 %[d0], %[tlo], %[g0]\n\t" "v_xor_b32 %[d1], %[tlo], %[g1]\n\t"
-#define NVB_PD3_COL0(L) L \
+#define NVB_PD3_COL0_(L, P, Q) L \
             "v_pk_maximum3_f16 %[f0], %[f1], %[s1], %[z0]\n\t" \
-            "v_add_u32 %[d], %[s0], %[d]\n\t" \
+            "v_add_u32 %[d], %[s0], %[d]\n\t" P \
             "v_pk_max_u16 %[h], %[f0], %[d]\n\t" \
             "v_subrev_u32 %[s0], %[dd], %[h]\n\t" \
-            "v_add_u32 %[rk], %[k0], %[h]"
+            "v_add_u32 %[rk], %[k0], %[h]" Q
+#define NVB_PD3_COL0(L) NVB_PD3_COL0_(L, "", "")
 #define NVB_PD3_COL0_OUT [f0] "=&v"(F0), [d] "=&v"(d), [h] "=&v"(h), [s0] "+&v"(S0), [rk] "=&v"(rowkey)
 #define NVB_PD3_COL0_IN  [g0] "v"(g0), [tlo] "v"(tlo), [thi] "v"(thi), [f1] "v"(F1), [s1] "v"(S1), [z0] "s"(Z0)
     template <int FORM>
@@ -288,18 +327,20 @@
                                                 const uint32_t g0, const uint32_t D, const uint32_t tlo, const uint32_t thi, const uint32_t Z0, const uint32_t K0)
     {
         uint32_t d = g0, h;
-        if constexpr ((FORM & PF_SUBLDS) != 0)      asm(NVB_PD3_COL0("") : [f0] "=&v"(F0), [d] "+&v"(d), [h] "=&v"(h), [s0] "+&v"(S0), [rk] "=&v"(rowkey)
+        if constexpr ((FORM & PF_PAD_EDGE) != 0)    asm(NVB_PD3_COL0_("", "s_nop 0\n\t", "\n\ts_nop 0") : [f0] "=&v"(F0), [d] "+&v"(d), [h] "=&v"(h), [s0] "+&v"(S0), [rk] "=&v"(rowkey)
+                                                                         : [f1] "v"(F1), [s1] "v"(S1), [z0] "s"(Z0), [dd] "v"(D), [k0] "n"(klit<FORM>(0)));
+        else if constexpr ((FORM & PF_SUBLDS) != 0) asm(NVB_PD3_COL0("") : [f0] "=&v"(F0), [d] "+&v"(d), [h] "=&v"(h), [s0] "+&v"(S0), [rk] "=&v"(rowkey)
                                                                          : [f1] "v"(F1), [s1] "v"(S1), [z0] "s"(Z0), [dd] "v"(D), [k0] "n"(klit<FORM>(0)));
         else if constexpr ((FORM & PF_KO_PERM) != 0) asm(NVB_PD3_COL0(NVB_PD3_XOR1) : NVB_PD3_COL0_OUT : NVB_PD3_COL0_IN, [dd] "v"(D), [k0] "n"(klit<FORM>(0)));
         else if constexpr ((FORM & PF_CONST2) != 0) asm(NVB_PD3_COL0(NVB_PD3_PERM1) : NVB_PD3_COL0_OUT : NVB_PD3_COL0_IN, [dd] "v"(D), [k0] "n"(klit<FORM>(0)));
         else                                        asm(NVB_PD3_COL0(NVB_PD3_PERM1) : NVB_PD3_COL0_OUT : NVB_PD3_COL0_IN, [dd] "s"(D), [k0] "s"(K0));
     }
 
-#define NVB_PD3_CELL2(L, P) L \
+#define NVB_PD3_CELL2_(L, P, W0, W1) L \
             "v_pk_maximum3_f16 %[f0], %[f1], %[s1], %[z0]\n\t" \
             "v_pk_maximum3_f16 %[f1], %[f2], %[s2], %[z1]\n\t" \
-            "v_add_u32 %[d0], %[s0], %[d0]\n\t" \
-            "v_add_u32 %[d1], %[s1], %[d1]\n\t" P \
+            "v_add_u32 %[d0], %[s0], " W0 "\n\t" \
+            "v_add_u32 %[d1], %[s1], " W1 "\n\t" P \
             "v_pk_maximum3_f16 %[h], %[f0], %[d0], %[ei]\n\t" \
             "v_subrev_u32 %[s0], %[dd], %[h]\n\t" \
             "v_add_u32 %[d0], %[k0], %[h]\n\t" P \
@@ -309,6 +350,7 @@
             "v_add_u32 %[d1], %[k1], %[h]\n\t" P \
             "v_pk_max_u16 %[e], %[e], %[s1]\n\t" \
             "v_pk_maximum3_f16 %[rk], %[rk], %[d0], %[d1]"
+#define NVB_PD3_CELL2(L, P) NVB_PD3_CELL2_(L, P, "%[d0]", "%[d1]")
 #define NVB_PD3_CELL2_OUT [f0] "=&v"(F0), [f1] "+&v"(F1), [d0] "=&v"(d0), [d1] "=&v"(d1), [h] "=&v"(h), [s0] "+&v"(S0), [s1] "+&v"(S1), [e] "=&v"(E), [rk] "+&v"(rowkey)
 #define NVB_PD3_CELL2_IN  [g0] "v"(g0), [g1] "v"(g1), [tlo] "v"(tlo), [thi] "v"(thi), [f2] "v"(F2), [s2] "v"(S2), [ei] "v"(Ein), [z0] "s"(Z0), [z1] "s"(Z1)
     template <int FORM, int J>
@@ -317,7 +359,11 @@
                                                  const uint32_t Z0, const uint32_t Z1, const uint32_t K0, const uint32_t K1)
     {
         uint32_t d0 = g0, d1 = g1, h;
-        if constexpr ((FORM & PF_SUBLDS) != 0)
+        if constexpr ((FORM & PF_SUBLDS2) != 0)
+            asm(NVB_PD3_CELL2_("", "s_nop 0\n\t", "%[g0]", "%[g1]")
+                : [f0] "=&v"(F0), [f1] "+&v"(F1), [d0] "=&v"(d0), [d1] "=&v"(d1), [h] "=&v"(h), [s0] "+&v"(S0), [s1] "+&v"(S1), [e] "=&v"(E), [rk] "+&v"(rowkey)
+                : [g0] "v"(g0), [g1] "v"(g1), [f2] "v"(F2), [s2] "v"(S2), [ei] "v"(Ein), [z0] "s"(Z0), [z1] "s"(Z1), [dd] "v"(D), [k0] "n"(klit<FORM>(J)), [k1] "n"(klit<FORM>(J + 1)));
+        else if constexpr ((FORM & PF_SUBLDS) != 0)
             asm(NVB_PD3_CELL2("", "s_nop 0\n\t")
                 : [f0] "=&v"(F0), [f1] "+&v"(F1), [d0] "+&v"(d0), [d1] "+&v"(d1), [h] "=&v"(h), [s0] "+&v"(S0), [s1] "+&v"(S1), [e] "=&v"(E), [rk] "+&v"(rowkey)
                 : [f2] "v"(F2), [s2] "v"(S2), [ei] "v"(Ein), [z0] "s"(Z0), [z1] "s"(Z1), [dd] "v"(D), [k0] "n"(klit<FORM>(J)), [k1] "n"(klit<FORM>(J + 1)));
@@ -326,18 +372,19 @@
         else                                        asm(NVB_PD3_CELL2(NVB_PD3_PERM2, "") : NVB_PD3_CELL2_OUT : NVB_PD3_CELL2_IN, [dd] "s"(D), [k0] "s"(K0), [k1] "s"(K1));
     }
 
-#define NVB_PD3_TAIL2(L) L \
+#define NVB_PD3_TAIL2_(L, P, W0, W1) L \
             "v_pk_max_u16 %[f0], %[s1], %[z0]\n\t" \
-            "v_add_u32 %[d0], %[s0], %[d0]\n\t" \
-            "v_add_u32 %[d1], %[s1], %[d1]\n\t" \
+            "v_add_u32 %[d0], %[s0], " W0 "\n\t" \
+            "v_add_u32 %[d1], %[s1], " W1 "\n\t" P \
             "v_pk_maximum3_f16 %[h], %[f0], %[d0], %[ei]\n\t" \
             "v_subrev_u32 %[s0], %[dd], %[h]\n\t" \
-            "v_add_u32 %[d0], %[k0], %[h]\n\t" \
+            "v_add_u32 %[d0], %[k0], %[h]\n\t" P \
             "v_pk_max_u16 %[e], %[ei], %[s0]\n\t" \
             "v_pk_maximum3_f16 %[h], %[e], %[d1], %[z1]\n\t" \
             "v_subrev_u32 %[s1], %[dd], %[h]\n\t" \
-            "v_add_u32 %[d1], %[k1], %[h]\n\t" \
+            "v_add_u32 %[d1], %[k1], %[h]\n\t" P \
             "v_pk_maximum3_f16 %[rk], %[rk], %[d0], %[d1]"
+#define NVB_PD3_TAIL2(L) NVB_PD3_TAIL2_(L, "", "%[d0]", "%[d1]")
 #define NVB_PD3_TAIL2_OUT [f0] "=&v"(F0), [d0] "=&v"(d0), [d1] "=&v"(d1), [h] "=&v"(h), [e] "=&v"(e), [s0] "+&v"(S0), [s1] "+&v"(S1), [rk] "+&v"(rowkey)
 #define NVB_PD3_TAIL2_IN  [g0] "v"(g0), [g1] "v"(g1), [tlo] "v"(tlo), [thi] "v"(thi), [ei] "v"(Ein), [z0] "s"(Z0), [z1] "s"(Z1)
     template <int FORM, int J>
@@ -346,7 +393,17 @@
                                                  const uint32_t Z0, const uint32_t Z1, const uint32_t K0, const uint32_t K1)
     {
         uint32_t d0 = g0, d1 = g1, h, e;
-        if constexpr ((FORM & PF_SUBLDS) != 0)
+        if constexpr ((FORM & PF_SUBLDS2) != 0 && (FORM & PF_PAD_EDGE) != 0)
+            asm(NVB_PD3_TAIL2_("", "s_nop 0\n\t", "%[g0]", "%[g1]") : NVB_PD3_TAIL2_OUT
+                : [g0] "v"(g0), [g1] "v"(g1), [ei] "v"(Ein), [z0] "s"(Z0), [z1] "s"(Z1), [dd] "v"(D), [k0] "n"(klit<FORM>(J)), [k1] "n"(klit<FORM>(J + 1)));
+        else if constexpr ((FORM & PF_SUBLDS2) != 0)
+            asm(NVB_PD3_TAIL2_("", "", "%[g0]", "%[g1]") : NVB_PD3_TAIL2_OUT
+                : [g0] "v"(g0), [g1] "v"(g1), [ei] "v"(Ein), [z0] "s"(Z0), [z1] "s"(Z1), [dd] "v"(D), [k0] "n"(klit<FORM>(J)), [k1] "n"(klit<FORM>(J + 1)));
+        else if constexpr ((FORM & PF_PAD_EDGE) != 0)
+            asm(NVB_PD3_TAIL2_("", "s_nop 0\n\t", "%[d0]", "%[d1]")
+                : [f0] "=&v"(F0), [d0] "+&v"(d0), [d1] "+&v"(d1), [h] "=&v"(h), [e] "=&v"(e), [s0] "+&v"(S0), [s1] "+&v"(S1), [rk] "+&v"(rowkey)
+                : [ei] "v"(Ein), [z0] "s"(Z0), [z1] "s"(Z1), [dd] "v"(D), [k0] "n"(klit<FORM>(J)), [k1] "n"(klit<FORM>(J + 1)));
+        else if constexpr ((FORM & PF_SUBLDS) != 0)
             asm(NVB_PD3_TAIL2("")
                 : [f0] "=&v"(F0), [d0] "+&v"(d0), [d1] "+&v"(d1), [h] "=&v"(h), [e] "=&v"(e), [s0] "+&v"(S0), [s1] "+&v"(S1), [rk] "+&v"(rowkey)
                 : [ei] "v"(Ein), [z0] "s"(Z0), [z1] "s"(Z1), [dd] "v"(D), [k0] "n"(klit<FORM>(J)), [k1] "n"(klit<FORM>(J + 1)));
@@ -383,6 +440,31 @@
     template <int BAND, int R, int FORM, int END>
     struct SubCells<BAND, R, FORM, END, END> {
         static __device__ __forceinline__ void run(PairState<BAND>&, const ColumnFrame<BAND>&, const uint32_t Ein, uint32_t& E, uint32_t&, const uint32_t (&)[BAND]) { E = Ein; }
+    };
+
+    template <int FORM> static constexpr int sub2_ahead() { return (FORM & PF_AHEAD2) ? 2 : 1; }
+    template <int BAND, int R, int FORM>
+    static __device__ __forceinline__ void sub2_read(const PairState<BAND>& st, uint32_t (&w)[BAND], const uint32_t rw, const uint32_t* sub, const int k)
+    {
+        uint32_t a = rw ^ st.tc[(R + 2 * k - 1) & 15];
+        if constexpr ((FORM & PF_PAD_XOR) != 0) asm volatile("s_nop 0" : "+v"(a));
+        const uint2 t = *reinterpret_cast<const uint2*>(reinterpret_cast<const char*>(sub) + a);
+        w[2 * k - 1] = t.x; w[2 * k] = t.y;
+    }
+    template <int BAND, int R, int FORM, int K, int END>
+    struct Sub2Cells {
+        static __device__ __forceinline__ void run(PairState<BAND>& st, const ColumnFrame<BAND>& fr, const uint32_t Ein, uint32_t& E, uint32_t& rowkey, uint32_t (&w)[BAND],
+                                                   const uint32_t rw, const uint32_t* sub)
+        {
+            uint32_t En;
+            if constexpr (K + sub2_ahead<FORM>() <= (BAND - 1) / 2) sub2_read<BAND, R, FORM>(st, w, rw, sub, K + sub2_ahead<FORM>());
+            SubCells<BAND, R, FORM, 2 * K - 1, 2 * K + 1>::run(st, fr, Ein, En, rowkey, w);
+            Sub2Cells<BAND, R, FORM, K + 1, END>::run(st, fr, En, E, rowkey, w, rw, sub);
+        }
+    };
+    template <int BAND, int R, int FORM, int END>
+    struct Sub2Cells<BAND, R, FORM, END, END> {
+        static __device__ __forceinline__ void run(PairState<BAND>&, const ColumnFrame<BAND>&, const uint32_t Ein, uint32_t& E, uint32_t&, uint32_t (&)[BAND], uint32_t, const uint32_t*) { E = Ein; }
     };
 
     template <int BAND>
@@ -405,17 +487,71 @@
         fr.z[(2 * R + BAND - 2) & 15] += fr.step;
         fr.z[(2 * R + BAND - 1) & 15] += fr.step;
         uint32_t rowkey, E;
-        if constexpr ((FORM & PF_SUBLDS) != 0)
-        {
+        if constexpr ((FORM & PF_SUBLDS2) != 0)
+        {
+            st.tc[(R + BAND - 2) & 15] = g_new;
+            uint32_t w[BAND];
+            uint32_t a0 = tlo ^ st.tc[R & 15];
+            if constexpr ((FORM & PF_PAD_XOR) != 0) asm volatile("s_nop 0" : "+v"(a0));
+            w[0] = *reinterpret_cast<const uint32_t*>(reinterpret_cast<const char*>(sub) + a0);
+            #pragma unroll
+            for (int k = 1; k <= sub2_ahead<FORM>(); ++k) sub2_read<BAND, R, FORM>(st, w, tlo, sub, k);
+            col0<FORM>(st.F[0], st.F[1], st.S[0], st.S[1], rowkey, w[0], fr.D, 0u, 0u, fr.z[(2 * R) & 15], fr.k[0]);
+            Sub2Cells<BAND, R, FORM, 1, (BAND - 1) / 2>::run(st, fr, st.S[0], E, rowkey, w, tlo, sub);
+            tail2<FORM, BAND - 2>(st.F[BAND - 2], st.S[BAND - 2], st.S[BAND - 1], E, rowkey, w[BAND - 2], w[BAND - 1], fr.D, 0u, 0u,
+                                  fr.z[(2 * R + BAND - 2) & 15], fr.z[(2 * R + BAND - 1) & 15], fr.k[BAND - 2], fr.k[BAND - 1]);
+        }
+        else if constexpr ((FORM & PF_KO_XOR8) != 0)
+        {
+            struct alignas(4) W2 { uint32_t x, y; };
             constexpr int HEAD = 8, SPLIT = 5;
             st.tc[(R + BAND - 1) & 15] = g_new;
             uint32_t w[BAND], Em;
             #pragma unroll
-            for (int j = 0; j < HEAD; ++j) w[j] = *reinterpret_cast<const uint32_t*>(reinterpret_cast<const char*>(sub) + (tlo ^ st.tc[(R + j) & 15]));
+            for (int j = 0; j < HEAD; j += 2) { const W2 t = *reinterpret_cast<const W2*>(reinterpret_cast<const char*>(sub) + (tlo ^ st.tc[(R + j) & 15])); w[j] = t.x; if (j + 1 < BAND) w[j + 1] = t.y; }
             col0<FORM>(st.F[0], st.F[1], st.S[0], st.S[1], rowkey, w[0], fr.D, 0u, 0u, fr.z[(2 * R) & 15], fr.k[0]);
             SubCells<BAND, R, FORM, 1, SPLIT>::run(st, fr, st.S[0], Em, rowkey, w);
             #pragma unroll
-            for (int j = HEAD; j < BAND; ++j) w[j] = *reinterpret_cast<const uint32_t*>(reinterpret_cast<const char*>(sub) + (tlo ^ st.tc[(R + j) & 15]));
+            for (int j = HEAD; j < BAND; j += 2) { const W2 t = *reinterpret_cast<const W2*>(reinterpret_cast<const char*>(sub) + (tlo ^ st.tc[(R + j) & 15])); w[j] = t.x; if (j + 1 < BAND) w[j + 1] = t.y; }
+            SubCells<BAND, R, FORM, SPLIT, BAND - 2>::run(st, fr, Em, E, rowkey, w);
+            tail2<FORM, BAND - 2>(st.F[BAND - 2], st.S[BAND - 2], st.S[BAND - 1], E, rowkey, w[BAND - 2], w[BAND - 1], fr.D, 0u, 0u,
+                                  fr.z[(2 * R + BAND - 2) & 15], fr.z[(2 * R + BAND - 1) & 15], fr.k[BAND - 2], fr.k[BAND - 1]);
+        }
+        else if constexpr ((FORM & PF_SUBLDS) != 0)
+        {
+            constexpr int HEAD = 8, SPLIT = 5;
+            st.tc[(R + BAND - 1) & 15] = g_new;
+            uint32_t w[BAND], Em;
+            if constexpr ((FORM & PF_PAD_XOR) != 0)
+            {
+                uint32_t a[HEAD];
+                #pragma unroll
+                for (int j = 0; j < HEAD; ++j) a[j] = tlo ^ st.tc[(R + j) & 15];
+                asm volatile("s_nop 0" : "+v"(a[0]), "+v"(a[1]), "+v"(a[2]), "+v"(a[3]), "+v"(a[4]), "+v"(a[5]), "+v"(a[6]), "+v"(a[7]));
+                #pragma unroll
+                for (int j = 0; j < HEAD; ++j) w[j] = *reinterpret_cast<const uint32_t*>(reinterpret_cast<const char*>(sub) + a[j]);
+            }
+            else
+            {
+                #pragma unroll
+                for (int j = 0; j < HEAD; ++j) w[j] = *reinterpret_cast<const uint32_t*>(reinterpret_cast<const char*>(sub) + (tlo ^ st.tc[(R + j) & 15]));
+            }
+            col0<FORM>(st.F[0], st.F[1], st.S[0], st.S[1], rowkey, w[0], fr.D, 0u, 0u, fr.z[(2 * R) & 15], fr.k[0]);
+            SubCells<BAND, R, FORM, 1, SPLIT>::run(st, fr, st.S[0], Em, rowkey, w);
+            if constexpr ((FORM & PF_PAD_XOR) != 0)
+            {
+                uint32_t a[BAND - HEAD];
+                #pragma unroll
+                for (int j = HEAD; j < BAND; ++j) a[j - HEAD] = tlo ^ st.tc[(R + j) & 15];
+                asm volatile("s_nop 0" : "+v"(a[0]), "+v"(a[1]), "+v"(a[2]), "+v"(a[3]), "+v"(a[4]), "+v"(a[5]), "+v"(a[6]));
+                #pragma unroll
+                for (int j = HEAD; j < BAND; ++j) w[j] = *reinterpret_cast<const uint32_t*>(reinterpret_cast<const char*>(sub) + a[j - HEAD]);
+            }
+            else
+            {
+                #pragma unroll
+                for (int j = HEAD; j < BAND; ++j) w[j] = *reinterpret_cast<const uint32_t*>(reinterpret_cast<const char*>(sub) + (tlo ^ st.tc[(R + j) & 15]));
+            }
             SubCells<BAND, R, FORM, SPLIT, BAND - 2>::run(st, fr, Em, E, rowkey, w);
             tail2<FORM, BAND - 2>(st.F[BAND - 2], st.S[BAND - 2], st.S[BAND - 1], E, rowkey, w[BAND - 2], w[BAND - 1], fr.D, 0u, 0u,
                                   fr.z[(2 * R + BAND - 2) & 15], fr.z[(2 * R + BAND - 1) & 15], fr.k[BAND - 2], fr.k[BAND - 1]);
@@ -445,17 +581,27 @@
 
 template <typename CELL, int BAND, int FORM, int R, int END>
 struct PairRows {
+    template <int NX>
     static __device__ __forceinline__ void run(PairState<BAND>& st, ColumnFrame<BAND>& fr, const uint32_t i0, const uint32_t M, const uint32_t D, const uint32_t G,
-                                               const uint64_t PA, const uint64_t PB, const uint32_t (&XT)[2], const uint32_t* tab, const uint32_t (&KT)[2], uint32_t& rk2)
+                                               const uint64_t PA, const uint64_t PB, const uint32_t (&XT)[NX], const uint32_t* tab, const uint32_t (&KT)[2], uint32_t& rk2)
     {
         if ((FORM & PF_KO_BOUND) || i0 + R < M)
         {
-            if constexpr ((FORM & PF_SUBLDS) != 0)
+            if constexpr ((FORM & PF_SUBLDS2) != 0)
+            {
+                constexpr int K = R >> 1, Q = R >> 2;
+                const uint32_t zw = uint32_t(((R & 1) ? PB : PA) >> (32 * (K >> 2))), xw = XT[R & 3];
+                uint32_t rw = (K & 3) == 0 ? (zw << 5) & 0x1FE0u : (zw >> ((8 * (K & 3) + 27) & 31)) & 0x1FE0u;
+                uint32_t cw = Q == 0 ? (xw << 3) & 0x7F8u : (xw >> ((8 * Q + 29) & 31)) & 0x7F8u;
+                asm("" : "+v"(rw)); asm("" : "+v"(cw));
+                CELL::template row<BAND, R, FORM>(st, fr, i0 + R, cw, rw, 0u, rk2, tab);
+            }
+            else if constexpr ((FORM & PF_SUBLDS) != 0)
             {
                 constexpr int K = R >> 1;
                 const uint32_t zw = uint32_t(((R & 1) ? PB : PA) >> (32 * (K >> 2))), xw = XT[R & 1];
-                uint32_t rw = (K & 3) == 0 ? (zw << 2) & 0x3FCu : (zw >> (8 * (K & 3) - 2)) & 0x3FCu;
-                uint32_t cw = K == 0 ? (xw << 2) & 0x3Cu : (xw >> (4 * K - 2)) & 0x3Cu;
+                uint32_t rw = (K & 3) == 0 ? (zw << 2) & 0x3FCu : (zw >> ((8 * (K & 3) + 30) & 31)) & 0x3FCu;
+                uint32_t cw = K == 0 ? (xw << 2) & 0x3Cu : (xw >> ((4 * K + 30) & 31)) & 0x3Cu;
                 asm("" : "+v"(rw)); asm("" : "+v"(cw));
                 CELL::template row<BAND, R, FORM>(st, fr, i0 + R, cw, rw, 0u, rk2, tab);
             }
@@ -476,7 +622,8 @@
     }
 };
 template <typename CELL, int BAND, int FORM, int END> struct PairRows<CELL, BAND, FORM, END, END> {
-    static __device__ __forceinline__ void run(PairState<BAND>&, ColumnFrame<BAND>&, uint32_t, uint32_t, uint32_t, uint32_t, uint64_t, uint64_t, const uint32_t (&)[2], const uint32_t*, const uint32_t (&)[2], uint32_t&) {}
+    template <int NX>
+    static __device__ __forceinline__ void run(PairState<BAND>&, ColumnFrame<BAND>&, uint32_t, uint32_t, uint32_t, uint32_t, uint64_t, uint64_t, const uint32_t (&)[NX], const uint32_t*, const uint32_t (&)[2], uint32_t&) {}
 };
 
 constexpr int PAIR_LANES = 128;
@@ -485,17 +632,27 @@
 banded_gotoh_pair_kernel(const GotohParams p)
 {
     static_assert(BAND >= 3 && BAND <= 16, "the ring of 16");
-    constexpr bool STREAM = (FORM & PF_STREAM) != 0, KEY = (FORM & PF_SINK_KEY) != 0, FOLD2 = (FORM & PF_FOLD2) != 0, SUBLDS = (FORM & PF_SUBLDS) != 0;
+    constexpr bool STREAM = (FORM & PF_STREAM) != 0, KEY = (FORM & PF_SINK_KEY) != 0, FOLD2 = (FORM & PF_FOLD2) != 0, SUBLDS = (FORM & PF_SUBLDS) != 0, SUBLDS2 = (FORM & PF_SUBLDS2) != 0;
     static_assert(!(FORM & (PF_SUBLDS | PF_KO_PERM)) || ((FORM & PF_FOLD2) && (FORM & PF_CONST2) == PF_CONST2), "the LDS words and the probe's xor row are forms of the library's row");
     static_assert(!SUBLDS || !(FORM & (PF_KO_TABLE | PF_KO_PERM)), "the LDS words have no lookup to knock out");
+    static_assert(!(FORM & (PF_SUBLDS2 | PF_KO_XOR8 | PF_PAD_XOR | PF_PAD_EDGE | PF_AHEAD2)) || SUBLDS, "the pair read, its ceiling and the pads are forms of the LDS words' row");
+    static_assert(!SUBLDS2 || !(FORM & PF_KO_XOR8), "the ceiling is the single read's row");
     static_assert(!(FORM & (PF_FOLD2 | PF_CONST2)) || CELL::COLUMN, "the pair fold and the literals are the column frame's");
     static_assert(!FOLD2 || !(FORM & (PF_SINK_KEY | PF_KO_SINK | PF_KO_BOUND)), "the pair fold is the compare-and-select fold's, over the job's own rows");
     static_assert(!(FORM & PF_GE3) || (FORM & PF_CONST2), "|G_e| is the literal form's parameter");
     constexpr bool P4 = !(FORM & PF_PAT2), PBE = (FORM & PF_PBE) != 0, TBE = (FORM & PF_TBE) != 0;
     __shared__ uint32_t s_tab[16];
-    __shared__ uint32_t s_sub[256];
-    if constexpr (SUBLDS)
-    {
+    __shared__ uint32_t s_sub[(FORM & PF_KO_XOR8) ? 258 : 256];
+    __shared__ uint2 s_sub2[1024];
+    if constexpr (SUBLDS2)
+    {
+        const uint32_t tg = uint32_t(-p.gap_ext * 32);
+        const uint32_t sm = uint32_t((p.match - p.gap_open) * 32) + tg, sx = uint32_t((p.mismatch - p.gap_open) * 32) + tg;
+        for (uint32_t k = threadIdx.x; k < 1024u; k += uint32_t(PAIR_LANES)) s_sub2[k] = make_uint2(sub2_word(k, 0u, sm, sx), sub2_word(k, 1u, sm, sx));
+    }
+    else if constexpr (SUBLDS)
+    {
+        if constexpr ((FORM & PF_KO_XOR8) != 0) { if (threadIdx.x < 2u) s_sub[256u + threadIdx.x] = 0u; }
         const uint32_t tg = uint32_t(-p.gap_ext * 32);
         const uint32_t sm = uint32_t((p.match - p.gap_open) * 32) + tg, sx = uint32_t((p.mismatch - p.gap_open) * 32) + tg;
         for (uint32_t k = threadIdx.x; k < 256u; k += uint32_t(PAIR_LANES))
@@ -536,10 +693,19 @@
     uint32_t rk2 = 0u;
     {
         const uint32_t TA = fetch16_2bit(ts[0], tb[0]), TB = fetch16_2bit(ts[1], tb[1]);
-        #pragma unroll
-        for (int j = 0; j < BAND - 1; ++j)
-            st.tc[j] = SUBLDS ? (((TA >> (2 * j)) & 3u) | (((TB >> (2 * j)) & 3u) << 2)) << 2
-                              : CELL::SEL_BASE | ((TA >> (2 * j)) & 3u) | (((TB >> (2 * j)) & 3u) << 16);
+        if constexpr (SUBLDS2)
+        {
+            #pragma unroll
+            for (int t = 0; t < 16; ++t)
+                st.tc[t] = t < BAND - 2 ? sub2_col_byte((TA >> (2 * t)) & 3u, (TB >> (2 * t)) & 3u, (TA >> (2 * t + 2)) & 3u, (TB >> (2 * t + 2)) & 3u) << 3 : 0u;
+        }
+        else
+        {
+            #pragma unroll
+            for (int j = 0; j < BAND - 1; ++j)
+                st.tc[j] = SUBLDS ? (((TA >> (2 * j)) & 3u) | (((TB >> (2 * j)) & 3u) << 2)) << 2
+                                  : CELL::SEL_BASE | ((TA >> (2 * j)) & 3u) | (((TB >> (2 * j)) & 3u) << 16);
+        }
     }
 
     const uint32_t plast = stream_last_off(p.pat.s), tlast = stream_last_off(p.txt.s);
@@ -575,7 +741,16 @@
             PAn = fetch_pattern16(ps[0], pb[0] + i0 + 16u); PBn = fetch_pattern16(ps[1], pb[1] + i0 + 16u);
             TAn = fetch16_2bit(ts[0], tb[0] + i0 + 16u + BAND - 1); TBn = fetch16_2bit(ts[1], tb[1] + i0 + 16u + BAND - 1);
         }
-        if constexpr (SUBLDS)
+        if constexpr (SUBLDS2)
+        {
+            uint64_t RE, RO;
+            sub2_row_words(PA, PB, RE, RO);
+            uint32_t CW[4];
+            const uint32_t last = st.tc[12] ^ (st.tc[12] >> 2);
+            sub2_col_words(TA, TB, (last >> 3) & 3u, (last >> 7) & 3u, CW);
+            PairRows<CELL, BAND, FORM, 0, 16>::run(st, fr, i0, M, D, G, RE, RO, CW, reinterpret_cast<const uint32_t*>(s_sub2), KT, rk2);
+        }
+        else if constexpr (SUBLDS)
         {
             uint64_t RE, RO;
             sub_row_words(PA, PB, RE, RO);
@@ -602,13 +777,17 @@
     }
 
     if constexpr (FOLD2) { if (M & 1u) CELL::template fold_last<BAND, FORM>(st, rk2, M, d32, g32); }
+    uint32_t lane_out = SUBLDS2 ? lane : 0u;
+    if constexpr (SUBLDS2) asm volatile("" : "+v"(lane_out));
+    const uint32_t id2[2] = { 2u * lane_out, 2u * lane_out + 1u < p.n ? 2u * lane_out + 1u : 2u * lane_out };
+    const uint32_t (&od)[2] = SUBLDS2 ? id2 : id;
     #pragma unroll
     for (int h = 0; h < 2; ++h)
     {
-        if (h == 1 && id[1] == id[0]) break;
+        if (h == 1 && od[1] == od[0]) break;
         const uint32_t j = st.best[h] & (FOLD2 ? 15u : 31u), i = KEY ? (st.best[h] >> 5) & 1023u : st.besti[h] + (FOLD2 ? (st.best[h] >> 4) & 1u : 0u);
-        p.out_score[id[h]] = int32_t(st.best[h] >> (KEY ? 20 : 5));
-        reinterpret_cast<uint2*>(p.out_sink)[id[h]] = make_uint2(i + j + 1u, i + 1u);
+        p.out_score[od[h]] = int32_t(st.best[h] >> (KEY ? 20 : 5));
+        reinterpret_cast<uint2*>(p.out_sink)[od[h]] = make_uint2(i + j + 1u, i + 1u);
     }
 }
 
diff --git a/nvbio_amd/csrc/banded_gotoh_pair_b15_sub2.hip b/nvbio_amd/csrc/banded_gotoh_pair_b15_sub2.hip
--- /dev/null
+++ b/nvbio_amd/csrc/banded_gotoh_pair_b15_sub2.hip
@@ -0,0 +1,6 @@
+#include "banded_gotoh_pair.h"
+namespace nvb {
+#define NVB_INST(CELL, F) template hipError_t launch_band_pair<15, CELL, (F)>(const GotohParams&, hipStream_t);
+NVB_PAIR_INSTANCES_B15_SUB2(NVB_INST)
+#undef NVB_INST
+}
diff --git a/nvbio_amd/csrc/common.h b/nvbio_amd/csrc/common.h
--- a/nvbio_amd/csrc/common.h
+++ b/nvbio_amd/csrc/common.h
@@ -16,6 +16,7 @@
     const char* row    = "";
     const char* consts = "";
     const char* sub    = "";
+    const char* subread = "";
 };
 extern thread_local PairLaunch g_last_pair;
 
```

Result: faster. 7.074 billion reads/s, median of 6 (+1.7%).
